# carlobaldassi/gimp-lqr-plugin

Measured on AMD Instinct MI355X. Metric: Mseams*pixels/sec on 4K RGBA, higher is better.
Workload: dtype f32; 1 GPU; batch4k: 64 x 3840x2160 RGBA per GPU, resize to 3640x2160 (200 vertical seams each), side-switch 2; images_per_gpu=64, width=3840, height=2160, new_width=3640, new_height=2160, parallelism=images sharded i mod N, no data-path collective, streams_per_gpu=1

## Files before the change

gimp-lqr-plugin_amd/csrc/k_levels.hip:

```cpp
#include "lqr_common.h"
#include "lqr_kernels.h"

__device__ unsigned long long g_lv_stats[8];
#ifdef LQR_TIMING
__device__ unsigned long long g_lv_time[16][2][10];
#define LTT(i) do { __builtin_amdgcn_sched_barrier(0); const unsigned long long t__ = __builtin_readcyclecounter(); __builtin_amdgcn_sched_barrier(0); ltt[i] += t__ - ltprev; ltprev = t__; } while (0)
extern "C" int lqrhip_band_levels_timing(unsigned long long *out) { (void) hipDeviceSynchronize(); return hipMemcpyFromSymbol(out, HIP_SYMBOL(g_lv_time), sizeof(unsigned long long) * 320) == hipSuccess ? 0 : -1; }
#else
#define LTT(i) do { } while (0)
#endif
__device__ int g_lv_dbg;

#ifdef LQR_JITTER
#define LJIT(site) do { if (dbg & 16) { unsigned h__ = (unsigned) (slot * 131 + L * 17 + (site) * 7 + epoch * 2654435761u + q * 40503u + image * 977u); h__ ^= h__ >> 13; h__ *= 0x5bd1e995u; h__ ^= h__ >> 15; \
    for (unsigned i__ = h__ & 15u; i__ > 0; i__--) __builtin_amdgcn_s_sleep(127); } } while (0)
#else
#define LJIT(site) do { } while (0)
#endif
__device__ __forceinline__ unsigned long long uni64(unsigned long long v)
{
    return ((unsigned long long) (unsigned) __builtin_amdgcn_readfirstlane((int) (v >> 32)) << 32) | (unsigned) __builtin_amdgcn_readfirstlane((int) v);
}
struct LvMask {
    unsigned long long lo;
    __device__ __forceinline__ void set(int t) { lo |= 1ull << t; }
    __device__ __forceinline__ bool has(int t) const { return t >= 0 && t < LV_MAX_TILES && ((lo >> t) & 1ull); }
    __device__ __forceinline__ void set_range(int a, int b) { lo |= ((b - a >= 63) ? ~0ull : ((1ull << (b - a + 1)) - 1ull)) << a; }
    __device__ __forceinline__ int first() const { return lo ? __builtin_ctzll(lo) : -1; }
    __device__ __forceinline__ int last() const { return lo ? 63 - __builtin_clzll(lo) : -1; }
};

template <bool LR, bool RIG, int DELTA, bool RIGM>
__global__ __launch_bounds__(128) __attribute__((amdgpu_waves_per_eu(2, 2)))
void k_band_levels(DevCarver *cs, DpK p, int w, int h, int stride, unsigned long long *exch, int epoch, int *dev_err, int P, int n_img)
{
    static_assert(DELTA >= 1 && DELTA <= LQR_FAST_MAX_DELTA && (DELTA <= 4 || RIG) && (RIG || !RIGM), "delta_x 1 .. 10 (5 .. 10: the rigidity form, with a zero table if there is none); a rigidity mask only matters with rigidity");
    constexpr int PX = 2, HALO = 32, OWN = LV_OWN, HL = 16, R = lv_rows(DELTA, RIGM), TILE = 128;
    static_assert(R * DELTA <= HALO, "a level's errors stay inside the halo");
    typedef LaneVec<2>::F FV;
    typedef LaneVec<2>::L LV;
    typedef GLOBAL_AS FV GFV;
    typedef GLOBAL_AS LV GLV;
    typedef GLOBAL_AS unsigned long long gu64;
    __shared__ int s_tlo[LV_MAX_LEVELS], s_thi[LV_MAX_LEVELS];
    __shared__ int s_fail;
    __shared__ int s_polled;
    __shared__ unsigned long long s_A[2];
        const int tid = threadIdx.x, lane = tid & 63;
    const int q = __builtin_amdgcn_readfirstlane(tid >> 6);
    const int dbg = __builtin_amdgcn_readfirstlane(g_lv_dbg);
    const int b_xcd = (int) blockIdx.x & 7, b_k = (int) blockIdx.x >> 3;
    const int slot = (dbg & 8) ? (int) blockIdx.x % P : b_k % P, image = (dbg & 8) ? (int) blockIdx.x / P : (b_k / P) * 8 + b_xcd;
    if (image >= n_img) return;
    const int nblk = (h + R - 1) / R;
    const int ntiles = lv_tiles(w);
    GCarver c = gview(cs[image]);
    if constexpr (RIG && DELTA == 1 && !RIGM) { c.en = uni_ptr(c.en); c.m = uni_ptr(c.m); c.least = uni_ptr(c.least); }
    const size_t near_off = lv_near_off(ntiles);
    gu64 *ex_img = (gu64 *) exch + exch_image_off(image, near_off);
    gu64 *flagw = ex_img;
    gu64 *gran = ex_img + LV_FLAG_WORDS;
    const float INF = __int_as_float(0x7f800000);
    const float rig_l = p.rigmap[0], rig_r = p.rigmap[2];
    float rg[2 * DELTA + 1];
#pragma unroll
    for (int i = 0; i < 2 * DELTA + 1; i++) rg[i] = p.rigmap[i];
    const int ix_own = 2 * (lane % P), ix_right = 2 * ((lane + 1) % P), ix_left = 2 * ((lane + P - 1) % P);

    for (int i = tid; i < nblk; i += 128) { s_tlo[i] = 1 << 30; s_thi[i] = -1; }
    if (tid == 0) { s_fail = 0; s_polled = -1; }
    __syncthreads();
    for (int y = tid; y < h; y += 128) {
        const int v0 = c.seam_x[y], vm = c.seam_x[max(y - 1, 0)], vp = c.seam_x[min(y + 1, h - 1)];
        const int t0 = max(min(min(v0, vm), vp) - DELTA - 1, 0), t1 = min(max(max(v0, vm), vp) + DELTA, w - 1);
        atomicMin(&s_tlo[y / R], t0); atomicMax(&s_thi[y / R], t1);
    }
    __syncthreads();
    __shared__ unsigned long long s_tm[LV_MAX_LEVELS + 2];
    for (int L = tid; L < nblk + 2; L += 128) {
        unsigned long long m = 0ull;
        if (L < nblk && s_thi[L] >= s_tlo[L]) {
            const int a = max(0, (s_tlo[L] - (OWN - 1 + HALO + 2) + OWN - 1) / OWN), b = min(ntiles - 1, (s_thi[L] + HALO + 2) / OWN);
            m = ((b - a >= 63) ? ~0ull : ((1ull << (b - a + 1)) - 1ull)) << a;
        }
        s_tm[L] = m;
    }
    __syncthreads();
    auto touch_mask = [&](int L) -> LvMask {
        LvMask m;
        m.lo = uni64(s_tm[L]);
        return m;
    };
    unsigned long long res_mine = 0ull;
    for (int t = slot; t < LV_MAX_TILES; t += P) res_mine |= 1ull << t;
    res_mine = uni64(res_mine);
    auto my_tile = [&](const LvMask &A, int which) -> int {
        unsigned long long m = A.lo & res_mine;
        if (which && m) m &= m - 1ull;
        return m ? __builtin_ctzll(m) : -1;
    };
    auto any_collision = [&](const LvMask &A) -> bool {
        const int a = A.first(), b = A.last();
        if (a < 0 || b - a < 2 * P) return false;
        unsigned long long res_zero = 0ull;
        for (int t = 0; t < LV_MAX_TILES; t += P) res_zero |= 1ull << t;
        for (int r = 0; r < P; r++)
            if (__popcll(A.lo & (res_zero << r)) > 2) return true;
        return false;
    };
    auto nearest_tile = [&](int a, int b) -> int {
        const unsigned long long up_m = res_mine & (~0ull << a), dn_m = res_mine & (b >= 63 ? ~0ull : ((1ull << (b + 1)) - 1ull));
        const int up = up_m ? __builtin_ctzll(up_m) : -1, dn = dn_m ? 63 - __builtin_clzll(dn_m) : -1;
        if (up >= 0 && up <= b) return up;
        if (up < 0 || up >= ntiles) return dn;
        if (dn < 0) return up;
        return (up - b <= a - dn) ? up : dn;
    };

    int cur_t = -1, cur_L = -1;
    bool cur_full = false;
    int x0 = 0;
    unsigned lo_off = 0;
    constexpr bool LEAN = RIG && DELTA == 1 && !RIGM;
    bool in[PX] = {false, false}, own = false, interior = false;
    const bool own_lane = lane >= HL && lane < 64 - HL;
    auto X0 = [&]() -> int { int v = x0; asm volatile("" : "+v"(v)); return v; };
    auto in_k = [&](int k) -> bool { if constexpr (LEAN) return (unsigned) (X0() + k) < (unsigned) w; else return in[k]; };
    auto is_own = [&]() -> bool { if constexpr (LEAN) return own_lane && X0() < w; else return own; };
    auto is_interior = [&]() -> bool {
        if constexpr (LEAN) { const int t0 = __builtin_amdgcn_readfirstlane(X0()); return t0 >= 0 && t0 + TILE <= w; }
        else return interior;
    };
    auto set_tile = [&](int t) {
        x0 = t * OWN - HALO + PX * lane;
        lo_off = (unsigned) min(max(x0, 0), stride - PX);
        if constexpr (!LEAN) {
#pragma unroll
            for (int k = 0; k < PX; k++) in[k] = x0 + k >= 0 && x0 + k < w;
            own = own_lane && x0 < w;
            interior = (x0 - PX * lane >= 0) && (x0 - PX * lane + TILE <= w);
        }
    };
    auto owner_of = [&](int t) -> int { return lane < HL ? t - 1 : lane >= 64 - HL ? t + 1 : t; };
    const int owner_col = lane < HL ? HALO + PX * lane : lane >= 64 - HL ? PX * (lane - (64 - HL)) : PX * (lane - HL);
    FV q_e[R], q_mo[R], q_ab, q_rf[RIGM ? R : 1];
    LV q_lo[R];
    q_ab[0] = q_ab[1] = INF;
    auto issue_full = [&](int L) {
        const int ybase = L * R;
#pragma unroll
        for (int r = 0; r < R; r++) {
            const unsigned row = (unsigned) min(ybase + r, h - 1) * (unsigned) stride;
            const unsigned ro = row + lo_off, ro4 = (row << 2) + (lo_off << 2);
            q_e[r] = *(const GFV *) ((const gu8 *) c.en + ro4);
            q_mo[r] = *(const GFV *) ((const gu8 *) c.m + ro4);
            q_lo[r] = *(const GLV *) (c.least + ro);
            if (RIGM) q_rf[RIGM ? r : 0] = *(const GFV *) ((const gu8 *) c.rig + ro4);
        }
        q_ab = *(const GFV *) ((const gu8 *) c.m + ((((unsigned) max(ybase - 1, 0) * (unsigned) stride) + lo_off) << 2));
    };
    float mp[PX] = {INF, INF};
    int acc_l0 = 0, acc_l1 = 0;
    auto batch_u = [&](int ybase) {
        const int nr = min(R, h - ybase);
#pragma unroll
        for (int r = 0; r < R; r++) {
            float mc[PX], e[PX], mo[PX];
            uint32_t lnew = 0;
            bool ch[PX];
#pragma unroll
            for (int k = 0; k < PX; k++) { e[k] = q_e[r][k]; mo[k] = q_mo[r][k]; }
            if constexpr (DELTA == 1 && !RIGM) {
                const float left = __int_as_float(__builtin_amdgcn_mov_dpp(__float_as_int(mp[PX - 1]), DPP_WAVE_SHR1, 0xf, 0xf, true));
                const float right = __int_as_float(__builtin_amdgcn_mov_dpp(__float_as_int(mp[0]), DPP_WAVE_SHL1, 0xf, 0xf, true));
                dp_row<PX, LR, RIG, true, false>(mp, left, right, e, mo, (uint32_t) q_lo[r], in, rig_l, rig_r, mc, lnew, ch);
            } else {
                float nl[DELTA], nr[DELTA], rf[PX];
                lane_reach<PX, DELTA>(mp, nl, nr);
#pragma unroll
                for (int k = 0; k < PX; k++) rf[k] = RIGM ? q_rf[RIGM ? r : 0][k] : 1.0f;
                dp_row_g<PX, DELTA, LR, RIG, RIGM, true, false>(mp, nl, nr, e, mo, (uint32_t) q_lo[r], in, rg, rf, mc, lnew, ch);
            }
            if (r == 0 && ybase == 0) {
#pragma unroll
                for (int k = 0; k < PX; k++) mc[k] = e[k];
                lnew = 0;
            }
            if (r == R - 1) {
                const int msk = (r < nr) ? -1 : 0;
                acc_l0 = (__float_as_int(mc[0]) ^ __float_as_int(mo[0])) & msk;
                acc_l1 = (__float_as_int(mc[1]) ^ __float_as_int(mo[1])) & msk;
            }
#pragma unroll
            for (int k = 0; k < PX; k++) { mp[k] = mc[k]; q_mo[r][k] = mc[k]; }
            q_lo[r] = (LV) lnew;
        }
    };
    auto store_u = [&](int ybase) {
        const bool own_ = is_own();
        const unsigned inc = own_ ? (unsigned) stride : 0u, inc4 = inc * 4u;
        unsigned so = own_ ? (unsigned) ybase * (unsigned) stride + (unsigned) x0 : (unsigned) h * (unsigned) stride + (unsigned) (PX * lane), so4 = so * 4u;
        const int nr = min(R, h - ybase);
#pragma unroll
        for (int r = 0; r < R; r++, so += inc, so4 += inc4) {
            if (r < nr) {
                *(GFV *) ((gu8 *) c.m + so4) = q_mo[r];
                *(GLV *) (c.least + so) = q_lo[r];
            }
        }
    };
    auto wait_level = [&](int L, int spec_t, const LvMask &prev, unsigned long long &fw, unsigned long long (&g)[PX]) -> int {
        const unsigned want = ((unsigned) epoch << 10) | (unsigned) L;
        gu64 *fsrc = flagw + (size_t) ((L - 1) & 1) * 2 * LV_PMAX + (lane < 2 * P ? lane : 0);
        const bool need_g = spec_t >= 0 && prev.has(owner_of(spec_t)) && (in_k(0) || in_k(1));
        gu64 *gsrc = gran + ((size_t) ((L - 1) & 1) * ntiles + (need_g ? owner_of(spec_t) : 0)) * OWN + (need_g ? owner_col : 0);
        int sp = 0;
        while (true) {
            const size_t off = (!(dbg & 4) && (sp & 3) != 3) ? near_off : 0;
            fw = __hip_atomic_load(fsrc + off, __ATOMIC_RELAXED, __HIP_MEMORY_SCOPE_AGENT);
            if (spec_t >= 0) {
#pragma unroll
                for (int k = 0; k < PX; k++) g[k] = __hip_atomic_load(gsrc + off + k, __ATOMIC_RELAXED, __HIP_MEMORY_SCOPE_AGENT);
            }
            const bool okf = __all(lane >= 2 * P || (unsigned) (fw >> 32) == want);
            bool okg = true;
#pragma unroll
            for (int k = 0; k < PX; k++) okg &= (unsigned) (g[k] >> 32) == want;
            if (okf && __all(!need_g || okg)) return 0;
            if (dbg & 2) __builtin_amdgcn_s_sleep(16); else if (okf || sp < 8) __builtin_amdgcn_s_sleep(1); else if (sp < 64) __builtin_amdgcn_s_sleep(8); else __builtin_amdgcn_s_sleep(48);
            ++sp;
            if ((sp & 255) == 0 && dev_failed(dev_err)) return 1;
            if (sp > (1 << 18)) { if (lane == 0) dev_fail(dev_err, DEVERR_TILE_TIMEOUT); return 1; }
        }
    };
    auto row_above = [&](int L, int t, const LvMask &prev, bool have_g, unsigned long long (&g)[PX]) -> int {
        const int u = owner_of(t);
        const bool from_gran = prev.has(u) && (in_k(0) || in_k(1));
        if (!have_g) {
            gu64 *src = gran + ((size_t) ((L - 1) & 1) * ntiles + (from_gran ? u : 0)) * OWN + (from_gran ? owner_col : 0);
            const unsigned want = ((unsigned) epoch << 10) | (unsigned) L;
            int sp = 0;
            while (true) {
                const size_t off = (!(dbg & 4) && (sp & 3) != 3) ? near_off : 0;
#pragma unroll
                for (int k = 0; k < PX; k++) g[k] = __hip_atomic_load(src + off + k, __ATOMIC_RELAXED, __HIP_MEMORY_SCOPE_AGENT);
                bool ok = true;
#pragma unroll
                for (int k = 0; k < PX; k++) ok &= (unsigned) (g[k] >> 32) == want;
                if (__all(ok || !from_gran)) break;
                __builtin_amdgcn_s_sleep(1);
                if (++sp > (1 << 16)) { if (lane == 0) dev_fail(dev_err, DEVERR_TILE_TIMEOUT); return 1; }
            }
        }
#pragma unroll
        for (int k = 0; k < PX; k++) mp[k] = !in_k(k) ? INF : from_gran ? __uint_as_float((unsigned) g[k]) : q_ab[k];
        return 0;
    };
    unsigned n_proc = 0, n_idle = 0, n_sync = 0, n_two = 0;
    int hold_L = -1;
#ifdef LQR_TIMING
    unsigned long long ltt[10] = {0, 0, 0, 0, 0, 0, 0, 0, 0, 0};
    unsigned long long ltprev = __builtin_readcyclecounter();
    const unsigned long long ltstart = ltprev;
#endif
    for (int L = 0; L <= nblk; L++) {
        const bool mine = (L & 1) == q;
        int t = -1;
        bool have_g = false, passed = false;
        unsigned long long g[PX] = {0ull, 0ull};
        LvMask A = {0ull}, A_prev = {0ull};
        if (L > 0) A_prev.lo = uni64(s_A[(L - 1) & 1]);
        LTT(8);
        if (mine) {
            unsigned long long fw = 0;
            A = touch_mask(L);
            passed = true;
            if (L > 0) {
                const int spec_t = (hold_L < 0 && cur_full && cur_L == L && L < nblk && !(dbg & 1)) ? cur_t : -1;
                LJIT(1);
                const int wl_rc = wait_level(L, spec_t, A_prev, fw, g);
                LJIT(2);
                LTT(0);
                if (wl_rc) { LDS_FLAG(s_fail) = 1; passed = false; }
                else if (L < nblk) {
                    const int wl = (int) (unsigned) fw;
                    bool act = false;
                    unsigned wo[2], wr[2], wlf[2];
#pragma unroll
                    for (int i = 0; i < 2; i++) {
                        wo[i] = (unsigned) __builtin_amdgcn_ds_bpermute((ix_own + i) << 2, wl);
                        wr[i] = (unsigned) __builtin_amdgcn_ds_bpermute((ix_right + i) << 2, wl);
                        wlf[i] = (unsigned) __builtin_amdgcn_ds_bpermute((ix_left + i) << 2, wl);
                    }
#pragma unroll
                    for (int i = 0; i < 2; i++) {
                        act |= (wo[i] & 0x900u) == 0x900u && (int) (wo[i] & 0xffu) == lane;
                        act |= (wr[i] & 0xa00u) == 0xa00u && (int) (wr[i] & 0xffu) == lane + 1;
                        act |= (wlf[i] & 0xc00u) == 0xc00u && (int) (wlf[i] & 0xffu) == lane - 1;
                    }
                    A.lo |= __ballot(act && lane < ntiles);
                    have_g = spec_t >= 0;
                }
            }
            if (lane == 0) { s_A[L & 1] = A.lo; if (passed) LDS_FLAG(s_polled) = L; }
        } else {
            int spins = 0;
            while (LDS_FLAG(s_polled) < L && LDS_FLAG(s_fail) != 1 && ++spins < (1 << 24)) __builtin_amdgcn_s_sleep(1);
            passed = LDS_FLAG(s_polled) >= L;
            if (passed) A.lo = uni64(s_A[L & 1]);
            else if (LDS_FLAG(s_fail) != 1) { LDS_FLAG(s_fail) = 1; if (lane == 0) dev_fail(dev_err, DEVERR_TILE_TIMEOUT); }
            LTT(2);
        }
        LTT(1);
        LJIT(3);
        if (hold_L >= 0 && passed) { store_u(hold_L * R); hold_L = -1; }
        LTT(3);
        if (L == nblk) break;
        if (mine && passed && any_collision(A)) {
            if (slot == 0 && lane == 0) { __hip_atomic_fetch_min(c.flags + FLAG_OVF_ROW, L * R, __ATOMIC_RELAXED, __HIP_MEMORY_SCOPE_AGENT); atomicAdd(&g_lv_stats[0], 1ull); }
            LDS_FLAG(s_fail) = 2;
            passed = false;
        }
        if (passed) t = my_tile(A, mine ? 0 : 1);
        if (!mine && t < 0 && passed && lane == 0) {
            const unsigned long long tag = (unsigned long long) (((unsigned) epoch << 10) | (unsigned) (L + 1)) << 32;
            gu64 *fdst = flagw + (size_t) (L & 1) * 2 * LV_PMAX + 2 * slot + 1;
            if (!(dbg & 4)) __hip_atomic_store(fdst + near_off, tag, __ATOMIC_RELAXED, __HIP_MEMORY_SCOPE_WORKGROUP);
            __hip_atomic_store(fdst, tag, __ATOMIC_RELAXED, __HIP_MEMORY_SCOPE_AGENT);
        }
        {
            int ld_t = -1, ld_L = L;
            if (t >= 0) {
                if (!(cur_full && cur_t == t && cur_L == L)) { ld_t = t; n_sync++; have_g = false; }
                if (!mine) n_two++;
            } else if (!mine && passed && L + 1 < nblk) {
                LvMask M = touch_mask(L + 1);
                M.lo |= A.lo;
                int pt = my_tile(M, 0);
                if (pt < 0 && M.first() >= 0) { pt = nearest_tile(M.first(), M.last()); if (pt < M.first() - 1 || pt > M.last() + 1 || pt >= ntiles) pt = -1; }
                ld_t = pt; ld_L = L + 1;
                cur_t = -1; cur_L = ld_L; cur_full = false;
            }
            LTT(1);
            LJIT(4);
            if (ld_t >= 0) { set_tile(ld_t); issue_full(ld_L); cur_t = ld_t; cur_L = ld_L; cur_full = true; }
#ifdef LQR_TIMING
            if (t >= 0 && ld_t >= 0) asm volatile("s_waitcnt vmcnt(0)" ::: "memory");
#endif
            LTT(4);
        }
        unsigned word = 0;
        if (t >= 0) {
            n_proc++;
            if (L > 0 && row_above(L, t, A_prev, have_g, g)) LDS_FLAG(s_fail) = 1;
#ifdef LQR_TIMING
            asm volatile("s_waitcnt vmcnt(0)" ::: "memory");
#endif
            LTT(5);
            if (!is_interior()) {
                const bool ik[PX] = {in_k(0), in_k(1)};
#pragma unroll
                for (int r = 0; r < R; r++)
#pragma unroll
                    for (int k = 0; k < PX; k++) { q_e[r][k] = ik[k] ? q_e[r][k] : INF; q_mo[r][k] = ik[k] ? q_mo[r][k] : INF; }
            }
            batch_u(L * R);
            LTT(6);
            hold_L = L;
            cur_full = false;
            LJIT(5);
            if (L + 1 < nblk && own_lane) {
                gu64 *dst = gran + ((size_t) (L & 1) * ntiles + t) * OWN + PX * (lane - HL);
                const unsigned long long tag = (unsigned long long) (((unsigned) epoch << 10) | (unsigned) (L + 1)) << 32;
#pragma unroll
                for (int k = 0; k < PX; k++) {
                    if (!(dbg & 4)) __hip_atomic_store(dst + near_off + k, tag | __float_as_uint(mp[k]), __ATOMIC_RELAXED, __HIP_MEMORY_SCOPE_WORKGROUP);
                    __hip_atomic_store(dst + k, tag | __float_as_uint(mp[k]), __ATOMIC_RELAXED, __HIP_MEMORY_SCOPE_AGENT);
                }
            }
            const bool chg = own_lane && (acc_l0 | acc_l1) != 0;
            const bool any_o = __any(chg), any_l = __any(chg && lane < 32), any_r = __any(chg && lane >= 32);
            word = 0x800u | (any_o ? 0x100u : 0u) | (any_l ? 0x200u : 0u) | (any_r ? 0x400u : 0u) | (unsigned) t;
        } else if (mine && passed) n_idle++;
        LJIT(6);
        if (lane == 0 && (t >= 0 || mine) && LDS_FLAG(s_fail) == 0) {
            const unsigned long long tag = (unsigned long long) (((unsigned) epoch << 10) | (unsigned) (L + 1)) << 32;
            gu64 *fdst = flagw + (size_t) (L & 1) * 2 * LV_PMAX + 2 * slot + (mine ? 0 : 1);
            if (!(dbg & 4)) __hip_atomic_store(fdst + near_off, tag | word, __ATOMIC_RELAXED, __HIP_MEMORY_SCOPE_WORKGROUP);
            __hip_atomic_store(fdst, tag | word, __ATOMIC_RELAXED, __HIP_MEMORY_SCOPE_AGENT);
        }
        LTT(7);
        asm volatile("s_waitcnt lgkmcnt(0)\n\ts_barrier" ::: "memory");
        LTT(8);
        if (LDS_FLAG(s_fail)) return;
    }
#ifdef LQR_TIMING
    if (image == 0 && lane == 0 && slot < 16) { ltt[9] = __builtin_readcyclecounter() - ltstart; for (int i = 0; i < 10; i++) g_lv_time[slot][q][i] = ltt[i]; }
#endif
    if (lane == 0) { atomicAdd(&g_lv_stats[2], (unsigned long long) n_proc); atomicAdd(&g_lv_stats[3], (unsigned long long) n_idle); if (n_two) atomicAdd(&g_lv_stats[4], (unsigned long long) n_two); }
    if (lane == 0 && n_sync) atomicAdd(&g_lv_stats[1], (unsigned long long) n_sync);
}

extern "C" void lqrhip_band_levels_debug(int v) { if (lqrhip_init() < 0) return; (void) hipMemcpyToSymbol(HIP_SYMBOL(g_lv_dbg), &v, sizeof v); }
extern "C" int lqrhip_band_levels_stats(unsigned long long *out, int reset)
{
    if (lqrhip_init() < 0) return -1;
    (void) hipDeviceSynchronize();
    if (hipMemcpyFromSymbol(out, HIP_SYMBOL(g_lv_stats), sizeof(unsigned long long) * 8) != hipSuccess) return -1;
    if (reset) { unsigned long long z[8] = {0}; (void) hipMemcpyToSymbol(HIP_SYMBOL(g_lv_stats), z, sizeof z); }
    return 0;
}

#define INST(...) template __global__ void k_band_levels<__VA_ARGS__>(DevCarver *, DpK, int, int, int, unsigned long long *, int, int *, int, int);
K_BAND_LEVELS_FORMS(INST)
#undef INST
```

gimp-lqr-plugin_amd/csrc/lqr_geom.h:

```cpp
#pragma once
#include <stddef.h>
#include <stdint.h>
#include "lqr_beside.h"

constexpr int tiles_of(int w, int own) { return (w + own - 1) / own; }
constexpr size_t blocks_of(size_t n, size_t per) { return (n + per - 1) / per; }

constexpr size_t LDS_ATTR_BYTES = 64 * 1024;
constexpr bool lds_needs_attr(size_t bytes) { return bytes > LDS_ATTR_BYTES; }
constexpr size_t VMAP_T_ATTR_BYTES = 56 * 1024;
constexpr bool vmap_t_needs_attr(size_t bytes) { return bytes > VMAP_T_ATTR_BYTES; }

constexpr int PLANE_SLACK = 1024;
constexpr int plane_stride(int w) { return ((w + 16) + 63) & ~63; }
constexpr size_t plane_elems(int stride, int h) { return (size_t) stride * (h + 1) + PLANE_SLACK; }
constexpr int SEAM_X_SLACK = 8;
constexpr size_t seam_x_elems(int h) { return (size_t) h + SEAM_X_SLACK; }
constexpr size_t seam_log_elems(int n_seams, int h) { return (size_t) n_seams * h; }

struct MaskClip { int x0, y0, x1, y1, nx, ny; };
constexpr MaskClip mask_clip(int w0, int h0, int width, int height, int x_off, int y_off, int transposed)
{
    const int wt = transposed ? h0 : w0, ht = transposed ? w0 : h0;
    const int x0 = x_off < 0 ? x_off : 0, y0 = y_off < 0 ? y_off : 0;
    const int x1 = x_off > 0 ? x_off : 0, y1 = y_off > 0 ? y_off : 0;
    const long long xe = (long long) width + x_off, ye = (long long) height + y_off;
    const int x2 = wt < xe ? wt : (int) xe, y2 = ht < ye ? ht : (int) ye;
    return MaskClip{x0, y0, x1, y1, x2 - x1, y2 - y1};
}

constexpr int dppx_px(int px) { return px == 3 ? 2 : px; }
constexpr int dppx_hl(int px) { return px == 3 ? 24 : 16; }
constexpr int dpp_halo(int px) { return dppx_hl(px) * dppx_px(px); }
constexpr int dpp_own(int px) { return 64 * dppx_px(px) - 2 * dpp_halo(px); }
constexpr int dpp_ex_tile(int px) { return px == 3 ? 2 * dpp_own(3) : 2 * 2 * dpp_halo(px); }
constexpr int dpp_tiles(int w, int px) { return tiles_of(w, dpp_own(px)); }
constexpr int DPP_CTR_WORDS = 8;
constexpr size_t dpp_ctr_off(int ntiles, int px) { return (size_t) ntiles * dpp_ex_tile(px); }
constexpr size_t dpp_near_off(int ntiles, int px) { return dpp_ctr_off(ntiles, px) + DPP_CTR_WORDS; }
constexpr size_t exch_image_off(size_t image, size_t near_off) { return image * 2 * near_off; }
constexpr size_t exch_words(size_t near_off, size_t n) { return 2 * near_off * n; }
constexpr int exch_layout_dpp(int px) { return px; }
constexpr int EXCH_LAYOUT_LEVELS = 103;
constexpr int DPP_EPOCH_BITS = 19;
constexpr int dpp_epoch(int launches) { return 1 + (launches % ((1 << DPP_EPOCH_BITS) - 2)); }

constexpr int LV_PMAX = 16;
constexpr int LV_OWN = 64;
constexpr int lv_tiles(int w) { return tiles_of(w, LV_OWN); }
constexpr int LV_FLAG_WORDS = 4 * LV_PMAX;
constexpr size_t lv_near_off(int ntiles) { return (size_t) LV_FLAG_WORDS + (size_t) 2 * ntiles * LV_OWN; }
constexpr int LV_LEVEL_BITS = 10, LV_EPOCH_BITS = 22;
constexpr int lv_epoch(int launches) { return 1 + (launches % ((1 << LV_EPOCH_BITS) - 2)); }
struct LvBlock { int image, slot; };
constexpr unsigned lv_grid(size_t n, int P) { return (unsigned) (8 * ((n + 7) / 8) * P); }
constexpr LvBlock lv_block(int b, int P) { return LvBlock{((b >> 3) / P) * 8 + (b & 7), (b >> 3) % P}; }

struct CuBlock { bool energy; int image, index; };
constexpr int cu_energy_blocks(int n, int h) { return n * bb_energy_entries(h); }
constexpr unsigned cu_grid(unsigned n, int h) { return n * (unsigned) bb_energy_entries(h) + n * (unsigned) bb_carve_entries(h); }
constexpr CuBlock cu_block(unsigned b, int n, int h)
{
    const int eblk = bb_energy_entries(h), ne = n * eblk;
    if ((int) b < ne) {
        const int img = b / eblk, blk = b - img * eblk;
        return CuBlock{true, img, blk};
    }
    const int rblk = bb_carve_entries(h), cb = b - ne, img = cb / rblk, rb = cb - img * rblk;
    return CuBlock{false, img, rb};
}
constexpr unsigned cv_grid(unsigned n, int h) { return n + (unsigned) bb_entries((int) n, h); }
constexpr size_t cv_list_words(int n, int h) { return (size_t) BB_LIST_HEAD + (size_t) bb_entries(n, h); }

constexpr int VP_MAP_SLACK = 64;
constexpr int vp_col_blocks(int w) { return (w + 255) / 256; }
constexpr int vp_quads(int rows) { return (rows + 3) / 4; }
constexpr size_t vp_map_bytes(int nchunks, int stride) { return (size_t) (nchunks + 1) * stride + VP_MAP_SLACK; }
constexpr size_t vp_path_bytes(int nchunks, int stride, int rows) { return vp_map_bytes(nchunks, stride) * 4 * vp_quads(rows); }
constexpr size_t vp_map_row(int chunk, int stride) { return (size_t) chunk * stride; }
constexpr size_t vp_path_chunk(int chunk, int R4, int stride) { return (size_t) chunk * R4 * stride; }
constexpr size_t vp_path_quad(int r4, int stride) { return (size_t) r4 * stride; }
constexpr size_t vp_path_step(int chunk, int R4, int r, int stride, int x) { return (((size_t) chunk * R4 + (r >> 2)) * stride + x) * 4 + (r & 3); }
constexpr size_t vp_solve_lds(int nchunks) { return (size_t) (nchunks + 2) * sizeof(int); }

constexpr int FC_SLACK = 16;
constexpr int fc_w_from(int from, int to, int w_at_to) { return w_at_to + (to - from); }
constexpr int fc_rem_off(int from, int to) { return to - from; }
constexpr size_t fc_lds(int from, int to, int w_from) { return (size_t) (to - from) * sizeof(int) + (size_t) w_from + FC_SLACK; }
constexpr int vsc_lvl_off(int n_seams) { return n_seams; }
constexpr size_t vsc_lds(int n_seams, int wc0) { return ((size_t) n_seams + wc0) * sizeof(int); }
constexpr size_t VSC_LDS_MAX = 150 * 1024;
constexpr size_t inflate_lds(int l, int max_level) { return (size_t) ((l - max_level + 1 + 31) / 32 + 1) * sizeof(unsigned); }
constexpr int VT_LINES = 32;
constexpr size_t vmap_words(int depth) { return (size_t) (depth + 31) / 32; }
constexpr size_t vmap_check_lds(int depth) { return vmap_words(depth) * sizeof(unsigned); }
constexpr size_t vmap_check_t_lds(int depth) { return VT_LINES * vmap_words(depth) * sizeof(unsigned); }
constexpr int vmap_t_blocks(int width) { return tiles_of(width, VT_LINES); }
constexpr size_t band_mw_lds(int h) { return (size_t) h * sizeof(int); }
constexpr size_t band_tw_lds(int h) { return (size_t) 2 * h * sizeof(int); }
constexpr int band_tw_touchR_off(int h) { return h; }
constexpr size_t BAND_MW_LDS_MAX = 60 * 1024, BAND_TW_LDS_MAX = 64 * 1024;
constexpr bool band_mw_fits(int h) { return band_mw_lds(h) <= BAND_MW_LDS_MAX; }
constexpr bool band_tw_fits(int h) { return band_tw_lds(h) <= BAND_TW_LDS_MAX; }
constexpr int sweep_wpad(int w) { return (w + 3) & ~3; }
constexpr size_t sweep_lds(int w) { return (size_t) 2 * sweep_wpad(w) * sizeof(float); }
constexpr size_t fwd_lds(int L) { return (size_t) 2 * L * sizeof(float); }
constexpr int fwd_row_off(int parity, int L) { return parity * L; }

constexpr int CLIP_COST_FLOATS = 4, CLIP_REFRESH_VALUES = 6;
constexpr size_t clip_intensity_elems(int n, size_t px) { return (size_t) n * px; }
constexpr size_t clip_frame_off(int t, size_t px) { return (size_t) t * px; }
constexpr size_t clip_cost_elems(size_t px) { return px * CLIP_COST_FLOATS; }
constexpr size_t clip_cost_off(int y, int x, int L) { return ((size_t) y * L + x) * CLIP_COST_FLOATS; }
constexpr int clip_fold_groups(int n, int group) { return tiles_of(n, group); }
constexpr int clip_refresh_off(int wave) { return wave * CLIP_REFRESH_VALUES; }
constexpr size_t clip_refresh_lds_elems(int threads) { return (size_t) (threads / 64) * CLIP_REFRESH_VALUES; }
```

gimp-lqr-plugin_amd/csrc/lqr_kernels.h:

```cpp
#pragma once
#include "lqr_common.h"
#include "lqr_pixel.h"


template <class FORM> __global__ void k_wk_init(const DevCarver *cs, int w, int h, int stride, typename FORM::Arg a);
template <class FORM> __global__ __launch_bounds__(256) void k_wk_init_visible(const DevCarver *cs, int w0, int h, int stride, typename FORM::Arg a);
#define K_EMAP_FORMS(X) X(0, false) X(1, false) X(2, false) X(3, false) X(4, false) X(5, false) X(6, false) X(0, true) X(1, true) X(2, true) X(6, true)
#define K_EMAP_UPDATE_NT_FORMS(X, ...) X(12, __VA_ARGS__) X(36, __VA_ARGS__) X(68, __VA_ARGS__)
template <int NRG, bool VALUE> __global__ void k_emap_full(const DevCarver *cs, DpK p, int w, int h, int stride);
#define K_WK_INIT_EMAP_FORMS(X) X(0) X(1) X(2) X(3) X(4) X(5) X(6)
template <int NRG> __global__ __launch_bounds__(256) void k_wk_init_emap(const DevCarver *cs, DpK p, int w, int h, int stride);
__global__ void k_mask_add(float *plane, int w0, const uint8_t *mask, int channels, int mw, int x0, int y0, int x1, int y1,
                           int nx, int ny, int transposed, int is_rig, int bias_factor);
template <int NRG, int EU_NT, bool VALUE> __global__ __launch_bounds__(64) void k_emap_update(const DevCarver *cs, DpK p, int w, int h, int stride, int k, int epoch);
template <bool VALUE> __global__ __launch_bounds__(256) void k_frozen_catchup(const DevCarver *cs, int from, int to, int w_from, int h, int stride);

__global__ __launch_bounds__(VPATH_THREADS) void k_vpath(const DevCarver *cs, int w, int h, int stride, int lr, int delta, int log_index, int moved_unit);
#define K_VPATH1_FORMS(X) X(1) X(2) X(3) X(4) X(5) X(6) X(7)
#define K_VP_FORMS(X) K_VPATH1_FORMS(X) X(8) X(9) X(10)
template <int DELTA> __global__ __launch_bounds__(VPATH_THREADS) void k_vpath1(const DevCarver *cs, int w, int h, int stride, int lr, int log_index, int moved_unit);
unsigned long long *lqr_moved_bytes_dev(void);

template <int DELTA> __global__ __launch_bounds__(256) void k_vp_maps(const DevCarver *cs, int w, int h, int stride);
template <int DELTA> __global__ __launch_bounds__(VPATH_THREADS) void k_vp_solve(const DevCarver *cs, int w, int h, int stride, int lr, int log_index, int moved_unit);

__global__ __launch_bounds__(256) void k_carve(const DevCarver *cs, int w, int h, int stride, int delta, int move_dp);
#define K_CARVE_E_FORMS(X) X(0) X(1) X(2) X(3) X(4) X(5) X(6)
template <int NRG> __global__ __launch_bounds__(256) void k_carve_e(const DevCarver *cs, DpK p, int w, int h, int stride, int move_dp, int k, int epoch);
#define K_CARVE_U_FORMS(X) X(0) X(1) X(2) X(3) X(4) X(5) X(6)
template <int NRG> __global__ __launch_bounds__(256) void k_carve_u(const DevCarver *cs, DpK p, int w, int h, int stride, int move_dp, int k, int epoch, int n);
#define K_CARVE_V_DELTAS(X) X(1) X(2)
#define K_CARVE_V_FORMS(X) X(0, 1) X(1, 1) X(2, 1) X(3, 1) X(4, 1) X(5, 1) X(6, 1) X(0, 2) X(1, 2) X(2, 2) X(3, 2) X(4, 2) X(5, 2) X(6, 2)
template <int NRG, int DELTA> __global__ __launch_bounds__(256) __attribute__((amdgpu_waves_per_eu(5))) void k_carve_v(const DevCarver *cs, DpK p, int w, int h, int stride, int lr, int move_dp, int k, int epoch, int n,
                                                                                  int moved_unit, unsigned tag, unsigned long long *list, unsigned long long *moved_bytes, int *dev_err);

#define K_DP_SWEEP_PXT_FORMS(X) X(1) X(2) X(4) X(8) X(16)
#define K_LR_RIG_FORMS(X) X(false, false) X(false, true) X(true, false) X(true, true)
template <int PXT, bool UPDATE, int NTH = DP_THREADS> __global__ __launch_bounds__(NTH) void k_dp_sweep(const DevCarver *cs, DpK p, int w, int h, int stride, int lr);
__global__ __launch_bounds__(64) void k_band_update(const DevCarver *cs, DpK p, int w, int h, int stride, int lr);
template <int PXL, int NW, int R, bool LR, bool RIG> __global__ __launch_bounds__(64 * NW) void k_band_update_mw(const DevCarver *cs, DpK p, int w, int h, int stride);
template <int NW, bool LR, bool RIG> __global__ __launch_bounds__(128 * NW) void k_band_update_tw(const DevCarver *cs, DpK p, int w, int h, int stride, int *dev_err);

template <bool LR, bool RIG> __global__ __launch_bounds__(64) void k_dp_tile(const DevCarver *cs, DpK p, int w, int h, int stride, int y0);
#define K_DP_TILE_P_FORMS_D(X, LR, UPD, D) X(GENERAL, 2, LR, false, UPD, D, false, 16) X(GENERAL, 2, LR, true, UPD, D, false, 16) X(GENERAL, 2, LR, true, UPD, D, true, 16)
#define K_DP_TILE_P_FORMS_W(X, LR, UPD, D) X(GENERAL, 2, LR, true, UPD, D, false, 16) X(GENERAL, 2, LR, true, UPD, D, true, 16)
#define K_DP_TILE_P_FORMS_LR(X, LR, UPD) \
    X(PX4, 4, LR, false, UPD, 1, false, 16) X(PX4, 4, LR, true, UPD, 1, false, 16) X(PLAIN, 2, LR, false, UPD, 1, false, 16) X(PLAIN, 2, LR, true, UPD, 1, false, 16) \
    X(GENERAL, 2, LR, true, UPD, 1, true, 16) K_DP_TILE_P_FORMS_D(X, LR, UPD, 2) K_DP_TILE_P_FORMS_D(X, LR, UPD, 3) K_DP_TILE_P_FORMS_D(X, LR, UPD, 4) \
    K_DP_TILE_P_FORMS_W(X, LR, UPD, 5) K_DP_TILE_P_FORMS_W(X, LR, UPD, 6) K_DP_TILE_P_FORMS_W(X, LR, UPD, 7) K_DP_TILE_P_FORMS_W(X, LR, UPD, 8) K_DP_TILE_P_FORMS_W(X, LR, UPD, 9) K_DP_TILE_P_FORMS_W(X, LR, UPD, 10)
#define K_DP_TILE_P_FORMS_24(X, UPD) X(PLAIN, 2, false, false, UPD, 1, false, 24) X(PLAIN, 2, false, true, UPD, 1, false, 24) X(PLAIN, 2, true, false, UPD, 1, false, 24) X(PLAIN, 2, true, true, UPD, 1, false, 24)
#define K_DP_TILE_P_FORMS(X) K_DP_TILE_P_FORMS_LR(X, false, false) K_DP_TILE_P_FORMS_LR(X, false, true) K_DP_TILE_P_FORMS_LR(X, true, false) K_DP_TILE_P_FORMS_LR(X, true, true) \
    K_DP_TILE_P_FORMS_24(X, false) K_DP_TILE_P_FORMS_24(X, true)
template <int PX, bool LR, bool RIG, bool UPDATE, int DELTA = 1, bool RIGM = false, int HLN = 16>
__global__ __launch_bounds__(64 * DPP_W) void k_dp_tile_p(DevCarver *cs, DpK p, int w, int h, int stride, unsigned long long *exch, int epoch, int *dev_err);

#define K_BAND_LEVELS_FORMS_D(X, LR, D) X(LR, false, D, false) X(LR, true, D, false) X(LR, true, D, true)
#define K_BAND_LEVELS_FORMS_W(X, LR, D) X(LR, true, D, false) X(LR, true, D, true)
#define K_BAND_LEVELS_FORMS_LR(X, LR) K_BAND_LEVELS_FORMS_D(X, LR, 1) K_BAND_LEVELS_FORMS_D(X, LR, 2) K_BAND_LEVELS_FORMS_D(X, LR, 3) K_BAND_LEVELS_FORMS_D(X, LR, 4) \
    K_BAND_LEVELS_FORMS_W(X, LR, 5) K_BAND_LEVELS_FORMS_W(X, LR, 6) K_BAND_LEVELS_FORMS_W(X, LR, 7) K_BAND_LEVELS_FORMS_W(X, LR, 8) K_BAND_LEVELS_FORMS_W(X, LR, 9) K_BAND_LEVELS_FORMS_W(X, LR, 10)
#define K_BAND_LEVELS_FORMS(X) K_BAND_LEVELS_FORMS_LR(X, false) K_BAND_LEVELS_FORMS_LR(X, true)
template <bool LR, bool RIG, int DELTA, bool RIGM>
__global__ __launch_bounds__(128) __attribute__((amdgpu_waves_per_eu(2, 2))) void k_band_levels(DevCarver *cs, DpK p, int w, int h, int stride, unsigned long long *exch, int epoch, int *dev_err, int P, int n_img);

__global__ __launch_bounds__(256) void k_vs_commit(const DevCarver *cs, int w0, int h0, int wc0, int n_seams, int first_level, int finish);
template <bool DEEP> __global__ __launch_bounds__(256) void k_inflate(const InflateDev *jobs, int w0, int w1, int l, int max_level, int *dev_err);
__global__ __launch_bounds__(256) void k_vmap_check(const int32_t *map, int len, int depth, int *dev_err);
__global__ __launch_bounds__(256) void k_vmap_check_t(const int32_t *map, int32_t *out, int width, int height, int depth, int *dev_err);
__global__ __launch_bounds__(256) void k_seam_check(const DevCarver *cs, int h, int wc0, int n_seams, int delta, int *dev_err);
__global__ __launch_bounds__(256) void k_vs_rollback(const DevCarver *cs, size_t n, int first_level, int finish_level);
__global__ void k_inject(const DevCarver *cs, int what, int h, int w0, int log_index, int first_level);
template <bool DEEP> __global__ __launch_bounds__(256) void k_compact(const uint8_t *rgb, const int32_t *vs, const float *bias, const float *rig,
                                                  uint8_t *nrgb, float *nbias, float *nrig, int32_t *nvmap, int w0, int w, int ch, int level, int depth);
template <bool DEEP> __global__ __launch_bounds__(256) void k_compact_jobs(const InflateDev *jobs, int w0, int w, int level);
__global__ void k_transpose(const InflateDev *jobs, int w, int h);
__global__ void k_transpose_px(const InflateDev *jobs, int w, int h);
__global__ __launch_bounds__(256) void k_mask_line_max(const uint8_t *mask, int channels, int width, int a0, int b0, int line_len, int direction, int *out);

#define K_COMPACT_SIZES_FORMS(X) X(false) X(true)
#define K_TRANSPOSE_SIZES_FORMS(X) X(false) X(true)
template <bool DEEP> __global__ __launch_bounds__(256) void k_compact_sizes(const uint8_t *rgb, const int32_t *vs, const SizeJob *jobs, int n_jobs, int w0, int bytes);
template <bool WIDE> __global__ __launch_bounds__(256) void k_transpose_sizes(const SizeJob *jobs, int h, int bytes);

#define K_FWD_INIT_FORMS(X) X(0) X(1) X(2) X(3)
#define K_FWD_SEAM_FORMS(X) X(1) X(2) X(4) X(8) X(16)
template <int DEPTH> __global__ __launch_bounds__(256) void k_fwd_init(const FwdJob *jobs, int L, int H, int fw0, int strided, DeepRead rd, int w_start, int orientation);
template <int PXT> __global__ __launch_bounds__(FWD_THREADS) void k_fwd_seam(const FwdJob *jobs, int wc, int L, int H);
__global__ __launch_bounds__(FWD_REMOVE_THREADS) void k_fwd_remove(const FwdJob *jobs, int wc, int L, int H, int level, int orientation);

#define K_CLIP_SEAM_FORMS(X) X(1) X(2) X(4) X(8) X(16)
__global__ __launch_bounds__(CLIPFWD_FOLD_THREADS) void k_clip_fold(const FwdJob *jobs, const float *in, int first, int count, int last, int L, int H, int fw0, int strided,
                                                                   int w_start, float temporal, float *cost, float *pm);
template <int PXT> __global__ __launch_bounds__(FWD_THREADS) void k_clip_seam(const float *cost, int8_t *choice, int32_t *seam, int wc, int L, int H);
__global__ __launch_bounds__(FWD_REMOVE_THREADS) void k_clip_remove(float *cost, uint16_t *pos, const int32_t *seam, int32_t *map, int wc, int L, int H, int level, int orientation);
__global__ __launch_bounds__(CLIPFWD_REFRESH_THREADS) void k_clip_refresh(const float *in, int n, float *cost, const uint16_t *pos, const int32_t *seam, int wn, int L, int H);

#define K_STATIC_FOLD_FORMS(X) X(0, 0, true) X(1, 0, true) X(2, 0, true) X(6, 0, true) X(0, 0, false) X(1, 0, false) X(2, 0, false) X(6, 0, false) \
    X(0, 1, false) X(1, 1, false) X(2, 1, false) X(6, 1, false) X(0, 2, false) X(1, 2, false) X(2, 2, false) X(6, 2, false) \
    X(0, 3, false) X(1, 3, false) X(2, 3, false) X(6, 3, false)
template <int NRG, int DEPTH, bool PACKED>
__global__ __launch_bounds__(STATIC_THREADS) void k_static_fold(const StaticFrame *frames, int count, int first, int W, int H, int transposed, int orientation, DeepRead rd,
                                                     float alpha, float *s_plane, float *t_plane, float *i_plane, float *e_out);

template <class T> __global__ __launch_bounds__(256) void k_mask_add_f(float *plane, int w0, const T *mask, int mw, int x0, int y0, int x1, int y1, int nx, int ny,
                                                                       int transposed, int is_rig, int bias_factor);
__global__ __launch_bounds__(256) void k_mask_scatter(float *plane, const int *index, const double *value, size_t n, int is_rig);
__global__ __launch_bounds__(256) void k_plane_transpose(const float *plane, float *out, int w0, int h0);

template <bool PIC> __global__ __launch_bounds__(256) void k_energy_range(const DevCarver *cs, int w, int h, int stride, float *partials);
__global__ __launch_bounds__(256) void k_energy_plane(const DevCarver *cs, int w, int h, int stride, int transposed, int normalised,
                                                      const float *partials, int n_partials, float *out);
#define K_ENERGY_OUT_FORMS_T(X, T) X(T, 0) X(T, 1) X(T, 2) X(T, 3)
#define K_ENERGY_OUT_FORMS(X) K_ENERGY_OUT_FORMS_T(X, 0) K_ENERGY_OUT_FORMS_T(X, 1) K_ENERGY_OUT_FORMS_T(X, 2) K_ENERGY_OUT_FORMS_T(X, 3) K_ENERGY_OUT_FORMS_T(X, 4) K_ENERGY_OUT_FORMS_T(X, 5) K_ENERGY_OUT_FORMS_T(X, 6)
template <int TYPE, int DEPTH> __global__ __launch_bounds__(256) void k_energy_out(const DevCarver *cs, int w, int h, int stride, int transposed,
                                                                                    const float *partials, int n_partials, uint8_t *out);
```

gimp-lqr-plugin_amd/csrc/lqr_plan.h:

```cpp
#pragma once
#include <algorithm>
#include <stddef.h>
#include "../../include/lqr_hip.h"
#include "lqr_beside.h"
#include "lqr_geom.h"

#define DP_THREADS 1024
constexpr int dpp_rb(int px, int delta) { return delta >= 5 ? dpp_halo(2) / delta : delta >= 3 ? 8 : dpp_halo(px) / delta; }
constexpr int DPP_R = 16;
constexpr int DPP_W = 2;
static_assert(dpp_halo(2) % (2 * DPP_R) == 0 && dpp_halo(4) % (2 * DPP_R) == 0, "a block (halo / delta_x rows, delta_x <= 2) is a whole number of batches");
constexpr int DPP_BLK_BITS = 12;
static_assert(DPP_EPOCH_BITS + DPP_BLK_BITS == 31, "a granule's tag: epoch above block index, the sign bit free");
#define DPT_ROWS 32
#define DPT_OWN 192
constexpr int LV_MAX_TILES = 64;
constexpr int LV_MAX_LEVELS = 1020;
static_assert(LV_MAX_LEVELS + 1 < (1 << LV_LEVEL_BITS), "level + 1 fits its field of the tags");
constexpr int lv_rows(int delta, bool rigm = false) { return delta == 1 ? (rigm ? 16 : 32) : delta == 2 ? 16 : delta <= 4 ? 8 : 32 / delta; }
constexpr int LQR_FAST_MAX_DELTA = 10;
constexpr int VP_REACH = 56;
constexpr int VP_STAGE = 20;
constexpr int vp_chunk_rows(int delta) { return VP_REACH / delta; }
constexpr int eu_samples(int delta_x) { return delta_x <= 2 ? 12 : delta_x <= 8 ? 36 : 68; }
#ifndef FROZEN_LAG_MAX
#define FROZEN_LAG_MAX 128
#endif
constexpr int frozen_lag(int images) { return images <= 4 ? FROZEN_LAG_MAX / 4 : FROZEN_LAG_MAX; }
constexpr int LV_AUTO_MIN = 7;

struct PlanKnobs {
    int vpath_mode = -1;
    int vpath_par_max = 3, vpath_min_rows = 1000;
    int sweep_threads = 256;
    int carve_fused = 4;
    int carve_beside = -1;
    int backtrack_beside = -1;
    int update_mode = -1;
    int band_levels = -1;
    int dpp_limit = -1;
    int dpp_px = 0;
    int sub_batches = 0;
    long long tiled_update_px = 8LL * 3840 * 2160;
};
struct PlanDevice {
    int wgs_plain = 0, wgs_general = 0, wgs_px4 = 0, wgs_levels = 0;
    int n_cu = 0, hw_queues = 0;
};
struct PlanBatch {
    int images = 1;
    bool shared = false;
    int shared_n = 1;
    bool spin = true;
    int wk_h = 0;
    bool value = false;
    bool rigmask = false;
    size_t group() const { return (size_t) images * (size_t) std::max(shared_n, 1); }
    bool rigm(bool use_rig) const { return use_rig && rigmask; }
};

struct DpPlan {
    int form = -1, px = 0, per = 0, threads = 0;
    bool general = false;
    size_t lds = 0;
};
struct StepPlan {
    int backtrack = 0;
    int vp_rows = 0, vp_chunks = 0;
    int carve = 0;
    bool energy_beside = false;
    bool backtrack_beside = false;
    bool catchup = false;
    int eu_nt = 0;
    bool full = false;
    int band = -1;
    int levels_P = 0;
    DpPlan dp;
};

static inline int plan_limit(const PlanKnobs &k, int bound) { return k.dpp_limit >= 0 ? std::min(k.dpp_limit, bound) : bound; }

static inline int plan_streams(const PlanKnobs &k, const PlanDevice &d, int n)
{
    const int nb = k.sub_batches ? k.sub_batches : d.hw_queues >= 8 ? (n >= 49 ? 4 : n >= 32 ? 2 : 1) : 1;
    return n >= 2 * nb ? nb : 1;
}

static inline int plan_persistent_px(const PlanKnobs &k, const PlanDevice &d, const PlanBatch &b, int w, bool general, int delta, int images)
{
    if (b.shared || !b.spin) return 0;
    const size_t n = (size_t) images;
    const int limit = plan_limit(k, general ? d.wgs_general : d.wgs_plain);
    const int maxblk = (1 << DPP_BLK_BITS) - 1;
    if (!general && delta == 1 && (k.dpp_px == 3 || k.dpp_px == 0) && b.wk_h <= maxblk * dpp_rb(3, 1) &&
        tiles_of(w, dpp_own(3)) * n <= (size_t) std::min(limit, k.dpp_px == 3 ? limit : d.n_cu)) return 3;
    if ((general || (k.dpp_px != 4 && k.dpp_px != 3)) && b.wk_h <= maxblk * dpp_rb(2, delta) && tiles_of(w, dpp_own(2)) * n <= (size_t) limit) return 2;
    if (!general && k.dpp_px != 2 && k.dpp_px != 3 && b.wk_h <= maxblk * dpp_halo(4) && tiles_of(w, dpp_own(4)) * n <= (size_t) plan_limit(k, d.wgs_px4)) return 4;
    return 0;
}
static inline DpPlan plan_persistent(int px, bool general, int per)
{
    DpPlan p;
    p.form = general ? LQRHIP_CENSUS_TILE_P_GENERAL : px == 3 ? LQRHIP_CENSUS_TILE_P_G3 : px == 2 ? LQRHIP_CENSUS_TILE_P_G2 : LQRHIP_CENSUS_TILE_P_G4;
    p.px = px; p.general = general; p.per = per;
    return p;
}

static inline DpPlan plan_sweep(const PlanKnobs &k, int w, bool update)
{
    DpPlan p;
    p.form = update ? LQRHIP_CENSUS_SWEEP_UPDATE : LQRHIP_CENSUS_SWEEP_FULL;
    p.threads = (update && k.sweep_threads == 256 && w <= 16 * 256) ? 256 : DP_THREADS;
    for (p.px = 1; p.px <= 16 && p.px * p.threads < w;) p.px *= 2;
    if (p.px > 16) p.px = 0;
    p.lds = sweep_lds(w);
    return p;
}

static inline DpPlan plan_full_dp(const PlanKnobs &k, const PlanDevice &d, const PlanBatch &b, int w, int delta, bool use_rig)
{
    const bool general = delta != 1 || b.rigm(use_rig);
    if (delta >= 1 && delta <= LQR_FAST_MAX_DELTA) {
        int per = b.images, px;
        while (!(px = plan_persistent_px(k, d, b, w, general, delta, per)) && general && per > 1) per = (per + 1) / 2;
        if (px) return plan_persistent(px, general, per);
        if (!general) { DpPlan p; p.form = LQRHIP_CENSUS_DP_TILE; return p; }
    }
    return plan_sweep(k, w, false);
}

static inline bool levels_auto(const PlanKnobs &k, int delta, size_t group, bool plain)
{
    return k.update_mode < 0 && delta <= 4 && group >= 8 && (group <= 64 || !plain);
}
static inline int plan_levels_P(const PlanKnobs &k, const PlanDevice &d, const PlanBatch &b, int w, int h, int delta)
{
    if (!b.spin || k.band_levels == 0 || delta < 1 || delta > LQR_FAST_MAX_DELTA || tiles_of(h, lv_rows(delta, true)) > LV_MAX_LEVELS || tiles_of(w, 64) > LV_MAX_TILES) return 0;
    const int per_batch = plan_limit(k, d.wgs_levels) / std::max(b.shared_n, 1);
    const int want = k.band_levels > 0 ? k.band_levels : std::max(LV_AUTO_MIN, std::min(12, (int) ((b.shared ? 384 : 2 * d.n_cu) / std::max<size_t>(b.group(), 1))));
    const int P = std::min({LV_PMAX, per_batch / std::max(b.images, 1), want});
    return P >= (k.band_levels > 0 ? 1 : LV_AUTO_MIN) ? P : 0;
}
static inline int plan_general_batch_limit(const PlanKnobs &k, const PlanDevice &d, int w, int delta)
{
    const int tiled = plan_limit(k, d.wgs_general) / tiles_of(w, dpp_own(2));
    const int lv = plan_limit(k, d.wgs_levels) / LV_AUTO_MIN;
    return levels_auto(k, delta, (size_t) std::max(lv, 0), false) && k.band_levels != 0 && tiles_of(w, 64) <= LV_MAX_TILES ? std::max(tiled, lv) : tiled;
}

constexpr int CARVE_BESIDE_MIN = 8;
static inline bool plan_carve_beside(const PlanKnobs &k, const PlanBatch &b, int delta, int wnew)
{
    if (k.carve_beside == 0 || delta > 2 || b.value || wnew <= 1) return false;
    return k.carve_beside > 0 || (!b.shared && b.group() >= (size_t) CARVE_BESIDE_MIN);
}

constexpr int BACKTRACK_BESIDE_MIN = 8;
static inline bool plan_backtrack_beside(const PlanKnobs &k, const PlanBatch &b, int delta, int h, bool energy_beside, int backtrack, bool catchup)
{
    if (k.backtrack_beside == 0 || !energy_beside || backtrack != LQRHIP_CENSUS_VPATH1 || delta < 1 || delta > 2 || !b.spin || catchup) return false;
    if (h < BB_MIN_ROWS || h > BB_MAX_ROWS || b.images > BB_MAX_IMAGES) return false;
    return k.backtrack_beside > 0 || (!b.shared && b.group() >= (size_t) BACKTRACK_BESIDE_MIN);
}

static inline StepPlan plan_seam_step(const PlanKnobs &k, const PlanDevice &d, const PlanBatch &b, int delta, bool use_rig, int w, int h, bool full_rebuild, int lag)
{
    StepPlan s;
    const int wnew = w - 1, mode = k.update_mode;
    const bool fast_delta = delta >= 1 && delta <= LQR_FAST_MAX_DELTA, general = delta != 1 || b.rigm(use_rig);
    if (fast_delta && h >= 2 && k.vpath_mode != 0 && (k.vpath_mode == 1 || delta >= 5 || (b.group() <= (size_t) k.vpath_par_max && h >= k.vpath_min_rows))) {
        s.backtrack = LQRHIP_CENSUS_VP_PARALLEL;
        s.vp_rows = vp_chunk_rows(delta);
        s.vp_chunks = tiles_of(h - 1, s.vp_rows);
    } else s.backtrack = delta >= 1 && delta <= 7 ? LQRHIP_CENSUS_VPATH1 : LQRHIP_CENSUS_VPATH;
    s.carve = delta <= 2 && b.group() <= (size_t) k.carve_fused && wnew > 1 && !b.value ? LQRHIP_CENSUS_CARVE_E : LQRHIP_CENSUS_CARVE;
    s.energy_beside = s.carve == LQRHIP_CENSUS_CARVE && plan_carve_beside(k, b, delta, wnew);
    s.catchup = lag > frozen_lag(b.images);
    s.backtrack_beside = plan_backtrack_beside(k, b, delta, h, s.energy_beside, s.backtrack, s.catchup);
    s.eu_nt = eu_samples(delta);
    if (wnew <= 1) return s;
    if (full_rebuild) {
        s.full = true;
        s.dp = plan_full_dp(k, d, b, wnew, delta, use_rig);
        return s;
    }
    const bool plain = !general && mode != 3;
    const bool tiled = (plain ? (mode < 0 ? (long long) b.images * w * h <= k.tiled_update_px : mode == 1) : (fast_delta && mode != 0 && mode != 2 && mode != 3)) &&
                       plan_persistent_px(k, d, b, w, general, delta, b.images) != 0;
    if (fast_delta && mode != 3 && (mode == 5 || levels_auto(k, delta, b.group(), plain))) s.levels_P = plan_levels_P(k, d, b, wnew, h, delta);
    if (s.levels_P > 0) s.band = LQRHIP_CENSUS_BAND_LEVELS;
    else if (tiled) {
        s.dp = plan_persistent(plan_persistent_px(k, d, b, wnew, general, delta, b.images), general, b.images);
        return s;
    } else if (plain && band_mw_fits(h)) {
        s.band = mode != 2 && wnew <= 4200 && band_tw_fits(h) ? LQRHIP_CENSUS_BAND_TW : wnew > 4200 ? LQRHIP_CENSUS_BAND_MW16 : LQRHIP_CENSUS_BAND_MW8;
    } else s.band = LQRHIP_CENSUS_BAND_GENERIC;
    s.dp = plan_sweep(k, wnew, true);
    return s;
}
```

gimp-lqr-plugin_amd/csrc/lqr_shim.hip:

```cpp
#include "lqr_common.h"
#include "lqr_kernels.h"
#include "lqr_own.h"
#include "lqr_pool.h"
#include "lqr_stage.h"
#include <atomic>
#include <memory>
#include <dirent.h>

static thread_local std::string g_err;
static int g_device = -1;

static int *g_dev_err_host = nullptr;
static int *g_dev_err = nullptr;

#define HIPCK_VOID(expr) do { hipError_t e__ = (expr); if (e__ != hipSuccess) { g_err = std::string(#expr) + ": " + hipGetErrorString(e__); (void) hipGetLastError(); } } while (0)
#define HIPCK(expr)                                                                   \
    do {                                                                              \
        hipError_t e__ = (expr);                                                      \
        if (e__ != hipSuccess) {                                                      \
            g_err = std::string(#expr) + ": " + hipGetErrorString(e__);               \
            (void) hipGetLastError();                                                 \
            return (e__ == hipErrorOutOfMemory) ? LQRHIP_ENOMEM : LQRHIP_EHIP;        \
        }                                                                             \
    } while (0)

static PlanKnobs g_knobs;
static PlanDevice g_dev;

namespace {
struct WorkingPlanes {
    DevBuf<uint32_t> pix;
    DevBuf<float> en, m, m2, bias, rig;
    DevBuf<int8_t> least, least2;
    DevBuf<int32_t> seam_x, seam_log, flags;
    DevBuf<int8_t> vp_map, vp_path;
};
}
struct __attribute__((visibility("hidden"))) LqrHipCarver {
    int ch = 0;
    int depth = 0;
    int luma = 0;
    int mode = RD_RGB, alpha = -1, black = -1;
    int pix_deep = 0;
    int w0 = 0, h0 = 0;
    DevBuf<uint8_t> rgb0;
    DevBuf<int32_t> vs;
    DevBuf<float> bias0, rig0;
    int active = 0;
    int stride = 0, wk_h = 0;
    WorkingPlanes wk;
    int log_cap = 0, log_h = 0;
    int frozen_epoch = 0;
    int owed_to = 0, owed_w = 0, owed_h = 0;
    LqrHipCarver *root = nullptr;
    std::vector<LqrHipCarver *> aux;
    LqrHipBatch *batch = nullptr;
};

static inline size_t px_bytes(const LqrHipCarver *c) { return (size_t) c->ch << (c->depth == 0 ? 0 : c->depth == 1 ? 1 : c->depth == 2 ? 2 : 3); }
static inline int32_t *vs_of(const LqrHipCarver *c) { return (c->root ? c->root : c)->vs; }

namespace {
struct PlaneJob {
    LqrHipCarver *c;
    DevBuf<uint8_t> nrgb;
    DevBuf<float> nbias, nrig;
};
}
struct PlaneJobs {
    std::vector<PlaneJob> jobs;
    std::vector<DevBuf<int32_t>> new_vs;
    std::vector<InflateDev> dev;
    DevBuf<InflateDev> d_dev;
    size_t n_narrow = 0;
    int add(LqrHipCarver *c, const int32_t *vs_old, int32_t *nvs, size_t n1)
    {
        jobs.push_back(PlaneJob{c, {}, {}, {}});
        PlaneJob &j = jobs.back();
        int rc = j.nrgb.alloc(n1 * px_bytes(c), "&j.nrgb");
        if (!rc && c->bias0) rc = j.nbias.alloc(n1, "&j.nbias");
        if (!rc && c->rig0) rc = j.nrig.alloc(n1, "&j.nrig");
        if (rc) return rc;
        dev.push_back(InflateDev{c->rgb0, vs_old, c->bias0, c->rig0, j.nrgb, nvs, j.nbias, j.nrig, (int) px_bytes(c), c->depth});
        return 0;
    }
    int stage(hipStream_t s, bool by_width)
    {
        n_narrow = std::stable_partition(dev.begin(), dev.end(), [&](const InflateDev &d) { return d.ch <= 4 && (by_width || d.depth == 0); }) - dev.begin();
        int rc = d_dev.alloc(dev.size(), "&d_dev");
        if (rc) return rc;
        HIPCK(hipMemcpyAsync(d_dev, dev.data(), dev.size() * sizeof(InflateDev), hipMemcpyHostToDevice, s));
        return 0;
    }
    size_t n_wide() const { return dev.size() - n_narrow; }
    const InflateDev *d_wide() const { return d_dev + n_narrow; }
};
static void commit(PlaneJobs &pj)
{
    for (auto &j : pj.jobs) {
        j.c->rgb0 = std::move(j.nrgb);
        if (j.nbias) j.c->bias0 = std::move(j.nbias);
        if (j.nrig) j.c->rig0 = std::move(j.nrig);
    }
}

struct PendingInflate { PlaneJobs pj; int kind = 0 , w1 = 0, h1 = 0; };

struct LqrHipBatch {
    std::vector<LqrHipCarver *> cs;
    DevCarver *d_desc = nullptr;
    size_t desc_cap = 0;
    hipStream_t stream = nullptr;
    DevBuf<unsigned long long> exch;
    int exch_ntiles = 0, exch_n = 0, exch_px = 0;
    int tile_epoch = 0;
    DevBuf<unsigned long long> wlist;
    unsigned wlist_launches = 0;
    bool dirty = true;
    int shared_n = 1;
    bool shared = false;
    bool safe = false;
    std::unique_ptr<PendingInflate> pending_inflate;
};
static bool g_no_spin = false;

struct ProfRec {
    std::vector<std::pair<hipEvent_t, hipEvent_t>> ev;
    double bytes = 0;
};
static int g_prof = 0;
static std::map<std::string, ProfRec> g_profrec;
static hipStream_t g_stream0 = nullptr;
static unsigned long long g_census[LQRHIP_CENSUS_SLOTS];
#define CENSUS(slot) (g_census[(slot)]++)
extern "C" int lqrhip_launch_census(unsigned long long *out, int n, int reset)
{
    if (out && n > 0) memcpy(out, g_census, (size_t) std::min(n, (int) LQRHIP_CENSUS_SLOTS) * sizeof g_census[0]);
    if (reset) memset(g_census, 0, sizeof g_census);
    return LQRHIP_CENSUS_SLOTS;
}

extern "C" const char *lqrhip_last_error(void) { return g_err.c_str(); }

static void dpp_resident_workgroups(int dev)
{
    hipDeviceProp_t prop;
    if (hipGetDeviceProperties(&prop, dev) != hipSuccess || prop.multiProcessorCount <= 0) return;
    enum { PX4, PLAIN, GENERAL, LEVELS, N_CLASSES };
    int per_cu[N_CLASSES] = {1 << 20, 1 << 20, 1 << 20, 1 << 20};
    auto q = [&](int cls, auto kern, int threads) {
        int n = 0;
        if (hipOccupancyMaxActiveBlocksPerMultiprocessor(&n, kern, threads, 0) != hipSuccess) { (void) hipGetLastError(); n = 0; }
        per_cu[cls] = std::min(per_cu[cls], n);
    };
#define QUERY(CLASS, ...) q(CLASS, k_dp_tile_p<__VA_ARGS__>, 64 * DPP_W);
    K_DP_TILE_P_FORMS(QUERY)
#undef QUERY
#define QUERY(...) q(LEVELS, k_band_levels<__VA_ARGS__>, 128);
    K_BAND_LEVELS_FORMS(QUERY)
#undef QUERY
    auto bound = [&](int blocks) { return std::max(0, blocks - 1) * prop.multiProcessorCount; };
    g_dev.n_cu = prop.multiProcessorCount;
    g_dev.wgs_px4 = bound(per_cu[PX4]);
    g_dev.wgs_plain = bound(std::min(per_cu[PX4], per_cu[PLAIN]));
    g_dev.wgs_general = bound(per_cu[GENERAL]);
    g_dev.wgs_levels = bound(per_cu[LEVELS]);
}

static bool kfd_is_open(void)
{
    DIR *d = opendir("/proc/self/fd");
    if (!d) return true;
    bool open_ = false;
    while (struct dirent *e = readdir(d)) {
        if (e->d_name[0] == '.') continue;
        char path[64], link[64];
        snprintf(path, sizeof path, "/proc/self/fd/%s", e->d_name);
        const ssize_t n = readlink(path, link, sizeof link - 1);
        if (n <= 0) continue;
        link[n] = 0;
        if (strcmp(link, "/dev/kfd") == 0) { open_ = true; break; }
    }
    closedir(d);
    return open_;
}
__attribute__((constructor)) static void lqrhip_on_load(void)
{
    if (!kfd_is_open()) setenv("GPU_MAX_HW_QUEUES", "8", 0);
}

extern "C" int lqrhip_init(void)
{
    if (g_device >= 0) return g_device;
    int n = 0;
    if (hipGetDeviceCount(&n) != hipSuccess || n <= 0) {
        g_err = "no HIP device visible: the MI355X engine needs a gfx950 GPU (there is no CPU fallback)";
        (void) hipGetLastError();
        return LQRHIP_EHIP;
    }
    int dev = 0;
    const char *lr = getenv("LOCAL_RANK");
    if (lr) dev = atoi(lr) % n;
    HIPCK(hipSetDevice(dev));
    HIPCK(hipStreamCreateWithFlags(&g_stream0, hipStreamNonBlocking));
    HIPCK(hipHostMalloc((void **) &g_dev_err_host, sizeof(int), hipHostMallocMapped));
    *g_dev_err_host = 0;
    HIPCK(hipHostGetDevicePointer((void **) &g_dev_err, g_dev_err_host, 0));
    dpp_resident_workgroups(dev);
    g_device = dev;
    return dev;
}

static std::vector<LqrHipBatch *> g_live_batches;
static void invalidate_all_batches(void);
static unsigned long long g_fault_stats[8];
extern "C" void lqrhip_set_no_spin(int on) { g_no_spin = on != 0; }
extern "C" int lqrhip_get_no_spin(void) { return g_no_spin ? 1 : 0; }
static int check_dev_error(void)
{
    if (!g_dev_err_host || *g_dev_err_host == 0) return 0;
    const int code = *g_dev_err_host;
    *g_dev_err_host = 0;
    invalidate_all_batches();
    switch (code) {
    case DEVERR_TILE_TIMEOUT:
        g_fault_stats[0]++;
        if (!g_no_spin) fprintf(stderr, "liblqr-hip: a persistent kernel's workgroups were not co-resident in time (GPU shared or partitioned?): "
                                        "this process now uses the non-spinning kernels\n");
        g_no_spin = true;
        g_err = "persistent tiled DP sweep: a neighbour tile never became resident (GPU shared or partitioned?); results of this session are invalid";
        break;
    case DEVERR_BAND_PREDICTION: g_fault_stats[1]++; g_err = "band update: activity prediction failed; results of this session are invalid"; break;
    case DEVERR_SEAMLOG: g_fault_stats[2]++; g_err = "self-check: the session's seam log does not describe delta_x-connected seams inside the frame; results of this session are invalid"; break;
    case DEVERR_LEVELS: g_fault_stats[3]++; g_err = "self-check: a level of the session is missing or occurs twice in a row of the visibility map; results of this session are invalid"; break;
    default: g_err = "device-side failure " + std::to_string(code) + "; results of this session are invalid"; break;
    }
    return LQRHIP_EFAULT;
}
extern "C" int lqrhip_fault_stats(unsigned long long *out8, int reset)
{
    memcpy(out8, g_fault_stats, sizeof g_fault_stats);
    if (reset) memset(g_fault_stats, 0, sizeof g_fault_stats);
    return 0;
}

__global__ void k_poison_random(unsigned *p, size_t n, int mode, int stride, int c0, int c1, int r0, int r1)
{
    for (size_t i = (size_t) blockIdx.x * blockDim.x + threadIdx.x; i < n; i += (size_t) gridDim.x * blockDim.x) {
        if (stride > 0) {
            const int col = (int) (i % stride), row = (int) (i / stride);
            if (col < c0 || col >= c1 || row < r0 || row >= r1) { p[i] = 0; continue; }
        }
        unsigned hsh = (unsigned) i * 2654435761u + 0x9e3779b9u;
        hsh ^= hsh >> 15; hsh *= 0x85ebca6bu; hsh ^= hsh >> 13; hsh *= 0xc2b2ae35u; hsh ^= hsh >> 16;
        p[i] = mode == 1 ? __float_as_uint((float) (hsh >> 8) * (100.0f / 16777216.0f)) : mode == 2 ? (hsh >> 21) : hsh;
    }
}
static int g_poison = -2;
static unsigned g_poison32 = 0;
static int pool_poison(void *p, size_t sz, const char *name)
{
    if (g_poison == -2) {
        const char *e = getenv("LQRHIP_POISON");
        g_poison = -1;
        if (e && e[0] == '0' && e[1] == 'x') { g_poison = 256; g_poison32 = (unsigned) strtoul(e, nullptr, 16); }
        else if (e && e[0] == 'r') g_poison = 256 + atoi(e + 1);
        else if (e && *e) g_poison = atoi(e) & 255;
    }
    if (g_poison < 0) return 0;
    {
        static long seq = 0, lo = 0, hi = -1;
        static int logit = -1;
        if (logit < 0) {
            logit = getenv("LQRHIP_POISON_LOG") != nullptr;
            const char *r = getenv("LQRHIP_POISON_RANGE");
            if (r) sscanf(r, "%ld:%ld", &lo, &hi);
        }
        const long me = seq++;
        if (logit) fprintf(stderr, "alloc %ld %zu %s\n", me, sz, name);
        if (hi >= 0 && (me < lo || me >= hi)) { HIPCK(hipMemset(p, 0, sz)); HIPCK(hipDeviceSynchronize()); return 0; }
    }
    if (g_poison > 256) {
        static int win[5] = {0, 0, 0, 0, 0};
        static bool once = false;
        if (!once) { once = true; const char *wv = getenv("LQRHIP_POISON_WINDOW"); if (wv) sscanf(wv, "%d:%d:%d:%d:%d", win, win + 1, win + 2, win + 3, win + 4); }
        hipLaunchKernelGGL(k_poison_random, dim3(1024), dim3(256), 0, 0, (unsigned *) p, sz / 4, g_poison - 256, win[0], win[1], win[2], win[3], win[4]);
    }
    else if (g_poison == 256) HIPCK(hipMemsetD32((hipDeviceptr_t) p, (int) g_poison32, sz / 4));
    else HIPCK(hipMemset(p, g_poison, sz));
    HIPCK(hipDeviceSynchronize());
    return 0;
}

static int raw_alloc(void **p, size_t bytes, std::string &why)
{
    hipError_t e = hipMalloc(p, bytes);
    if (e == hipSuccess) return 0;
    why = std::string("e: ") + hipGetErrorString(e);
    (void) hipGetLastError();
    return e == hipErrorOutOfMemory ? LQRHIP_ENOMEM : LQRHIP_EHIP;
}
static void raw_free(void *p) { (void) hipFree(p); }
static BlockCache g_cache((size_t) 24 << 30, LQRHIP_ENOMEM, raw_alloc, raw_free, pool_poison);
extern "C" void lqrhip_debug_fail_alloc(int nth) { g_cache.fail_in(nth); }
static int lqr_pool_alloc(void **p, size_t bytes, const char *name) { return g_cache.alloc(p, bytes, name, g_err); }
static void lqr_pool_free(void *p) { g_cache.free(p); }
extern "C" unsigned long long lqrhip_debug_pool_live(void) { return g_cache.live(); }

static void lqr_stream_wait(void *stream) { (void) hipStreamSynchronize((hipStream_t) stream); }

static hipError_t dzero(void *p, size_t bytes)
{
    hipError_t e = hipMemsetAsync(p, 0, bytes, g_stream0);
    return e != hipSuccess ? e : hipStreamSynchronize(g_stream0);
}

static const int STAGE_SLOTS = 16;
namespace {
struct Stream0Stage final : StageDevice {
    hipEvent_t ev[STAGE_SLOTS] = {};
    int slot_create(int slot, size_t bytes, void **host) override
    {
        hipError_t e = hipHostMalloc(host, bytes, hipHostMallocDefault);
        if (e == hipSuccess && (e = hipEventCreateWithFlags(&ev[slot], hipEventDisableTiming)) != hipSuccess) (void) hipHostFree(*host);
        if (e == hipSuccess) return 0;
        g_err = std::string("staging buffers: ") + hipGetErrorString(e);
        (void) hipGetLastError();
        return e == hipErrorOutOfMemory ? LQRHIP_ENOMEM : LQRHIP_EHIP;
    }
    void slot_destroy(int slot, void *host) override { (void) hipHostFree(host); (void) hipEventDestroy(ev[slot]); }
    int copy_up(void *dst, const void *src, size_t n) override { HIPCK(hipMemcpyAsync(dst, src, n, hipMemcpyHostToDevice, g_stream0)); return 0; }
    int copy_down(void *dst, const void *src, size_t n) override { HIPCK(hipMemcpyAsync(dst, src, n, hipMemcpyDeviceToHost, g_stream0)); return 0; }
    int record(int slot) override { HIPCK(hipEventRecord(ev[slot], g_stream0)); return 0; }
    int wait(int slot) override { HIPCK(hipEventSynchronize(ev[slot])); return 0; }
    bool landed(int slot) override { return hipEventQuery(ev[slot]) == hipSuccess; }
    int wait_stream(bool quiet) override
    {
        hipError_t e = hipStreamSynchronize(g_stream0);
        if (e == hipSuccess) return 0;
        if (!quiet) g_err = std::string("upload: ") + hipGetErrorString(e);
        return LQRHIP_EHIP;
    }
};
}
static StageRing &stage_ring(void)
{
    static Stream0Stage dev;
    static StageRing *ring = [] {
        const unsigned hw = std::thread::hardware_concurrency();
        return new StageRing(dev, STAGE_SLOTS, (size_t) 4 << 20, hw >= 16 ? 8 : hw >= 4 ? (int) hw / 2 : 1);
    }();
    return *ring;
}
static int h2d_staged(void *dst, const void *src, size_t bytes) { return stage_ring().upload(dst, src, bytes); }
static int d2h_staged(void *dst, const void *src, size_t bytes) { return stage_ring().download(dst, src, bytes); }

static inline bool reads_value(const LqrHipCarver *c)
{
    if (c->depth != 0 || c->ch > 4 || (c->mode != RD_GREY && c->mode != RD_RGB)) return true;
    return c->black >= 0 || c->alpha != (c->ch == 2 ? 1 : c->ch == 4 ? 3 : -1);
}
static inline DeepRead deep_read(const LqrHipCarver *c) { return DeepRead{c->ch, c->mode, c->alpha, c->black, c->luma}; }
template <class F> static inline void with_form(const LqrHipCarver *c, F f)
{
    if (reads_value(c)) f(std::true_type{}); else f(std::false_type{});
}
constexpr int plane_nrg(bool value, int nrg) { return value && nrg >= 3 && nrg <= 5 ? nrg - 3 : nrg; }
static inline int nrg_index(int nrg_func) { return nrg_func >= 0 && nrg_func <= 5 ? nrg_func : 6; }
static int no_form(const char *family) { g_err = std::string(family) + ": no instantiation for the parameters asked for"; return LQRHIP_EARG; }
#define LISTED_CASE_(N) if (v__ == N) { f__(std::integral_constant<int, N>{}); return true; }
#define with_listed(LIST, v, f) [&](int v__, auto f__) { LIST(LISTED_CASE_) return false; }(v, f)
static void default_read(LqrHipCarver *c)
{
    c->mode = c->ch <= 2 ? RD_GREY : c->ch <= 4 ? RD_RGB : c->ch == 5 ? RD_CMYK : RD_CUSTOM;
    c->alpha = c->ch == 2 ? 1 : c->ch == 4 ? 3 : c->ch == 5 ? 4 : -1;
    c->black = c->ch == 5 ? 3 : -1;
}

static int batch_sync_of(LqrHipCarver *c)
{
    LqrHipCarver *r = c->root ? c->root : c;
    if (r->batch) HIPCK(hipStreamSynchronize(r->batch->stream));
    return 0;
}

extern "C" LqrHipCarver *lqrhip_carver_create_ext(const void *rgb, int w, int h, int channels, int depth)
{
    if (depth < 0 || depth > 3 || channels < 1 || channels > LQRHIP_MAX_CHANNELS) { g_err = "unsupported colour depth / channels"; return nullptr; }
    if (lqrhip_init() < 0) return nullptr;
    LqrHipCarver *c = new LqrHipCarver();
    c->ch = channels; c->depth = depth; c->w0 = w; c->h0 = h;
    default_read(c);
    const size_t n = (size_t) w * h, bytes = n * px_bytes(c);
    if (c->rgb0.alloc(bytes, "&c->rgb0") || c->vs.alloc(n, "&c->vs")) { lqrhip_carver_destroy(c); return nullptr; }
    if (hipMemsetAsync(c->vs, 0, n * sizeof(int32_t), g_stream0) != hipSuccess || h2d_staged(c->rgb0, rgb, bytes) != 0) {
        g_err = "upload failed";
        lqrhip_carver_destroy(c);
        return nullptr;
    }
    return c;
}

extern "C" LqrHipCarver *lqrhip_carver_create(const unsigned char *rgb, int w, int h, int channels)
{
    return lqrhip_carver_create_ext(rgb, w, h, channels, 0);
}

extern "C" int lqrhip_carver_set_read_luma(LqrHipCarver *c, int luma)
{
    const int changed = reads_value(c) && (luma != 0) != (c->luma != 0);
    c->luma = luma != 0;
    return changed;
}

extern "C" int lqrhip_carver_set_read(LqrHipCarver *c, int image_type, int alpha, int black)
{
    static const int mode_of[8] = {RD_RGB, RD_RGB, RD_GREY, RD_GREY, RD_CMY, RD_CMYK, RD_CMYK, RD_CUSTOM};
    if (image_type < 0 || image_type > 7 || alpha >= c->ch || black >= c->ch) return LQRHIP_EARG;
    const bool was = reads_value(c);
    const int mode = mode_of[image_type], a = alpha < 0 ? -1 : alpha, k = black < 0 ? -1 : black;
    const bool differs = mode != c->mode || a != c->alpha || k != c->black;
    c->mode = mode; c->alpha = a; c->black = k;
    return (differs && (was || reads_value(c))) ? 1 : 0;
}

static inline void drop_catchup(LqrHipCarver *c)
{
    c->owed_to = 0; c->owed_w = 0; c->owed_h = 0;
    c->frozen_epoch = 0;
}

static void free_working(LqrHipCarver *c)
{
    c->wk = WorkingPlanes();
    c->log_cap = 0; c->log_h = 0;
    drop_catchup(c);
}

extern "C" void lqrhip_carver_destroy(LqrHipCarver *c)
{
    if (!c) return;
    {
        LqrHipCarver *r = c->root ? c->root : c;
        if (r->batch && r->batch->stream) (void) hipStreamSynchronize(r->batch->stream);
        if (c->batch && c->batch != r->batch && c->batch->stream) (void) hipStreamSynchronize(c->batch->stream);
        if (g_stream0) (void) hipStreamSynchronize(g_stream0);
        (void) hipGetLastError();
    }
    delete c;
}

extern "C" int lqrhip_carver_attach(LqrHipCarver *root, LqrHipCarver *aux)
{
    if (root->w0 != aux->w0 || root->h0 != aux->h0) return LQRHIP_EARG;
    aux->vs.reset();
    aux->root = root;
    root->aux.push_back(aux);
    if (root->batch) root->batch->dirty = true;
    return 0;
}

static int ensure_working(LqrHipCarver *c, int w, int h)
{
    int stride = plane_stride(w);
    bool need_bias = c->bias0 != nullptr, need_rig = c->rig0 != nullptr;
    const int deep = reads_value(c) ? 1 : 0;
    WorkingPlanes &k = c->wk;
    if (k.pix && c->stride == stride && c->wk_h == h && (!!k.bias == need_bias) && (!!k.rig == need_rig) && c->pix_deep == deep) return 0;
    free_working(c);
// ... 197 lines not shown
    if (lqrhip_init() < 0 || n <= 0) return nullptr;
    LqrHipBatch *b = new LqrHipBatch();
    for (int i = 0; i < n; i++) {
        b->cs.push_back(carvers[i]);
        carvers[i]->batch = b;
    }
    hipError_t e = hipSuccess;
    if (!g_parked_streams.empty()) { b->stream = g_parked_streams.back(); g_parked_streams.pop_back(); g_fixed_stats[0]++; }
    else e = hipStreamCreateWithFlags(&b->stream, hipStreamNonBlocking);
    if (e == hipSuccess) {
        auto it = g_parked_desc.lower_bound((size_t) n);
        if (it != g_parked_desc.end()) { b->d_desc = it->second; b->desc_cap = it->first; g_parked_desc.erase(it); }
        else if ((e = hipMalloc((void **) &b->d_desc, sizeof(DevCarver) * n)) == hipSuccess) b->desc_cap = (size_t) n;
    }
    if (e != hipSuccess) {
        g_err = "batch_create failed";
        (void) hipGetLastError();
        if (b->stream) (void) hipStreamDestroy(b->stream);
        for (auto *c : b->cs) if (c->batch == b) c->batch = nullptr;
        delete b;
        return nullptr;
    }
    g_live_batches.push_back(b);
    return b;
}

static void invalidate_all_batches(void)
{
    for (auto *b : g_live_batches) { b->exch_ntiles = 0; b->dirty = true; }
}

extern "C" void lqrhip_batch_abort(LqrHipBatch *b)
{
    if (!b) return;
    (void) hipStreamSynchronize(b->stream);
    (void) hipGetLastError();
    b->pending_inflate.reset();
    if (g_dev_err_host) *g_dev_err_host = 0;
    invalidate_all_batches();
}

extern "C" void lqrhip_batch_destroy(LqrHipBatch *b)
{
    if (!b) return;
    g_live_batches.erase(std::remove(g_live_batches.begin(), g_live_batches.end(), b), g_live_batches.end());
    if (b->stream) (void) hipStreamSynchronize(b->stream);
    for (auto *c : b->cs) if (c->batch == b) c->batch = nullptr;
    if (b->stream) {
        if (g_parked_streams.size() < MAX_PARKED) g_parked_streams.push_back(b->stream);
        else (void) hipStreamDestroy(b->stream);
    }
    if (b->d_desc) {
        if (g_parked_desc.size() < MAX_PARKED) g_parked_desc.emplace(b->desc_cap, b->d_desc);
        else (void) hipFree(b->d_desc);
    }
    delete b;
}

extern "C" int lqrhip_batch_sync(LqrHipBatch *b)
{
    HIPCK(hipStreamSynchronize(b->stream));
    return check_dev_error();
}
extern "C" void *lqrhip_batch_stream(LqrHipBatch *b) { return (void *) b->stream; }

static DevCarver make_desc(const LqrHipCarver *c)
{
    DevCarver d;
    const WorkingPlanes &k = c->wk;
    d.rgb0 = c->rgb0; d.vs = vs_of(c); d.bias0 = c->bias0; d.rig0 = c->rig0;
    d.pix = k.pix; d.en = k.en; d.m = k.m; d.least = k.least; d.m2 = k.m2; d.least2 = k.least2; d.bias = k.bias; d.rig = k.rig;
    d.seam_x = k.seam_x; d.seam_log = k.seam_log; d.flags = k.flags;
    d.vp_map = k.vp_map; d.vp_path = k.vp_path;
    return d;
}

static int batch_upload(LqrHipBatch *b)
{
    if (!b->dirty) return 0;
    std::vector<DevCarver> h;
    for (auto *c : b->cs) h.push_back(make_desc(c));
    HIPCK(hipStreamSynchronize(b->stream));
    HIPCK(hipMemcpy(b->d_desc, h.data(), sizeof(DevCarver) * h.size(), hipMemcpyHostToDevice));
    b->dirty = false;
    return 0;
}

static DpK make_dpk(const LqrHipDpParams *p, int ch)
{
    DpK k;
    k.delta = p->delta_x; k.use_rig = p->use_rigidity;
    memcpy(k.rigmap, p->rigidity_map, sizeof k.rigmap);
    k.nrg = p->nrg_func; k.radius = p->nrg_radius; k.w_start = p->w_start; k.ch = ch;
    return k;
}

struct ProfScope {
    ProfRec *rec = nullptr;
    hipEvent_t e0 = nullptr, e1 = nullptr;
    hipStream_t s;
    ProfScope(const char *name, hipStream_t stream, double bytes) : s(stream)
    {
        if (!g_prof || (g_prof == 2 && strcmp(name, "carve") != 0)) return;
        rec = &g_profrec[name];
        rec->bytes += bytes;
        (void) hipEventCreate(&e0); (void) hipEventCreate(&e1);
        (void) hipEventRecord(e0, s);
    }
    ~ProfScope()
    {
        if (!rec) return;
        (void) hipEventRecord(e1, s);
        rec->ev.emplace_back(e0, e1);
    }
};

extern "C" void lqrhip_prof_enable(int on) { g_prof = on; }
extern "C" void lqrhip_prof_reset(void)
{
    for (auto &kv : g_profrec) for (auto &e : kv.second.ev) { (void) hipEventDestroy(e.first); (void) hipEventDestroy(e.second); }
    g_profrec.clear();
}
extern "C" int lqrhip_prof_get(const char *kernel, double *ms_total, long long *launches, double *bytes_total)
{
    auto it = g_profrec.find(kernel);
    *ms_total = 0; *launches = 0; *bytes_total = 0;
    if (it == g_profrec.end()) return 0;
    (void) hipDeviceSynchronize();
    for (auto &e : it->second.ev) {
        float ms = 0;
        if (hipEventElapsedTime(&ms, e.first, e.second) == hipSuccess) *ms_total += ms;
    }
    *launches = (long long) it->second.ev.size();
    *bytes_total = it->second.bytes;
    return 0;
}

extern "C" int lqrhip_prof_get_union(const char *kernel, double *ms_union)
{
    *ms_union = 0;
    auto it = g_profrec.find(kernel);
    if (it == g_profrec.end() || it->second.ev.empty()) return 0;
    (void) hipDeviceSynchronize();
    const hipEvent_t base = it->second.ev[0].first;
    std::vector<std::pair<float, float>> iv;
    for (auto &e : it->second.ev) {
        float a = 0, b = 0;
        if (hipEventElapsedTime(&a, base, e.first) != hipSuccess) { (void) hipGetLastError(); float t = 0; if (hipEventElapsedTime(&t, e.first, base) == hipSuccess) a = -t; else (void) hipGetLastError(); }
        if (hipEventElapsedTime(&b, base, e.second) != hipSuccess) { (void) hipGetLastError(); float t = 0; if (hipEventElapsedTime(&t, e.second, base) == hipSuccess) b = -t; else (void) hipGetLastError(); }
        iv.emplace_back(a, b);
    }
    std::sort(iv.begin(), iv.end());
    float end = -1e30f;
    for (auto &p : iv) {
        if (p.first > end) { *ms_union += p.second - p.first; end = p.second; }
        else if (p.second > end) { *ms_union += p.second - end; end = p.second; }
    }
    return 0;
}

static int pay_catchup(LqrHipBatch *b);
static int wk_init_prepare(LqrHipBatch *b)
{
    LqrHipCarver *c0 = b->cs[0];
    int w = c0->w0, h = c0->h0, rc;
    for (auto *c : b->cs) {
        if (c->w0 != w || c->h0 != h || c->ch != c0->ch || c->depth != c0->depth || c->luma != c0->luma || c->mode != c0->mode ||
            c->alpha != c0->alpha || c->black != c0->black)
            return LQRHIP_EARG;
        if ((rc = ensure_working(c, w, h))) return rc;
    }
    if ((rc = batch_upload(b))) return rc;
    for (auto *c : b->cs) drop_catchup(c);
    return 0;
}
extern "C" int lqrhip_wk_init(LqrHipBatch *b, int from_visible)
{
    LqrHipCarver *c0 = b->cs[0];
    int w = c0->w0, h = c0->h0, rc;
    if ((rc = wk_init_prepare(b))) return rc;
    const dim3 grid(tiles_of(c0->stride, 256), h, (unsigned) b->cs.size()), grid_v(h, (unsigned) b->cs.size());
#define LAUNCH_WK(FORM, arg) do { if (from_visible) hipLaunchKernelGGL(k_wk_init_visible<FORM>, grid_v, dim3(256), 0, b->stream, b->d_desc, w, h, c0->stride, arg); \
                                  else hipLaunchKernelGGL(k_wk_init<FORM>, grid, dim3(256), 0, b->stream, b->d_desc, w, h, c0->stride, arg); } while (0)
    if (!reads_value(c0)) LAUNCH_WK(PixPacked, c0->ch);
    else if (c0->depth == 0) LAUNCH_WK(PixValue<0>, deep_read(c0));
    else if (c0->depth == 1) LAUNCH_WK(PixValue<1>, deep_read(c0));
    else if (c0->depth == 2) LAUNCH_WK(PixValue<2>, deep_read(c0));
    else LAUNCH_WK(PixValue<3>, deep_read(c0));
#undef LAUNCH_WK
    HIPCK(hipGetLastError());
    return 0;
}

extern "C" int lqrhip_emap_build(LqrHipBatch *b, const LqrHipDpParams *p, int w, int h)
{
    int rc;
    if ((rc = pay_catchup(b))) return rc;
    if ((rc = batch_upload(b))) return rc;
    LqrHipCarver *c0 = b->cs[0];
    dim3 grid(tiles_of(w, 256), h, (unsigned) b->cs.size());
    DpK k = make_dpk(p, c0->ch);
    const bool value = reads_value(c0);
    const int nrg = plane_nrg(value, nrg_index(p->nrg_func));
#define CASE(N, V) if (nrg == N && value == V) hipLaunchKernelGGL((k_emap_full<N, V>), grid, dim3(256), 0, b->stream, b->d_desc, k, w, h, c0->stride); else
    K_EMAP_FORMS(CASE) return no_form("k_emap_full");
#undef CASE
    HIPCK(hipGetLastError());
    return 0;
}

extern "C" int lqrhip_wk_init_emap(LqrHipBatch *b, const LqrHipDpParams *p, int w, int h)
{
    LqrHipCarver *c0 = b->cs[0];
    int rc;
    if (reads_value(c0) || w != c0->w0 || h != c0->h0) return (rc = lqrhip_wk_init(b, 0)) ? rc : lqrhip_emap_build(b, p, w, h);
    if ((rc = wk_init_prepare(b))) return rc;
    const dim3 grid(tiles_of(tiles_of(c0->stride, 4), 256), h, (unsigned) b->cs.size());
    DpK k = make_dpk(p, c0->ch);
    const int nrg = nrg_index(p->nrg_func);
#define CASE(N) if (nrg == N) hipLaunchKernelGGL(k_wk_init_emap<N>, grid, dim3(256), 0, b->stream, b->d_desc, k, w, h, c0->stride); else
    K_WK_INIT_EMAP_FORMS(CASE) return no_form("k_wk_init_emap");
#undef CASE
    HIPCK(hipGetLastError());
    return 0;
}

extern "C" int lqrhip_energy_out(LqrHipBatch *b, int w, int h, int transposed, int form, int depth, int image_type, void *out, int on_device)
{
    static const int channels_of[7] = {3, 4, 1, 2, 3, 4, 5};
    if (b->cs.size() != 1 || !out || w < 1 || h < 1 || form < 0 || form > 2) { g_err = "energy read-out: one carver, a buffer, form 0 .. 2"; return LQRHIP_EARG; }
    if (form != 2) { depth = 2; image_type = 2; }
    if (depth < 0 || depth > 3 || image_type < 0 || image_type > 6) { g_err = "energy read-out: depth 0 .. 3, image type 0 .. 6"; return LQRHIP_EARG; }
    int rc;
    if ((rc = batch_upload(b))) return rc;
    LqrHipCarver *c0 = b->cs[0];
    if (!c0->wk.en) return LQRHIP_EARG;
    const size_t bytes = (size_t) w * h * channels_of[image_type] << depth;
    const int chunks = (w + EO_CHUNK - 1) / EO_CHUNK;
    const int n_partials = form ? (int) std::min((long long) EO_MAX_PARTIALS, (long long) h * chunks) : 0;
    Scratch tmp(b->stream);
    float *partials = form ? tmp.get<float>((size_t) 2 * n_partials, "&partials", rc) : nullptr;
    if (rc) return rc;
    uint8_t *staged = on_device ? nullptr : tmp.get<uint8_t>(bytes, "&staged", rc);
    if (rc) return rc;
    uint8_t *dst = on_device ? (uint8_t *) out : staged;
    {
        ProfScope prof("energy_out", b->stream, (double) w * h * sizeof(float) * (form ? 2 : 1) + (double) bytes);
        if (form == 1) hipLaunchKernelGGL(k_energy_range<false>, dim3(n_partials), dim3(256), 0, b->stream, b->d_desc, w, h, c0->stride, partials);
        if (form == 2) hipLaunchKernelGGL(k_energy_range<true>, dim3(n_partials), dim3(256), 0, b->stream, b->d_desc, w, h, c0->stride, partials);
        const int W = transposed ? h : w, H = transposed ? w : h;
        const dim3 grid((W + EO_TILE - 1) / EO_TILE, (H + EO_TILE - 1) / EO_TILE);
#define CASE(T, D) if (image_type == T && depth == D) hipLaunchKernelGGL((k_energy_out<T, D>), grid, dim3(256), 0, b->stream, b->d_desc, w, h, c0->stride, transposed, partials, n_partials, dst); else
        if (form != 2)
            hipLaunchKernelGGL(k_energy_plane, grid, dim3(256), 0, b->stream, b->d_desc, w, h, c0->stride, transposed, form, partials, n_partials, (float *) dst);
        else K_ENERGY_OUT_FORMS(CASE) return no_form("k_energy_out");
#undef CASE
    }
    hipError_t e = hipGetLastError();
    if (e == hipSuccess) e = hipStreamSynchronize(b->stream);
    if (e != hipSuccess) { g_err = std::string("energy read-out: ") + hipGetErrorString(e); (void) hipGetLastError(); return LQRHIP_EHIP; }
    if ((rc = check_dev_error())) return rc;
    if (!on_device && (rc = d2h_staged(out, staged, bytes))) return rc;
    tmp.done();
    return 0;
}

static int launch_dp_tiled(LqrHipBatch *b, const DpK &k, int w, int h, int lr)
{
    LqrHipCarver *c0 = b->cs[0];
    const dim3 grid(tiles_of(w, DPT_OWN), (unsigned) b->cs.size());
    for (int y0 = 0; y0 < h; y0 += DPT_ROWS) {
        CENSUS(LQRHIP_CENSUS_DP_TILE);
#define CASE(LRV, RIGV) if ((lr != 0) == LRV && (k.use_rig != 0) == RIGV) hipLaunchKernelGGL((k_dp_tile<LRV, RIGV>), grid, dim3(64), 0, b->stream, b->d_desc, k, w, h, c0->stride, y0); else
        K_LR_RIG_FORMS(CASE) return no_form("k_dp_tile");
#undef CASE
    }
    HIPCK(hipGetLastError());
    return 0;
}

extern "C" void lqrhip_set_vpath_mode(int mode, int par_max) { g_knobs.vpath_mode = mode; if (par_max > 0) g_knobs.vpath_par_max = par_max; }
extern "C" void lqrhip_set_sweep_threads(int n) { g_knobs.sweep_threads = n == 256 ? 256 : DP_THREADS; }
extern "C" void lqrhip_set_carve_fused(int max_images) { g_knobs.carve_fused = max_images == 1 ? 4 : max_images < 0 ? 0 : max_images; }
extern "C" void lqrhip_set_carve_beside(int mode) { g_knobs.carve_beside = mode < 0 ? -1 : mode ? 1 : 0; }
static unsigned long long g_carve_beside_launches;
extern "C" unsigned long long lqrhip_carve_beside_launches(int reset)
{
    const unsigned long long v = g_carve_beside_launches;
    if (reset) g_carve_beside_launches = 0;
    return v;
}
extern "C" void lqrhip_set_backtrack_beside(int mode) { g_knobs.backtrack_beside = mode < 0 ? -1 : mode ? 1 : 0; }
static unsigned long long g_backtrack_beside_launches;
extern "C" unsigned long long lqrhip_backtrack_beside_launches(int reset)
{
    const unsigned long long v = g_backtrack_beside_launches;
    if (reset) g_backtrack_beside_launches = 0;
    return v;
}
extern "C" void lqrhip_set_update_mode(int mode) { g_knobs.update_mode = mode; }
extern "C" void lqrhip_set_dp_persistent_px(int px) { g_knobs.dpp_px = (px == 2 || px == 3 || px == 4) ? px : 0; }
extern "C" void lqrhip_set_dp_persistent_limit(int workgroups) { g_knobs.dpp_limit = workgroups; }
extern "C" void lqrhip_set_band_levels(int slots) { g_knobs.band_levels = slots; }
static PlanBatch plan_batch(const LqrHipBatch *b)
{
    PlanBatch pb;
    pb.images = (int) b->cs.size(); pb.shared = b->shared; pb.shared_n = b->shared_n; pb.spin = !(b->safe || g_no_spin);
    pb.wk_h = b->cs[0]->wk_h; pb.value = reads_value(b->cs[0]);
    for (auto *c : b->cs) pb.rigmask |= c->wk.rig != nullptr;
    return pb;
}
extern "C" int lqrhip_general_batch_limit_delta(int w, int delta)
{
    return lqrhip_init() < 0 || w < 1 ? 0 : plan_general_batch_limit(g_knobs, g_dev, w, delta);
}
extern "C" int lqrhip_general_batch_limit(int w) { return lqrhip_general_batch_limit_delta(w, 2); }

template <class Ready, class Make> static int grow_pairs(LqrHipBatch *b, Ready ready, Make make)
{
    int rc;
    bool grew = false;
    for (auto *c : b->cs) {
        if (ready(c)) continue;
        if (!grew) { HIPCK(hipStreamSynchronize(b->stream)); grew = true; }
        if ((rc = make(c))) return rc;
    }
    if (!grew) return 0;
    b->dirty = true;
    return batch_upload(b);
}

static int exch_ensure(LqrHipBatch *b, size_t near_off, int ntiles, int n, int layout)
{
    int rc;
    bool grew = false;
    const size_t need_elems = exch_words(near_off, (size_t) n);
    if (b->exch.size() < need_elems) HIPCK(hipStreamSynchronize(b->stream));
    if ((rc = b->exch.ensure(need_elems, "&b->exch", &grew))) return rc;
    if (grew) b->exch_ntiles = 0;
    if (b->exch_ntiles != ntiles || b->exch_n != n || b->exch_px != layout) {
        HIPCK(hipMemsetAsync(b->exch, 0, need_elems * sizeof(unsigned long long), b->stream));
        b->exch_ntiles = ntiles; b->exch_n = n; b->exch_px = layout;
    }
    return 0;
}

struct DpForm { bool lr, rig; int delta; bool rigm; };
static inline DpForm dp_form(const DpK &k, int lr, bool rigm) { return DpForm{lr != 0, k.use_rig != 0 || k.delta >= 5, k.delta, rigm}; }

template <bool UPDATE>
static int launch_dp_persistent(LqrHipBatch *b, const DpK &k, const DpPlan &dp, bool rigm, int w, int h, int lr, int first, int count)
{
    LqrHipCarver *c0 = b->cs[0];
    const size_t n = (size_t) count;
    const int px = dp.px;
    if (!px || (UPDATE && n != b->cs.size())) return LQRHIP_EARG;
    const int ntiles = dpp_tiles(w, px);
    int rc;
    if ((rc = exch_ensure(b, dpp_near_off(ntiles, px), ntiles, (int) n, exch_layout_dpp(px)))) return rc;
    auto make_second = [&](LqrHipCarver *c) -> int {
        const size_t pe = plane_elems(c->stride, c->wk_h);
        DevBuf<float> m2;
        DevBuf<int8_t> least2;
        int err;
        if ((err = m2.alloc(pe, "&c->m2")) || (err = least2.alloc(pe, "&c->least2"))) return err;
        hipError_t e = hipMemsetAsync(m2, 0, pe * sizeof(float), b->stream);
        if (e == hipSuccess) e = hipMemsetAsync(least2, 0, pe, b->stream);
        if (e != hipSuccess) { lqr_stream_wait(b->stream); HIPCK(e); }
        c->wk.m2 = std::move(m2); c->wk.least2 = std::move(least2);
        return 0;
    };
    if (UPDATE && (rc = grow_pairs(b, [](LqrHipCarver *c) { return c->wk.m2 && c->wk.least2; }, make_second))) return rc;
    const int epoch = dpp_epoch(b->tile_epoch++);
    const dim3 grid(ntiles, (unsigned) n);
    CENSUS(dp.general ? LQRHIP_CENSUS_TILE_P_GENERAL : px == 3 ? LQRHIP_CENSUS_TILE_P_G3 : px == 2 ? LQRHIP_CENSUS_TILE_P_G2 : LQRHIP_CENSUS_TILE_P_G4);
    const DpForm f = dp_form(k, lr, rigm);
    const int px_lane = px == 4 ? 4 : 2, hln = px == 3 ? 24 : 16;
    const bool found = [&] {
#define CASE(CLASS, PX, LR, RIG, UPD, DELTA, RIGM, HLN)                                                                         \
        if constexpr (UPD == UPDATE)                                                                                            \
            if (px_lane == PX && f.lr == LR && f.rig == RIG && f.delta == DELTA && f.rigm == RIGM && hln == HLN) {              \
                hipLaunchKernelGGL((k_dp_tile_p<PX, LR, RIG, UPD, DELTA, RIGM, HLN>), grid, dim3(64 * DPP_W), 0, b->stream, b->d_desc + first, k, w, h, c0->stride, b->exch.get(), epoch, g_dev_err); \
                return true;                                                                                                    \
            }
        K_DP_TILE_P_FORMS(CASE)
#undef CASE
        return false;
    }();
    if (!found) return no_form("k_dp_tile_p");
    HIPCK(hipGetLastError());
    if (UPDATE)
        for (auto *c : b->cs) { std::swap(c->wk.m, c->wk.m2); std::swap(c->wk.least, c->wk.least2); }
    return 0;
}

template <bool UPDATE>
static int launch_dp(LqrHipBatch *b, const DpK &k, const DpPlan &dp, bool rigm, int w, int h, int lr)
{
    LqrHipCarver *c0 = b->cs[0];
    if (dp.form == LQRHIP_CENSUS_DP_TILE) return launch_dp_tiled(b, k, w, h, lr);
    if (dp.form != LQRHIP_CENSUS_SWEEP_FULL && dp.form != LQRHIP_CENSUS_SWEEP_UPDATE) {
        const int total = (int) b->cs.size();
        int rc;
        for (int first = 0; first < total; first += std::max(dp.per, 1))
            if ((rc = launch_dp_persistent<UPDATE>(b, k, dp, rigm, w, h, lr, first, std::min(dp.per, total - first)))) return rc;
        return 0;
    }
    dim3 grid((unsigned) b->cs.size());
    auto launch = [&](auto kern, int P, int T) -> int {
        if (lds_needs_attr(dp.lds)) {
            HIPCK(hipFuncSetAttribute((const void *) kern, hipFuncAttributeMaxDynamicSharedMemorySize, (int) dp.lds));
            CENSUS(LQRHIP_CENSUS_LDS_ATTR_SWEEP);
        }
        CENSUS(LQRHIP_CENSUS_SWEEP + 2 * (P == 1 ? 0 : P == 2 ? 1 : P == 4 ? 2 : P == 8 ? 3 : 4) + (T == DP_THREADS ? 1 : 0));
        CENSUS(UPDATE ? LQRHIP_CENSUS_SWEEP_UPDATE : LQRHIP_CENSUS_SWEEP_FULL);
        hipLaunchKernelGGL(kern, grid, dim3(T), dp.lds, b->stream, b->d_desc, k, w, h, c0->stride, lr);
        HIPCK(hipGetLastError());
        return 0;
    };
#define CASE(P) if (dp.px == P) { if constexpr (UPDATE) { if (dp.threads == 256) return launch(k_dp_sweep<P, true, 256>, P, 256); } return launch(k_dp_sweep<P, UPDATE, DP_THREADS>, P, DP_THREADS); }
    K_DP_SWEEP_PXT_FORMS(CASE)
#undef CASE
    g_err = "image wider than 16384 px is not supported";
    return LQRHIP_EARG;
}

extern "C" int lqrhip_mmap_build(LqrHipBatch *b, const LqrHipDpParams *p, int w, int h, int leftright)
{
    int rc;
    if ((rc = batch_upload(b))) return rc;
    if (p->delta_x > LQRHIP_MAX_DELTA) return LQRHIP_EARG;
    ProfScope ps("dp_sweep", b->stream, 9.0 * w * h * b->cs.size());
    const PlanBatch pb = plan_batch(b);
    const bool use_rig = p->use_rigidity != 0;
    return launch_dp<false>(b, make_dpk(p, b->cs[0]->ch), plan_full_dp(g_knobs, g_dev, pb, w, p->delta_x, use_rig), pb.rigm(use_rig), w, h, leftright);
}

static int frozen_catchup(LqrHipBatch *b, size_t first, size_t count, int to, int w_at_to, int h)
{
    LqrHipCarver *c0 = b->cs[first];
    const int from = c0->frozen_epoch;
    if (to <= from) return 0;
    const int w_from = fc_w_from(from, to, w_at_to);
    with_form(c0, [&](auto value) {
        hipLaunchKernelGGL(k_frozen_catchup<value>, dim3(h, (unsigned) count), dim3(256), fc_lds(from, to, w_from), b->stream, b->d_desc + first, from, to, w_from, h, c0->stride);
    });
    HIPCK(hipGetLastError());
    for (size_t i = first; i < first + count; i++) b->cs[i]->frozen_epoch = to;
    return 0;
}

static int pay_catchup(LqrHipBatch *b)
{
    LqrHipCarver *c0 = b->cs[0];
    bool any = false, alike = true;
    for (auto *c : b->cs) {
        any |= c->owed_to > 0;
        alike &= c->owed_to == c0->owed_to && c->owed_w == c0->owed_w && c->owed_h == c0->owed_h && c->frozen_epoch == c0->frozen_epoch && c->stride == c0->stride;
    }
    if (!any) return 0;
    int rc;
    if ((rc = batch_upload(b))) return rc;
    const size_t per = alike ? b->cs.size() : 1;
    for (size_t i = 0; i < b->cs.size(); i += per)
        if ((rc = frozen_catchup(b, i, per, b->cs[i]->owed_to, b->cs[i]->owed_w, b->cs[i]->owed_h))) return rc;
    for (auto *c : b->cs) drop_catchup(c);
    return 0;
}

static int launch_band_levels(LqrHipBatch *b, const DpK &k, int w, int h, int lr, int P, bool rigm)
{
    LqrHipCarver *c0 = b->cs[0];
    const size_t n = b->cs.size();
    const int ntiles = lv_tiles(w);
    if (int rc = exch_ensure(b, lv_near_off(ntiles), ntiles, (int) n, EXCH_LAYOUT_LEVELS)) return rc;
    const int epoch = lv_epoch(b->tile_epoch++);
    const dim3 grid(lv_grid(n, P));
    CENSUS(LQRHIP_CENSUS_BAND_LEVELS);
    const DpForm f = dp_form(k, lr, rigm);
#define CASE(LR, RIG, DELTA, RIGM) if (f.lr == LR && f.rig == RIG && f.delta == DELTA && f.rigm == RIGM) \
        hipLaunchKernelGGL((k_band_levels<LR, RIG, DELTA, RIGM>), grid, dim3(128), 0, b->stream, b->d_desc, k, w, h, c0->stride, b->exch.get(), epoch, g_dev_err, P, (int) n); else
    K_BAND_LEVELS_FORMS(CASE) return no_form("k_band_levels");
#undef CASE
    HIPCK(hipGetLastError());
    return 0;
}
static void inject_after_step(LqrHipBatch *b, int h, int log_index);
static void inject_after_commit(LqrHipBatch *b, int w0, int h0, int first_level);
struct StepVals {
    DpK k;
    int w, h, stride, log_index;
    int lr_pick, lr_next;
    int move_dp;
    int moved_unit;
    int epoch;
    bool value, rigm;
    unsigned n;
};
static int catchup_within_lag(LqrHipBatch *b, const StepPlan &s, StepVals &v)
{
    const int rc = s.catchup ? frozen_catchup(b, 0, b->cs.size(), v.log_index + 1, v.w - 1, v.h) : 0;
    v.epoch = b->cs[0]->frozen_epoch;
    return rc;
}
static int launch_backtrack(LqrHipBatch *b, const StepPlan &s, const StepVals &v)
{
    const int w = v.w, h = v.h, stride = v.stride, n = (int) v.n;
    if (s.backtrack == LQRHIP_CENSUS_VP_PARALLEL) {
        const size_t need = vp_map_bytes(s.vp_chunks, stride), need_path = vp_path_bytes(s.vp_chunks, stride, s.vp_rows);
        if (int rc = grow_pairs(b, [&](LqrHipCarver *c) { return c->wk.vp_map.size() >= need && c->wk.vp_path.size() >= need_path; }, [&](LqrHipCarver *c) {
                c->wk.vp_map.reset(); c->wk.vp_path.reset();
                const int rc = c->wk.vp_map.alloc(need, "&c->vp_map");
                return rc ? rc : c->wk.vp_path.alloc(need_path, "&c->vp_path");
            })) return rc;
        ProfScope ps("vpath", b->stream, 0);
        CENSUS(LQRHIP_CENSUS_VP_PARALLEL);
        if (!with_listed(K_VP_FORMS, v.k.delta, [&](auto delta) {
                hipLaunchKernelGGL(k_vp_maps<delta>, dim3(vp_col_blocks(w), s.vp_chunks, n), dim3(256), 0, b->stream, b->d_desc, w, h, stride);
                hipLaunchKernelGGL(k_vp_solve<delta>, dim3(n), dim3(VPATH_THREADS), vp_solve_lds(s.vp_chunks), b->stream, b->d_desc, w, h, stride, v.lr_pick, v.log_index, v.moved_unit);
            })) return no_form("k_vp_maps");
    } else if (!s.backtrack_beside) {
        ProfScope ps("vpath", b->stream, 0);
        CENSUS(s.backtrack);
        if (!with_listed(K_VPATH1_FORMS, v.k.delta, [&](auto delta) {
                hipLaunchKernelGGL(k_vpath1<delta>, dim3(n), dim3(VPATH_THREADS), 0, b->stream, b->d_desc, w, h, stride, v.lr_pick, v.log_index, v.moved_unit);
            }))
            hipLaunchKernelGGL(k_vpath, dim3(n), dim3(VPATH_THREADS), 0, b->stream, b->d_desc, w, h, stride, v.lr_pick, v.k.delta, v.log_index, v.moved_unit);
    }
    return 0;
}
static int launch_carve(LqrHipBatch *b, const StepPlan &s, StepVals &v)
{
    int rc;
    const int w = v.w, h = v.h, stride = v.stride, n = (int) v.n;
    const double bytes = 4.0 * (double) w * h * n;
    if (s.carve == LQRHIP_CENSUS_CARVE_E) {
        if ((rc = catchup_within_lag(b, s, v))) return rc;
        ProfScope ps("carve", b->stream, bytes);
        CENSUS(LQRHIP_CENSUS_CARVE_E);
        if (!with_listed(K_CARVE_E_FORMS, nrg_index(v.k.nrg), [&](auto nrg) {
                hipLaunchKernelGGL((k_carve_e<nrg>), dim3(bb_carve_entries(h), n), dim3(256), 0, b->stream, b->d_desc, v.k, w, h, stride, v.move_dp, v.log_index, v.epoch);
            })) return no_form("k_carve_e");
    } else if (s.backtrack_beside) {
        const size_t need = cv_list_words(n, h);
        if (b->wlist.size() < need) {
            bool grew = false;
            HIPCK(hipStreamSynchronize(b->stream));
            if ((rc = b->wlist.ensure(need, "&b->wlist", &grew))) return rc;
            HIPCK(hipMemsetAsync(b->wlist, 0, need * sizeof(unsigned long long), b->stream));
        }
        unsigned long long *moved = lqr_moved_bytes_dev();
        if (!moved) { g_err = "k_carve_v: no address for the moved-bytes counter"; return LQRHIP_EHIP; }
        const unsigned tag = bb_tag(b->wlist_launches++);
        ProfScope ps("carve", b->stream, bytes);
        CENSUS(LQRHIP_CENSUS_VPATH1);
        CENSUS(LQRHIP_CENSUS_CARVE);
        g_carve_beside_launches++;
        g_backtrack_beside_launches++;
        bool launched = false;
        with_listed(K_CARVE_U_FORMS, nrg_index(v.k.nrg), [&](auto nrg) {
            launched = with_listed(K_CARVE_V_DELTAS, v.k.delta, [&](auto delta) {
                hipLaunchKernelGGL((k_carve_v<nrg, delta>), dim3(cv_grid(n, h)), dim3(256), 0, b->stream, b->d_desc, v.k, w, h, stride, v.lr_pick, v.move_dp, v.log_index, v.epoch,
                                   (int) n, v.moved_unit, tag, b->wlist.get(), moved, g_dev_err);
            });
        });
        if (!launched) return no_form("k_carve_v");
    } else if (s.energy_beside) {
        if ((rc = catchup_within_lag(b, s, v))) return rc;
        ProfScope ps("carve", b->stream, bytes);
        CENSUS(LQRHIP_CENSUS_CARVE);
        g_carve_beside_launches++;
        if (!with_listed(K_CARVE_U_FORMS, nrg_index(v.k.nrg), [&](auto nrg) {
                hipLaunchKernelGGL((k_carve_u<nrg>), dim3(cu_grid(n, h)), dim3(256), 0, b->stream, b->d_desc, v.k, w, h, stride, v.move_dp, v.log_index, v.epoch, (int) n);
            })) return no_form("k_carve_u");
    } else {
        ProfScope ps("carve", b->stream, bytes);
        CENSUS(LQRHIP_CENSUS_CARVE);
        hipLaunchKernelGGL(k_carve, dim3(bb_carve_entries(h), n), dim3(256), 0, b->stream, b->d_desc, w, h, stride, v.k.delta, v.move_dp);
    }
    return 0;
}
static int launch_energy(LqrHipBatch *b, const StepPlan &s, StepVals &v)
{
    if (s.carve == LQRHIP_CENSUS_CARVE_E || s.energy_beside) return 0;
    ProfScope ps("emap_update", b->stream, 0);
    if (int rc = catchup_within_lag(b, s, v)) return rc;
    const int h = v.h, stride = v.stride, wnew = v.w - 1, log_index = v.log_index, epoch = v.epoch, n = (int) v.n;
    const DpK &k = v.k;
    const bool value = v.value;
    const int nrg = plane_nrg(value, nrg_index(k.nrg)), nt = s.eu_nt;
#define CASE_NT(NT, N, V) if (nrg == N && value == V && nt == NT) hipLaunchKernelGGL((k_emap_update<N, NT, V>), dim3(bb_energy_entries(h), n), dim3(64), 0, b->stream, b->d_desc, k, wnew, h, stride, log_index, epoch); else
#define CASE(N, V) K_EMAP_UPDATE_NT_FORMS(CASE_NT, N, V)
    K_EMAP_FORMS(CASE) return no_form("k_emap_update");
#undef CASE
#undef CASE_NT
    return 0;
}
static int launch_band(LqrHipBatch *b, const StepPlan &s, const StepVals &v)
{
    const int h = v.h, stride = v.stride, wnew = v.w - 1, leftright_next = v.lr_next, n = (int) v.n;
    const DpK &k = v.k;
    if (s.band == LQRHIP_CENSUS_BAND_LEVELS) {
        ProfScope ps("band_levels", b->stream, 0);
        if (int rc = launch_band_levels(b, k, wnew, h, leftright_next, s.levels_P, v.rigm)) return rc;
    } else if (s.band == LQRHIP_CENSUS_BAND_TW) {
        ProfScope ps("band_update", b->stream, 0);
        CENSUS(LQRHIP_CENSUS_BAND_TW);
#define CASE(LRV, RIGV) if ((leftright_next != 0) == LRV && (k.use_rig != 0) == RIGV) hipLaunchKernelGGL((k_band_update_tw<4, LRV, RIGV>), dim3(n), dim3(128 * 4), band_tw_lds(h), b->stream, b->d_desc, k, wnew, h, stride, g_dev_err); else
        K_LR_RIG_FORMS(CASE) return no_form("k_band_update_tw");
#undef CASE
    } else if (s.band == LQRHIP_CENSUS_BAND_MW8 || s.band == LQRHIP_CENSUS_BAND_MW16) {
        ProfScope ps("band_update", b->stream, 0);
        const int nw = s.band == LQRHIP_CENSUS_BAND_MW16 ? 16 : 8;
        CENSUS(nw == 16 ? LQRHIP_CENSUS_BAND_MW16 : LQRHIP_CENSUS_BAND_MW8);
#define CASE_NW(NWV, LRV, RIGV) if (nw == NWV && (leftright_next != 0) == LRV && (k.use_rig != 0) == RIGV) hipLaunchKernelGGL((k_band_update_mw<2, NWV, 8, LRV, RIGV>), dim3(n), dim3(64 * NWV), band_mw_lds(h), b->stream, b->d_desc, k, wnew, h, stride); else
#define CASE(LRV, RIGV) CASE_NW(8, LRV, RIGV) CASE_NW(16, LRV, RIGV)
        K_LR_RIG_FORMS(CASE) return no_form("k_band_update_mw");
#undef CASE
#undef CASE_NW
    } else {
        ProfScope ps("band_update", b->stream, 0);
        CENSUS(LQRHIP_CENSUS_BAND_GENERIC);
        hipLaunchKernelGGL(k_band_update, dim3(n), dim3(64), 0, b->stream, b->d_desc, k, wnew, h, stride, leftright_next);
    }
    ProfScope ps("dp_update", b->stream, 0);
    return launch_dp<true>(b, k, s.dp, v.rigm, wnew, h, leftright_next);
}

static int seam_step_impl(LqrHipBatch *b, const LqrHipDpParams *p, int w, int h, int log_index, int leftright_pick,
                          int full_rebuild, int leftright_next)
{
    int rc;
    LqrHipCarver *c0 = b->cs[0];
    for (auto *c : b->cs)
        if (log_index >= c->log_cap || c->owed_to) return LQRHIP_EARG;
    if ((rc = batch_upload(b))) return rc;
    const PlanBatch pb = plan_batch(b);
    const StepPlan s = plan_seam_step(g_knobs, g_dev, pb, p->delta_x, p->use_rigidity != 0, w, h, full_rebuild != 0, log_index + 1 - c0->frozen_epoch);
    const int wnew = w - 1, move_dp = (wnew > 1 && !full_rebuild) ? 1 : 0;
    const int moved_unit = 2 * (4 + (move_dp ? 5 : 0) + (pb.rigmask ? 4 : 0));
    StepVals v{make_dpk(p, c0->ch), w, h, c0->stride, log_index, leftright_pick, leftright_next, move_dp, moved_unit, c0->frozen_epoch,
               pb.value, pb.rigm(p->use_rigidity != 0), (unsigned) b->cs.size()};
    if ((rc = launch_backtrack(b, s, v)) || (rc = launch_carve(b, s, v))) return rc;
    if (s.dp.form < 0) { HIPCK(hipGetLastError()); return 0; }
    if ((rc = launch_energy(b, s, v))) return rc;
    if (s.full || s.band < 0) {
        ProfScope ps(s.full ? "dp_sweep" : "dp_update_tiled", b->stream, s.full ? 9.0 * wnew * h * v.n : 0);
        rc = s.full ? launch_dp<false>(b, v.k, s.dp, v.rigm, wnew, h, leftright_next) : launch_dp<true>(b, v.k, s.dp, v.rigm, wnew, h, leftright_next);
    } else rc = launch_band(b, s, v);
    if (rc) return rc;
    HIPCK(hipGetLastError());
    return 0;
}

extern "C" int lqrhip_seam_step(LqrHipBatch *b, const LqrHipDpParams *p, int w, int h, int log_index, int leftright_pick,
                                int full_rebuild, int leftright_next)
{
    const int rc = seam_step_impl(b, p, w, h, log_index, leftright_pick, full_rebuild, leftright_next);
    if (rc == 0) inject_after_step(b, h, log_index);
    static const char *dump = getenv("LQRHIP_DUMP");
    if (rc == 0 && dump) {
        static int call = 0;
        LqrHipCarver *c = b->cs[0];
        HIPCK(hipStreamSynchronize(b->stream));
        const size_t np = (size_t) c->stride * h;
        std::vector<int> hdr = {w, h, c->stride, log_index, FLAG_COUNT}, flags(FLAG_COUNT), seam(h);
        std::vector<float> m(np);
        std::vector<int8_t> least(np);
        HIPCK(hipMemcpy(flags.data(), c->wk.flags, FLAG_COUNT * sizeof(int), hipMemcpyDeviceToHost));
        HIPCK(hipMemcpy(seam.data(), c->wk.seam_x, (size_t) h * sizeof(int), hipMemcpyDeviceToHost));
        HIPCK(hipMemcpy(m.data(), c->wk.m, np * sizeof(float), hipMemcpyDeviceToHost));
        HIPCK(hipMemcpy(least.data(), c->wk.least, np, hipMemcpyDeviceToHost));
        char path[512];
        snprintf(path, sizeof path, "%s_%04d.bin", dump, call++);
        if (FILE *f = fopen(path, "wb")) {
            fwrite(hdr.data(), sizeof(int), hdr.size(), f); fwrite(flags.data(), sizeof(int), flags.size(), f);
            fwrite(seam.data(), sizeof(int), seam.size(), f); fwrite(m.data(), sizeof(float), np, f); fwrite(least.data(), 1, np, f);
            fclose(f);
        }
    }
    return rc;
}

extern "C" int lqrhip_seam_log_reserve(LqrHipBatch *b, int n_seams, int h)
{
    int rc;
    if ((rc = pay_catchup(b))) return rc;
    for (auto *c : b->cs) if ((rc = ensure_log(c, n_seams, h))) return rc;
    return 0;
}

extern "C" int lqrhip_vs_commit(LqrHipBatch *b, int w0, int h0, int wc0, int n_seams, int first_level, int finish)
{
    int rc;
    if ((rc = batch_upload(b))) return rc;
    size_t lds = vsc_lds(n_seams, wc0);
    if (lds > VSC_LDS_MAX) { g_err = "vs_commit: session too large for LDS"; return LQRHIP_EARG; }
    if (lds_needs_attr(lds)) {
        HIPCK(hipFuncSetAttribute((const void *) k_vs_commit, hipFuncAttributeMaxDynamicSharedMemorySize, (int) lds));
        CENSUS(LQRHIP_CENSUS_LDS_ATTR_COMMIT);
    }
    hipLaunchKernelGGL(k_vs_commit, dim3(h0, (unsigned) b->cs.size()), dim3(256), lds, b->stream, b->d_desc, w0, h0, wc0, n_seams,
                       first_level, finish);
    HIPCK(hipGetLastError());
    inject_after_commit(b, w0, h0, first_level);
    for (auto *c : b->cs) {
        if (c->frozen_epoch < n_seams) { c->owed_to = n_seams; c->owed_w = wc0 - n_seams; c->owed_h = h0; }
        else drop_catchup(c);
    }
    return 0;
}

static int g_selfcheck = 1, g_recovery = 1;
extern "C" void lqrhip_set_selfcheck(int on) { g_selfcheck = on != 0; }
extern "C" void lqrhip_set_recovery(int on) { g_recovery = on != 0; }
extern "C" int lqrhip_get_recovery(void) { return g_recovery; }
extern "C" int lqrhip_session_check(LqrHipBatch *b, int h, int wc0, int n_seams, int delta_x)
{
    int rc;
    if (!g_selfcheck || n_seams < 1) return 0;
    if ((rc = batch_upload(b))) return rc;
    hipLaunchKernelGGL(k_seam_check, dim3(tiles_of(h, 256), (unsigned) b->cs.size()), dim3(256), 0, b->stream, b->d_desc, h, wc0, n_seams, delta_x, g_dev_err);
    HIPCK(hipGetLastError());
    return 0;
}
extern "C" int lqrhip_session_rollback(LqrHipBatch *b, int w0, int h0, int first_level, int finish)
{
    (void) hipStreamSynchronize(b->stream);
    b->pending_inflate.reset();
    (void) hipGetLastError();
    if (g_dev_err_host) *g_dev_err_host = 0;
    invalidate_all_batches();
    int rc;
    if ((rc = batch_upload(b))) return rc;
    const size_t n = (size_t) w0 * h0;
    hipLaunchKernelGGL(k_vs_rollback, dim3((unsigned) std::min<size_t>(blocks_of(n, 256), 4096), (unsigned) b->cs.size()), dim3(256), 0, b->stream, b->d_desc, n, first_level, finish ? w0 : 0);
    HIPCK(hipGetLastError());
    HIPCK(hipStreamSynchronize(b->stream));
    for (auto *c : b->cs) drop_catchup(c);
    g_fault_stats[4]++;
    return 0;
}
static int g_inject_kind = 0, g_inject_step = 0, g_inject_times = 0;
extern "C" void lqrhip_debug_inject(int kind, int at_step, int times) { g_inject_kind = kind; g_inject_step = at_step; g_inject_times = kind ? std::max(times, 1) : 0; }
static void inject_after_step(LqrHipBatch *b, int h, int log_index)
{
    if (g_inject_times <= 0 || log_index != g_inject_step) return;
    if (g_inject_kind == 1 || g_inject_kind == 2) { *g_dev_err_host = g_inject_kind == 1 ? DEVERR_TILE_TIMEOUT : DEVERR_BAND_PREDICTION; }
    else if (g_inject_kind == 3 || g_inject_kind == 4) hipLaunchKernelGGL(k_inject, dim3(1), dim3(64), 0, b->stream, b->d_desc, g_inject_kind - 3, h, 0, log_index, 0);
    else return;
    g_inject_times--; g_fault_stats[5]++;
}
static void inject_after_commit(LqrHipBatch *b, int w0, int h0, int first_level)
{
    if (g_inject_times <= 0 || (g_inject_kind != 5 && g_inject_kind != 6)) return;
    if (g_inject_step > 0) { g_inject_step--; return; }
    hipLaunchKernelGGL(k_inject, dim3(1), dim3(64), 0, b->stream, b->d_desc, g_inject_kind - 3, h0, w0, 0, first_level);
    g_inject_times--; g_fault_stats[5]++;
}

namespace {
struct Staging {
    LqrHipBatch *b;
    bool keep = false;
    Staging(LqrHipBatch *batch, int kind, int w1, int h1) : b(batch)
    {
        b->pending_inflate.reset(new PendingInflate());
        b->pending_inflate->kind = kind; b->pending_inflate->w1 = w1; b->pending_inflate->h1 = h1;
    }
    ~Staging() { if (!keep) { lqr_stream_wait(b->stream); b->pending_inflate.reset(); } }
    PlaneJobs &jobs() const { return b->pending_inflate->pj; }
    int kept() { keep = true; return 0; }
};
}
static int inflate_stage(LqrHipBatch *b, int w0, int h0, int l, int max_level, const int32_t *levels)
{
    int rc;
    const int w1 = w0 + l - max_level + 1;
    Staging st(b, 0, w1, h0);
    PlaneJobs &pj = st.jobs();
    for (auto *c : b->cs) {
        pj.new_vs.emplace_back();
        DevBuf<int32_t> &nvs = pj.new_vs.back();
        if ((rc = nvs.alloc((size_t) w1 * h0, "&nvs"))) return rc;
        const int32_t *vs = levels ? levels : c->vs.get();
        for (auto *a : c->aux)
            if ((rc = pj.add(a, vs, nullptr, (size_t) w1 * h0))) return rc;
        if ((rc = pj.add(c, vs, nvs, (size_t) w1 * h0))) return rc;
    }
    if ((rc = pj.stage(b->stream, false))) return rc;
    const size_t lds = inflate_lds(l, max_level);
    if (pj.n_narrow)
        hipLaunchKernelGGL(k_inflate<false>, dim3(h0, (unsigned) pj.n_narrow), dim3(256), lds, b->stream, pj.d_dev.get(), w0, w1, l, max_level, g_selfcheck ? g_dev_err : (int *) nullptr);
    if (pj.n_wide())
        hipLaunchKernelGGL(k_inflate<true>, dim3(h0, (unsigned) pj.n_wide()), dim3(256), lds, b->stream, pj.d_wide(), w0, w1, l, max_level, g_selfcheck ? g_dev_err : (int *) nullptr);
    HIPCK(hipGetLastError());
    HIPCK(hipStreamSynchronize(b->stream));
    if ((rc = check_dev_error())) return rc;
    return st.kept();
}
extern "C" int lqrhip_inflate(LqrHipBatch *b, int w0, int h0, int l, int max_level) { return inflate_stage(b, w0, h0, l, max_level, nullptr); }

struct __attribute__((visibility("hidden"))) LqrHipVMap {
    DevBuf<int32_t> own;
    const int32_t *plane = nullptr;
    int len = 0, lines = 0, depth = 0;
};
extern "C" int lqrhip_vmap_stage(const int *map, int on_device, int width, int height, int depth, int orientation, LqrHipVMap **out)
{
    *out = nullptr;
    if (lqrhip_init() < 0) return LQRHIP_EHIP;
    const int len = orientation ? height : width, lines = orientation ? width : height;
    if (!map || width < 1 || height < 1 || (orientation != 0 && orientation != 1) || depth < 1 || depth >= len || depth >= LQRHIP_MAX_FRAME_WIDTH) {
        g_err = "vmap: depth, size or orientation out of range";
        return LQRHIP_EARG;
    }
    int rc;
    const size_t n = (size_t) width * height;
    std::unique_ptr<LqrHipVMap> m(new LqrHipVMap());
    m->len = len; m->lines = lines; m->depth = depth;
    Scratch tmp(g_stream0);
    const int32_t *src = (const int32_t *) map;
    if (!on_device) {
        int32_t *d = orientation ? tmp.get<int32_t>(n, "&vmap_raw", rc) : ((rc = m->own.alloc(n, "&vmap")) ? nullptr : m->own.get());
        if (rc) return rc;
        if ((rc = h2d_staged(d, map, n * sizeof(int32_t)))) return rc;
        src = d;
    }
    if (orientation) {
        if ((rc = m->own.alloc(n, "&vmap_t"))) return rc;
        const size_t lds = vmap_check_t_lds(depth);
        if (vmap_t_needs_attr(lds)) HIPCK(hipFuncSetAttribute((const void *) k_vmap_check_t, hipFuncAttributeMaxDynamicSharedMemorySize, (int) lds));
        hipLaunchKernelGGL(k_vmap_check_t, dim3(vmap_t_blocks(width)), dim3(256), lds, g_stream0, src, m->own.get(), width, height, depth, g_dev_err);
        m->plane = m->own;
    } else {
        hipLaunchKernelGGL(k_vmap_check, dim3(height), dim3(256), vmap_check_lds(depth), g_stream0, src, width, depth, g_dev_err);
        m->plane = src;
    }
    HIPCK(hipGetLastError());
    HIPCK(hipStreamSynchronize(g_stream0));
    tmp.done();
    if (g_dev_err_host && *g_dev_err_host == DEVERR_VMAP) {
        *g_dev_err_host = 0;
        g_err = "vmap: a value outside [0, depth], or a level that is missing or occurs twice in a line";
        return LQRHIP_EMAP;
    }
    if ((rc = check_dev_error())) return rc;
    *out = m.release();
    return 0;
}
extern "C" void lqrhip_vmap_release(LqrHipVMap *m) { delete m; }
extern "C" int lqrhip_vmap_load(LqrHipBatch *b, const LqrHipVMap *m)
{
    if (!m || !m->plane) return LQRHIP_EARG;
    for (auto *c : b->cs)
        if (c->w0 != m->len || c->h0 != m->lines) { g_err = "vmap: the carver's frame is not the map's"; return LQRHIP_EARG; }
    return inflate_stage(b, m->len, m->lines, m->depth, 1, m->plane);
}
extern "C" int lqrhip_planes_commit(LqrHipBatch *b)
{
    PendingInflate *pi = b->pending_inflate.get();
    if (!pi) return LQRHIP_EARG;
    PlaneJobs &pj = pi->pj;
    commit(pj);
    for (auto &j : pj.jobs) { j.c->w0 = pi->w1; j.c->h0 = pi->h1; }
    if (pi->kind != 0)
        for (auto *c : b->cs) drop_catchup(c);
    if (pi->kind != 2) {
        size_t i = 0;
        for (auto *c : b->cs) c->vs = std::move(pj.new_vs[i++]);
    }
    b->dirty = true;
    b->pending_inflate.reset();
    return 0;
}
extern "C" int lqrhip_inflate_commit(LqrHipBatch *b) { return lqrhip_planes_commit(b); }

extern "C" int lqrhip_flatten(LqrHipBatch *b, int w0, int h0, int w, int level)
{
    int rc;
    Staging st(b, 1, w, h0);
    PlaneJobs &pj = st.jobs();
    for (auto *c : b->cs) {
        pj.new_vs.emplace_back();
        DevBuf<int32_t> &nvs = pj.new_vs.back();
        if ((rc = nvs.alloc((size_t) w * h0, "&nvs"))) return rc;
        HIPCK(hipMemsetAsync(nvs, 0, (size_t) w * h0 * sizeof(int32_t), b->stream));
        for (auto *a : c->aux)
            if ((rc = pj.add(a, c->vs, nullptr, (size_t) w * h0))) return rc;
        if ((rc = pj.add(c, c->vs, nullptr, (size_t) w * h0))) return rc;
    }
    if ((rc = pj.stage(b->stream, true))) return rc;
    if (pj.n_narrow)
        hipLaunchKernelGGL(k_compact_jobs<false>, dim3(h0, (unsigned) pj.n_narrow), dim3(256), 0, b->stream, pj.d_dev.get(), w0, w, level);
    if (pj.n_wide())
        hipLaunchKernelGGL(k_compact_jobs<true>, dim3(h0, (unsigned) pj.n_wide()), dim3(256), 0, b->stream, pj.d_wide(), w0, w, level);
    HIPCK(hipGetLastError());
    HIPCK(hipStreamSynchronize(b->stream));
    return st.kept();
}

extern "C" int lqrhip_transpose(LqrHipBatch *b, int w, int h)
{
    int rc;
    Staging st(b, 2, h, w);
    PlaneJobs &pj = st.jobs();
    for (auto *c : b->cs) {
// ... 770 lines not shown
```

include/lqr_hip.h:

```cpp
#ifndef LQR_HIP_H
#define LQR_HIP_H

#include <stddef.h>

#ifdef __cplusplus
extern "C" {
#endif

#define LQRHIP_OK 0
#define LQRHIP_ENOMEM (-2)
#define LQRHIP_EHIP (-1)
#define LQRHIP_EARG (-3)
#define LQRHIP_EFAULT (-4)
#define LQRHIP_EMAP (-5)
#define LQRHIP_MAX_DELTA 16
#define LQRHIP_MAX_CHANNELS 64
#define LQRHIP_MAX_FRAME_WIDTH 16384

typedef struct LqrHipCarver LqrHipCarver;
typedef struct LqrHipBatch LqrHipBatch;

typedef struct LqrHipDpParams {
    int delta_x;
    int use_rigidity;
    float rigidity_map[2 * LQRHIP_MAX_DELTA + 1];
    int nrg_func;
    int nrg_radius;
    int w_start;
} LqrHipDpParams;

int lqrhip_init(void);
const char *lqrhip_last_error(void);

LqrHipCarver *lqrhip_carver_create(const unsigned char *rgb, int w, int h, int channels);
LqrHipCarver *lqrhip_carver_create_ext(const void *rgb, int w, int h, int channels, int depth);
int lqrhip_carver_set_read_luma(LqrHipCarver *c, int luma);
int lqrhip_carver_set_read(LqrHipCarver *c, int image_type, int alpha, int black);
void lqrhip_carver_destroy(LqrHipCarver *c);
int lqrhip_carver_reset(LqrHipCarver *c, const void *device_rgb, int w, int h);
int lqrhip_carver_reset_batch(LqrHipCarver **cs, const void *const *device_rgb, int n, int w, int h);
int lqrhip_carver_reset_batch_count(void);
int lqrhip_reset_sync(void);
int lqrhip_carver_attach(LqrHipCarver *root, LqrHipCarver *aux);
int lqrhip_carver_activate(LqrHipCarver *c);

int lqrhip_mask_add(LqrHipCarver *c, const unsigned char *mask, int channels, int width, int height,
                    int x_off, int y_off, int transposed, int is_rigmask, int bias_factor);

int lqrhip_mask_add_f(LqrHipCarver *c, const void *mask, int depth, int on_device, int width, int height, int x_off, int y_off,
                      int transposed, int is_rigmask, int bias_factor);
int lqrhip_mask_plane_ensure(LqrHipCarver *c, int is_rigmask);
int lqrhip_mask_scatter(LqrHipCarver *c, int is_rigmask, const int *index, const double *value, const size_t *start, int buckets);
int lqrhip_mask_clear(LqrHipCarver *c, int is_rigmask);
int lqrhip_read_mask_plane(LqrHipCarver *c, int is_rigmask, int transposed, float *out);
unsigned long long lqrhip_debug_mask_flushes(void);

int lqrhip_sub_batches(int n);
int lqrhip_general_batch_limit(int w);
int lqrhip_general_batch_limit_delta(int w, int delta_x);
void lqrhip_set_sub_batches(int n);
LqrHipBatch *lqrhip_batch_create(LqrHipCarver **carvers, int n);
void lqrhip_batch_set_shared(LqrHipBatch *b, int shared);
void lqrhip_batch_destroy(LqrHipBatch *b);
int lqrhip_batch_sync(LqrHipBatch *b);
void lqrhip_batch_abort(LqrHipBatch *b);
void *lqrhip_batch_stream(LqrHipBatch *b);

int lqrhip_wk_init(LqrHipBatch *b, int from_visible);
int lqrhip_emap_build(LqrHipBatch *b, const LqrHipDpParams *p, int w, int h);
int lqrhip_wk_init_emap(LqrHipBatch *b, const LqrHipDpParams *p, int w, int h);
int lqrhip_energy_out(LqrHipBatch *b, int w, int h, int transposed, int form, int depth, int image_type, void *out, int on_device);
int lqrhip_mmap_build(LqrHipBatch *b, const LqrHipDpParams *p, int w, int h, int leftright);
int lqrhip_seam_step(LqrHipBatch *b, const LqrHipDpParams *p, int w, int h, int log_index,
                     int leftright_pick, int full_rebuild, int leftright_next);
int lqrhip_seam_log_reserve(LqrHipBatch *b, int n_seams, int h);
int lqrhip_vs_commit(LqrHipBatch *b, int w0, int h0, int wc0, int n_seams, int first_level, int finish);
int lqrhip_session_check(LqrHipBatch *b, int h, int wc0, int n_seams, int delta_x);
void lqrhip_set_selfcheck(int on);
void lqrhip_set_recovery(int on);
int lqrhip_get_recovery(void);
int lqrhip_session_rollback(LqrHipBatch *b, int w0, int h0, int first_level, int finish);
void lqrhip_batch_set_safe(LqrHipBatch *b, int safe);
void lqrhip_set_no_spin(int on);
int lqrhip_get_no_spin(void);
int lqrhip_fault_stats(unsigned long long *out8, int reset);
void lqrhip_debug_inject(int kind, int at_step, int times);
void lqrhip_debug_fail_alloc(int nth);
unsigned long long lqrhip_debug_pool_live(void);
void lqrhip_debug_fixedcost(unsigned long long out4[4], int reset);
int lqrhip_inflate(LqrHipBatch *b, int w0, int h0, int l, int max_level);
typedef struct LqrHipVMap LqrHipVMap;
int lqrhip_vmap_stage(const int *map, int on_device, int width, int height, int depth, int orientation, LqrHipVMap **out);
int lqrhip_vmap_load(LqrHipBatch *b, const LqrHipVMap *m);
void lqrhip_vmap_release(LqrHipVMap *m);
int lqrhip_flatten(LqrHipBatch *b, int w0, int h0, int w, int level);
int lqrhip_transpose(LqrHipBatch *b, int w, int h);
int lqrhip_planes_commit(LqrHipBatch *b);
int lqrhip_inflate_commit(LqrHipBatch *b);

int lqrhip_read_visible(LqrHipCarver *c, int w0, int h0, int w, int level, unsigned char *out);
int lqrhip_mask_line_max(const unsigned char *mask, int channels, int width, int height, int a0, int b0, int n_lines, int line_len,
                         int direction);
int lqrhip_read_visible_device(LqrHipCarver *c, int w0, int h0, int w, int level, void *device_out);
int lqrhip_read_sizes(LqrHipCarver *c, int w0, int h0, int transposed, const int *levels, int n, void *const *outs, int on_device);
#define LQRHIP_FORWARD_MAX_LINES 65535
typedef struct LqrHipForward LqrHipForward;
int lqrhip_forward_begin(LqrHipCarver *const *cs, int n, int depth, int orientation, int transposed, int luma, int w_start,
                         void *const *device_maps, LqrHipForward **out);
int lqrhip_forward_seams(LqrHipForward *f, int first_seam, int n_seams);
int lqrhip_forward_finish(LqrHipForward *f);
const int *lqrhip_forward_map(const LqrHipForward *f, int i);
int lqrhip_forward_read_map(LqrHipForward *f, int i, int *out);
void lqrhip_forward_release(LqrHipForward *f);
unsigned long long lqrhip_forward_launches(int reset);
int lqrhip_forward_intensity(LqrHipCarver *c, int orientation, int transposed, int luma, float *out);
int lqrhip_read_forward_intensity(const void *carver, int orientation, float *out);
#define LQRHIP_STATIC_MAX_FRAMES 65535
typedef struct LqrHipStatic LqrHipStatic;
int lqrhip_static_begin(LqrHipCarver *const *cs, int n, int orientation, int transposed, int nrg_func, float alpha, void *device_energy,
                        LqrHipStatic **out);
int lqrhip_static_groups(const LqrHipStatic *st);
int lqrhip_static_fold(LqrHipStatic *st);
int lqrhip_static_finish(LqrHipStatic *st, float *host_energy);
const float *lqrhip_static_energy(const LqrHipStatic *st);
void lqrhip_static_release(LqrHipStatic *st);
typedef struct LqrHipClipFwd LqrHipClipFwd;
int lqrhip_clipfwd_begin(LqrHipCarver *const *cs, int n, int depth, int orientation, int transposed, int luma, int w_start, float temporal,
                         void *device_map, LqrHipClipFwd **out);
int lqrhip_clipfwd_seams(LqrHipClipFwd *f, int first_seam, int n_seams);
int lqrhip_clipfwd_finish(LqrHipClipFwd *f);
const int *lqrhip_clipfwd_map(const LqrHipClipFwd *f);
int lqrhip_clipfwd_read_map(LqrHipClipFwd *f, int *out);
void lqrhip_clipfwd_release(LqrHipClipFwd *f);
unsigned long long lqrhip_clipfwd_launches(int reset);
double lqrhip_clipfwd_fold_ms(void);
int lqrhip_device_sync(void);
int lqrhip_mem_info(unsigned long long *free_bytes, unsigned long long *total_bytes, unsigned long long *cached_bytes);
int lqrhip_copy_bandwidth(unsigned long long bytes, int iters, double *gbps);
int lqrhip_vmap_to_rgba(const int *vmap, int w, int h, int depth, const double col_start[3], const double col_end[3],
                        unsigned char *out_rgba);
void lqrhip_pool_trim(void);
int lqrhip_read_vmap(LqrHipCarver *c, int w0, int h0, int w, int level, int depth, int *out);
int lqrhip_read_working(LqrHipCarver *c, int w, int h, float *en, float *m, int *least_dx);
int lqrhip_read_seam_flags(LqrHipCarver *c, int *org, int *org_prev, int *side);
int lqrhip_debug_seam_flags(const void *carver, int *org, int *org_prev, int *side);

void lqrhip_prof_enable(int on);
void lqrhip_set_update_mode(int mode);
void lqrhip_set_sweep_threads(int n);
void lqrhip_set_carve_fused(int max_images);
void lqrhip_set_carve_beside(int mode);
unsigned long long lqrhip_carve_beside_launches(int reset);
void lqrhip_set_backtrack_beside(int mode);
unsigned long long lqrhip_backtrack_beside_launches(int reset);
void lqrhip_set_vpath_mode(int mode, int par_max);
void lqrhip_set_dp_persistent_limit(int workgroups);
void lqrhip_set_dp_persistent_px(int px);
void lqrhip_prof_reset(void);
int lqrhip_prof_get(const char *kernel, double *ms_total, long long *launches, double *bytes_total);
int lqrhip_prof_get_union(const char *kernel, double *ms_union);
int lqrhip_moved_bytes(unsigned long long *bytes, int reset);
void lqrhip_set_band_levels(int slots);
int lqrhip_band_levels_stats(unsigned long long *out8, int reset);
enum {
    LQRHIP_CENSUS_VP_PARALLEL = 0,
    LQRHIP_CENSUS_VPATH1 = 1,
    LQRHIP_CENSUS_VPATH = 2,
    LQRHIP_CENSUS_CARVE_E = 3,
    LQRHIP_CENSUS_CARVE = 4,
    LQRHIP_CENSUS_TILE_P_G3 = 5,
    LQRHIP_CENSUS_TILE_P_G2 = 6,
    LQRHIP_CENSUS_TILE_P_G4 = 7,
    LQRHIP_CENSUS_TILE_P_GENERAL = 8,
    LQRHIP_CENSUS_DP_TILE = 9,
    LQRHIP_CENSUS_BAND_LEVELS = 10,
    LQRHIP_CENSUS_BAND_TW = 11,
    LQRHIP_CENSUS_BAND_MW8 = 12,
    LQRHIP_CENSUS_BAND_MW16 = 13,
    LQRHIP_CENSUS_BAND_GENERIC = 14,
    LQRHIP_CENSUS_SWEEP = 15,
    LQRHIP_CENSUS_SWEEP_FULL = 25,
    LQRHIP_CENSUS_SWEEP_UPDATE = 26,
    LQRHIP_CENSUS_LDS_ATTR_SWEEP = 27,
    LQRHIP_CENSUS_LDS_ATTR_COMMIT = 28,
    LQRHIP_CENSUS_COMPACT_SIZES = 29,
    LQRHIP_CENSUS_TRANSPOSE_SIZES = 30,
    LQRHIP_CENSUS_STATIC_FOLD = 31,
    LQRHIP_CENSUS_SLOTS = 32
};
int lqrhip_launch_census(unsigned long long *out, int n, int reset);

#ifdef __cplusplus
}
#endif
#endif
```

Measured before the change: 535,900 Mseams*px/s.

## Add paired-slot band-levels kernel packing two slots per 256-thread workgroup

Adds a k_band_levels2 variant that runs two level-pipeline slots inside one 256-thread workgroup for the delta=1, non-general, spin case. The planner picks it when the grid would otherwise exceed the CU count, so fewer workgroups are resident. Shared helpers move into a new header, and occupancy is queried separately for the new kernel. The aim is to cut cross-workgroup flag polling and improve residency, at the cost of a second kernel form and more complex selection logic.

```diff
diff --git a/gimp-lqr-plugin_amd/csrc/k_levels.hip b/gimp-lqr-plugin_amd/csrc/k_levels.hip
--- a/gimp-lqr-plugin_amd/csrc/k_levels.hip
+++ b/gimp-lqr-plugin_amd/csrc/k_levels.hip
@@ -1,414 +1,43 @@
 #include "lqr_common.h"
 #include "lqr_kernels.h"
+#include "lqr_levels.h"
 
 __device__ unsigned long long g_lv_stats[8];
 #ifdef LQR_TIMING
 __device__ unsigned long long g_lv_time[16][2][10];
-#define LTT(i) do { __builtin_amdgcn_sched_barrier(0); const unsigned long long t__ = __builtin_readcyclecounter(); __builtin_amdgcn_sched_barrier(0); ltt[i] += t__ - ltprev; ltprev = t__; } while (0)
 extern "C" int lqrhip_band_levels_timing(unsigned long long *out) { (void) hipDeviceSynchronize(); return hipMemcpyFromSymbol(out, HIP_SYMBOL(g_lv_time), sizeof(unsigned long long) * 320) == hipSuccess ? 0 : -1; }
-#else
-#define LTT(i) do { } while (0)
 #endif
 __device__ int g_lv_dbg;
 
-#ifdef LQR_JITTER
-#define LJIT(site) do { if (dbg & 16) { unsigned h__ = (unsigned) (slot * 131 + L * 17 + (site) * 7 + epoch * 2654435761u + q * 40503u + image * 977u); h__ ^= h__ >> 13; h__ *= 0x5bd1e995u; h__ ^= h__ >> 15; \
-    for (unsigned i__ = h__ & 15u; i__ > 0; i__--) __builtin_amdgcn_s_sleep(127); } } while (0)
-#else
-#define LJIT(site) do { } while (0)
-#endif
-__device__ __forceinline__ unsigned long long uni64(unsigned long long v)
-{
-    return ((unsigned long long) (unsigned) __builtin_amdgcn_readfirstlane((int) (v >> 32)) << 32) | (unsigned) __builtin_amdgcn_readfirstlane((int) v);
-}
-struct LvMask {
-    unsigned long long lo;
-    __device__ __forceinline__ void set(int t) { lo |= 1ull << t; }
-    __device__ __forceinline__ bool has(int t) const { return t >= 0 && t < LV_MAX_TILES && ((lo >> t) & 1ull); }
-    __device__ __forceinline__ void set_range(int a, int b) { lo |= ((b - a >= 63) ? ~0ull : ((1ull << (b - a + 1)) - 1ull)) << a; }
-    __device__ __forceinline__ int first() const { return lo ? __builtin_ctzll(lo) : -1; }
-    __device__ __forceinline__ int last() const { return lo ? 63 - __builtin_clzll(lo) : -1; }
-};
 
 template <bool LR, bool RIG, int DELTA, bool RIGM>
 __global__ __launch_bounds__(128) __attribute__((amdgpu_waves_per_eu(2, 2)))
 void k_band_levels(DevCarver *cs, DpK p, int w, int h, int stride, unsigned long long *exch, int epoch, int *dev_err, int P, int n_img)
 {
-    static_assert(DELTA >= 1 && DELTA <= LQR_FAST_MAX_DELTA && (DELTA <= 4 || RIG) && (RIG || !RIGM), "delta_x 1 .. 10 (5 .. 10: the rigidity form, with a zero table if there is none); a rigidity mask only matters with rigidity");
-    constexpr int PX = 2, HALO = 32, OWN = LV_OWN, HL = 16, R = lv_rows(DELTA, RIGM), TILE = 128;
-    static_assert(R * DELTA <= HALO, "a level's errors stay inside the halo");
-    typedef LaneVec<2>::F FV;
-    typedef LaneVec<2>::L LV;
-    typedef GLOBAL_AS FV GFV;
-    typedef GLOBAL_AS LV GLV;
-    typedef GLOBAL_AS unsigned long long gu64;
-    __shared__ int s_tlo[LV_MAX_LEVELS], s_thi[LV_MAX_LEVELS];
-    __shared__ int s_fail;
-    __shared__ int s_polled;
-    __shared__ unsigned long long s_A[2];
-        const int tid = threadIdx.x, lane = tid & 63;
-    const int q = __builtin_amdgcn_readfirstlane(tid >> 6);
-    const int dbg = __builtin_amdgcn_readfirstlane(g_lv_dbg);
-    const int b_xcd = (int) blockIdx.x & 7, b_k = (int) blockIdx.x >> 3;
-    const int slot = (dbg & 8) ? (int) blockIdx.x % P : b_k % P, image = (dbg & 8) ? (int) blockIdx.x / P : (b_k / P) * 8 + b_xcd;
-    if (image >= n_img) return;
-    const int nblk = (h + R - 1) / R;
-    const int ntiles = lv_tiles(w);
-    GCarver c = gview(cs[image]);
-    if constexpr (RIG && DELTA == 1 && !RIGM) { c.en = uni_ptr(c.en); c.m = uni_ptr(c.m); c.least = uni_ptr(c.least); }
-    const size_t near_off = lv_near_off(ntiles);
-    gu64 *ex_img = (gu64 *) exch + exch_image_off(image, near_off);
-    gu64 *flagw = ex_img;
-    gu64 *gran = ex_img + LV_FLAG_WORDS;
-    const float INF = __int_as_float(0x7f800000);
-    const float rig_l = p.rigmap[0], rig_r = p.rigmap[2];
-    float rg[2 * DELTA + 1];
-#pragma unroll
-    for (int i = 0; i < 2 * DELTA + 1; i++) rg[i] = p.rigmap[i];
-    const int ix_own = 2 * (lane % P), ix_right = 2 * ((lane + 1) % P), ix_left = 2 * ((lane + P - 1) % P);
-
-    for (int i = tid; i < nblk; i += 128) { s_tlo[i] = 1 << 30; s_thi[i] = -1; }
-    if (tid == 0) { s_fail = 0; s_polled = -1; }
-    __syncthreads();
-    for (int y = tid; y < h; y += 128) {
-        const int v0 = c.seam_x[y], vm = c.seam_x[max(y - 1, 0)], vp = c.seam_x[min(y + 1, h - 1)];
-        const int t0 = max(min(min(v0, vm), vp) - DELTA - 1, 0), t1 = min(max(max(v0, vm), vp) + DELTA, w - 1);
-        atomicMin(&s_tlo[y / R], t0); atomicMax(&s_thi[y / R], t1);
-    }
-    __syncthreads();
-    __shared__ unsigned long long s_tm[LV_MAX_LEVELS + 2];
-    for (int L = tid; L < nblk + 2; L += 128) {
-        unsigned long long m = 0ull;
-        if (L < nblk && s_thi[L] >= s_tlo[L]) {
-            const int a = max(0, (s_tlo[L] - (OWN - 1 + HALO + 2) + OWN - 1) / OWN), b = min(ntiles - 1, (s_thi[L] + HALO + 2) / OWN);
-            m = ((b - a >= 63) ? ~0ull : ((1ull << (b - a + 1)) - 1ull)) << a;
-        }
-        s_tm[L] = m;
-    }
-    __syncthreads();
-    auto touch_mask = [&](int L) -> LvMask {
-        LvMask m;
-        m.lo = uni64(s_tm[L]);
-        return m;
-    };
-    unsigned long long res_mine = 0ull;
-    for (int t = slot; t < LV_MAX_TILES; t += P) res_mine |= 1ull << t;
-    res_mine = uni64(res_mine);
-    auto my_tile = [&](const LvMask &A, int which) -> int {
-        unsigned long long m = A.lo & res_mine;
-        if (which && m) m &= m - 1ull;
-        return m ? __builtin_ctzll(m) : -1;
-    };
-    auto any_collision = [&](const LvMask &A) -> bool {
-        const int a = A.first(), b = A.last();
-        if (a < 0 || b - a < 2 * P) return false;
-        unsigned long long res_zero = 0ull;
-        for (int t = 0; t < LV_MAX_TILES; t += P) res_zero |= 1ull << t;
-        for (int r = 0; r < P; r++)
-            if (__popcll(A.lo & (res_zero << r)) > 2) return true;
-        return false;
-    };
-    auto nearest_tile = [&](int a, int b) -> int {
-        const unsigned long long up_m = res_mine & (~0ull << a), dn_m = res_mine & (b >= 63 ? ~0ull : ((1ull << (b + 1)) - 1ull));
-        const int up = up_m ? __builtin_ctzll(up_m) : -1, dn = dn_m ? 63 - __builtin_clzll(dn_m) : -1;
-        if (up >= 0 && up <= b) return up;
-        if (up < 0 || up >= ntiles) return dn;
-        if (dn < 0) return up;
-        return (up - b <= a - dn) ? up : dn;
-    };
-
-    int cur_t = -1, cur_L = -1;
-    bool cur_full = false;
-    int x0 = 0;
-    unsigned lo_off = 0;
-    constexpr bool LEAN = RIG && DELTA == 1 && !RIGM;
-    bool in[PX] = {false, false}, own = false, interior = false;
-    const bool own_lane = lane >= HL && lane < 64 - HL;
-    auto X0 = [&]() -> int { int v = x0; asm volatile("" : "+v"(v)); return v; };
-    auto in_k = [&](int k) -> bool { if constexpr (LEAN) return (unsigned) (X0() + k) < (unsigned) w; else return in[k]; };
-    auto is_own = [&]() -> bool { if constexpr (LEAN) return own_lane && X0() < w; else return own; };
-    auto is_interior = [&]() -> bool {
-        if constexpr (LEAN) { const int t0 = __builtin_amdgcn_readfirstlane(X0()); return t0 >= 0 && t0 + TILE <= w; }
-        else return interior;
-    };
-    auto set_tile = [&](int t) {
-        x0 = t * OWN - HALO + PX * lane;
-        lo_off = (unsigned) min(max(x0, 0), stride - PX);
-        if constexpr (!LEAN) {
-#pragma unroll
-            for (int k = 0; k < PX; k++) in[k] = x0 + k >= 0 && x0 + k < w;
-            own = own_lane && x0 < w;
-            interior = (x0 - PX * lane >= 0) && (x0 - PX * lane + TILE <= w);
-        }
-    };
-    auto owner_of = [&](int t) -> int { return lane < HL ? t - 1 : lane >= 64 - HL ? t + 1 : t; };
-    const int owner_col = lane < HL ? HALO + PX * lane : lane >= 64 - HL ? PX * (lane - (64 - HL)) : PX * (lane - HL);
-    FV q_e[R], q_mo[R], q_ab, q_rf[RIGM ? R : 1];
-    LV q_lo[R];
-    q_ab[0] = q_ab[1] = INF;
-    auto issue_full = [&](int L) {
-        const int ybase = L * R;
-#pragma unroll
-        for (int r = 0; r < R; r++) {
-            const unsigned row = (unsigned) min(ybase + r, h - 1) * (unsigned) stride;
-            const unsigned ro = row + lo_off, ro4 = (row << 2) + (lo_off << 2);
-            q_e[r] = *(const GFV *) ((const gu8 *) c.en + ro4);
-            q_mo[r] = *(const GFV *) ((const gu8 *) c.m + ro4);
-            q_lo[r] = *(const GLV *) (c.least + ro);
-            if (RIGM) q_rf[RIGM ? r : 0] = *(const GFV *) ((const gu8 *) c.rig + ro4);
-        }
-        q_ab = *(const GFV *) ((const gu8 *) c.m + ((((unsigned) max(ybase - 1, 0) * (unsigned) stride) + lo_off) << 2));
-    };
-    float mp[PX] = {INF, INF};
-    int acc_l0 = 0, acc_l1 = 0;
-    auto batch_u = [&](int ybase) {
-        const int nr = min(R, h - ybase);
-#pragma unroll
-        for (int r = 0; r < R; r++) {
-            float mc[PX], e[PX], mo[PX];
-            uint32_t lnew = 0;
-            bool ch[PX];
-#pragma unroll
-            for (int k = 0; k < PX; k++) { e[k] = q_e[r][k]; mo[k] = q_mo[r][k]; }
-            if constexpr (DELTA == 1 && !RIGM) {
-                const float left = __int_as_float(__builtin_amdgcn_mov_dpp(__float_as_int(mp[PX - 1]), DPP_WAVE_SHR1, 0xf, 0xf, true));
-                const float right = __int_as_float(__builtin_amdgcn_mov_dpp(__float_as_int(mp[0]), DPP_WAVE_SHL1, 0xf, 0xf, true));
-                dp_row<PX, LR, RIG, true, false>(mp, left, right, e, mo, (uint32_t) q_lo[r], in, rig_l, rig_r, mc, lnew, ch);
-            } else {
-                float nl[DELTA], nr[DELTA], rf[PX];
-                lane_reach<PX, DELTA>(mp, nl, nr);
-#pragma unroll
-                for (int k = 0; k < PX; k++) rf[k] = RIGM ? q_rf[RIGM ? r : 0][k] : 1.0f;
-                dp_row_g<PX, DELTA, LR, RIG, RIGM, true, false>(mp, nl, nr, e, mo, (uint32_t) q_lo[r], in, rg, rf, mc, lnew, ch);
-            }
-            if (r == 0 && ybase == 0) {
-#pragma unroll
-                for (int k = 0; k < PX; k++) mc[k] = e[k];
-                lnew = 0;
-            }
-            if (r == R - 1) {
-                const int msk = (r < nr) ? -1 : 0;
-                acc_l0 = (__float_as_int(mc[0]) ^ __float_as_int(mo[0])) & msk;
-                acc_l1 = (__float_as_int(mc[1]) ^ __float_as_int(mo[1])) & msk;
-            }
-#pragma unroll
-            for (int k = 0; k < PX; k++) { mp[k] = mc[k]; q_mo[r][k] = mc[k]; }
-            q_lo[r] = (LV) lnew;
-        }
-    };
-    auto store_u = [&](int ybase) {
-        const bool own_ = is_own();
-        const unsigned inc = own_ ? (unsigned) stride : 0u, inc4 = inc * 4u;
-        unsigned so = own_ ? (unsigned) ybase * (unsigned) stride + (unsigned) x0 : (unsigned) h * (unsigned) stride + (unsigned) (PX * lane), so4 = so * 4u;
-        const int nr = min(R, h - ybase);
-#pragma unroll
-        for (int r = 0; r < R; r++, so += inc, so4 += inc4) {
-            if (r < nr) {
-                *(GFV *) ((gu8 *) c.m + so4) = q_mo[r];
-                *(GLV *) (c.least + so) = q_lo[r];
-            }
-        }
-    };
-    auto wait_level = [&](int L, int spec_t, const LvMask &prev, unsigned long long &fw, unsigned long long (&g)[PX]) -> int {
-        const unsigned want = ((unsigned) epoch << 10) | (unsigned) L;
-        gu64 *fsrc = flagw + (size_t) ((L - 1) & 1) * 2 * LV_PMAX + (lane < 2 * P ? lane : 0);
-        const bool need_g = spec_t >= 0 && prev.has(owner_of(spec_t)) && (in_k(0) || in_k(1));
-        gu64 *gsrc = gran + ((size_t) ((L - 1) & 1) * ntiles + (need_g ? owner_of(spec_t) : 0)) * OWN + (need_g ? owner_col : 0);
-        int sp = 0;
-        while (true) {
-            const size_t off = (!(dbg & 4) && (sp & 3) != 3) ? near_off : 0;
-            fw = __hip_atomic_load(fsrc + off, __ATOMIC_RELAXED, __HIP_MEMORY_SCOPE_AGENT);
-            if (spec_t >= 0) {
-#pragma unroll
-                for (int k = 0; k < PX; k++) g[k] = __hip_atomic_load(gsrc + off + k, __ATOMIC_RELAXED, __HIP_MEMORY_SCOPE_AGENT);
-            }
-            const bool okf = __all(lane >= 2 * P || (unsigned) (fw >> 32) == want);
-            bool okg = true;
-#pragma unroll
-            for (int k = 0; k < PX; k++) okg &= (unsigned) (g[k] >> 32) == want;
-            if (okf && __all(!need_g || okg)) return 0;
-            if (dbg & 2) __builtin_amdgcn_s_sleep(16); else if (okf || sp < 8) __builtin_amdgcn_s_sleep(1); else if (sp < 64) __builtin_amdgcn_s_sleep(8); else __builtin_amdgcn_s_sleep(48);
-            ++sp;
-            if ((sp & 255) == 0 && dev_failed(dev_err)) return 1;
-            if (sp > (1 << 18)) { if (lane == 0) dev_fail(dev_err, DEVERR_TILE_TIMEOUT); return 1; }
-        }
-    };
-    auto row_above = [&](int L, int t, const LvMask &prev, bool have_g, unsigned long long (&g)[PX]) -> int {
-        const int u = owner_of(t);
-        const bool from_gran = prev.has(u) && (in_k(0) || in_k(1));
-        if (!have_g) {
-            gu64 *src = gran + ((size_t) ((L - 1) & 1) * ntiles + (from_gran ? u : 0)) * OWN + (from_gran ? owner_col : 0);
-            const unsigned want = ((unsigned) epoch << 10) | (unsigned) L;
-            int sp = 0;
-            while (true) {
-                const size_t off = (!(dbg & 4) && (sp & 3) != 3) ? near_off : 0;
-#pragma unroll
-                for (int k = 0; k < PX; k++) g[k] = __hip_atomic_load(src + off + k, __ATOMIC_RELAXED, __HIP_MEMORY_SCOPE_AGENT);
-                bool ok = true;
-#pragma unroll
-                for (int k = 0; k < PX; k++) ok &= (unsigned) (g[k] >> 32) == want;
-                if (__all(ok || !from_gran)) break;
-                __builtin_amdgcn_s_sleep(1);
-                if (++sp > (1 << 16)) { if (lane == 0) dev_fail(dev_err, DEVERR_TILE_TIMEOUT); return 1; }
-            }
-        }
-#pragma unroll
-        for (int k = 0; k < PX; k++) mp[k] = !in_k(k) ? INF : from_gran ? __uint_as_float((unsigned) g[k]) : q_ab[k];
-        return 0;
-    };
-    unsigned n_proc = 0, n_idle = 0, n_sync = 0, n_two = 0;
-    int hold_L = -1;
-#ifdef LQR_TIMING
-    unsigned long long ltt[10] = {0, 0, 0, 0, 0, 0, 0, 0, 0, 0};
-    unsigned long long ltprev = __builtin_readcyclecounter();
-    const unsigned long long ltstart = ltprev;
-#endif
-    for (int L = 0; L <= nblk; L++) {
-        const bool mine = (L & 1) == q;
-        int t = -1;
-        bool have_g = false, passed = false;
-        unsigned long long g[PX] = {0ull, 0ull};
-        LvMask A = {0ull}, A_prev = {0ull};
-        if (L > 0) A_prev.lo = uni64(s_A[(L - 1) & 1]);
-        LTT(8);
-        if (mine) {
-            unsigned long long fw = 0;
-            A = touch_mask(L);
-            passed = true;
-            if (L > 0) {
-                const int spec_t = (hold_L < 0 && cur_full && cur_L == L && L < nblk && !(dbg & 1)) ? cur_t : -1;
-                LJIT(1);
-                const int wl_rc = wait_level(L, spec_t, A_prev, fw, g);
-                LJIT(2);
-                LTT(0);
-                if (wl_rc) { LDS_FLAG(s_fail) = 1; passed = false; }
-                else if (L < nblk) {
-                    const int wl = (int) (unsigned) fw;
-                    bool act = false;
-                    unsigned wo[2], wr[2], wlf[2];
-#pragma unroll
-                    for (int i = 0; i < 2; i++) {
-                        wo[i] = (unsigned) __builtin_amdgcn_ds_bpermute((ix_own + i) << 2, wl);
-                        wr[i] = (unsigned) __builtin_amdgcn_ds_bpermute((ix_right + i) << 2, wl);
-                        wlf[i] = (unsigned) __builtin_amdgcn_ds_bpermute((ix_left + i) << 2, wl);
-                    }
-#pragma unroll
-                    for (int i = 0; i < 2; i++) {
-                        act |= (wo[i] & 0x900u) == 0x900u && (int) (wo[i] & 0xffu) == lane;
-                        act |= (wr[i] & 0xa00u) == 0xa00u && (int) (wr[i] & 0xffu) == lane + 1;
-                        act |= (wlf[i] & 0xc00u) == 0xc00u && (int) (wlf[i] & 0xffu) == lane - 1;
-                    }
-                    A.lo |= __ballot(act && lane < ntiles);
-                    have_g = spec_t >= 0;
-                }
-            }
-            if (lane == 0) { s_A[L & 1] = A.lo; if (passed) LDS_FLAG(s_polled) = L; }
-        } else {
-            int spins = 0;
-            while (LDS_FLAG(s_polled) < L && LDS_FLAG(s_fail) != 1 && ++spins < (1 << 24)) __builtin_amdgcn_s_sleep(1);
-            passed = LDS_FLAG(s_polled) >= L;
-            if (passed) A.lo = uni64(s_A[L & 1]);
-            else if (LDS_FLAG(s_fail) != 1) { LDS_FLAG(s_fail) = 1; if (lane == 0) dev_fail(dev_err, DEVERR_TILE_TIMEOUT); }
-            LTT(2);
-        }
-        LTT(1);
-        LJIT(3);
-        if (hold_L >= 0 && passed) { store_u(hold_L * R); hold_L = -1; }
-        LTT(3);
-        if (L == nblk) break;
-        if (mine && passed && any_collision(A)) {
-            if (slot == 0 && lane == 0) { __hip_atomic_fetch_min(c.flags + FLAG_OVF_ROW, L * R, __ATOMIC_RELAXED, __HIP_MEMORY_SCOPE_AGENT); atomicAdd(&g_lv_stats[0], 1ull); }
-            LDS_FLAG(s_fail) = 2;
-            passed = false;
-        }
-        if (passed) t = my_tile(A, mine ? 0 : 1);
-        if (!mine && t < 0 && passed && lane == 0) {
-            const unsigned long long tag = (unsigned long long) (((unsigned) epoch << 10) | (unsigned) (L + 1)) << 32;
-            gu64 *fdst = flagw + (size_t) (L & 1) * 2 * LV_PMAX + 2 * slot + 1;
-            if (!(dbg & 4)) __hip_atomic_store(fdst + near_off, tag, __ATOMIC_RELAXED, __HIP_MEMORY_SCOPE_WORKGROUP);
-            __hip_atomic_store(fdst, tag, __ATOMIC_RELAXED, __HIP_MEMORY_SCOPE_AGENT);
-        }
-        {
-            int ld_t = -1, ld_L = L;
-            if (t >= 0) {
-                if (!(cur_full && cur_t == t && cur_L == L)) { ld_t = t; n_sync++; have_g = false; }
-                if (!mine) n_two++;
-            } else if (!mine && passed && L + 1 < nblk) {
-                LvMask M = touch_mask(L + 1);
-                M.lo |= A.lo;
-                int pt = my_tile(M, 0);
-                if (pt < 0 && M.first() >= 0) { pt = nearest_tile(M.first(), M.last()); if (pt < M.first() - 1 || pt > M.last() + 1 || pt >= ntiles) pt = -1; }
-                ld_t = pt; ld_L = L + 1;
-                cur_t = -1; cur_L = ld_L; cur_full = false;
-            }
-            LTT(1);
-            LJIT(4);
-            if (ld_t >= 0) { set_tile(ld_t); issue_full(ld_L); cur_t = ld_t; cur_L = ld_L; cur_full = true; }
-#ifdef LQR_TIMING
-            if (t >= 0 && ld_t >= 0) asm volatile("s_waitcnt vmcnt(0)" ::: "memory");
-#endif
-            LTT(4);
-        }
-        unsigned word = 0;
-        if (t >= 0) {
-            n_proc++;
-            if (L > 0 && row_above(L, t, A_prev, have_g, g)) LDS_FLAG(s_fail) = 1;
-#ifdef LQR_TIMING
-            asm volatile("s_waitcnt vmcnt(0)" ::: "memory");
-#endif
-            LTT(5);
-            if (!is_interior()) {
-                const bool ik[PX] = {in_k(0), in_k(1)};
-#pragma unroll
-                for (int r = 0; r < R; r++)
-#pragma unroll
-                    for (int k = 0; k < PX; k++) { q_e[r][k] = ik[k] ? q_e[r][k] : INF; q_mo[r][k] = ik[k] ? q_mo[r][k] : INF; }
-            }
-            batch_u(L * R);
-            LTT(6);
-            hold_L = L;
-            cur_full = false;
-            LJIT(5);
-            if (L + 1 < nblk && own_lane) {
-                gu64 *dst = gran + ((size_t) (L & 1) * ntiles + t) * OWN + PX * (lane - HL);
-                const unsigned long long tag = (unsigned long long) (((unsigned) epoch << 10) | (unsigned) (L + 1)) << 32;
-#pragma unroll
-                for (int k = 0; k < PX; k++) {
-                    if (!(dbg & 4)) __hip_atomic_store(dst + near_off + k, tag | __float_as_uint(mp[k]), __ATOMIC_RELAXED, __HIP_MEMORY_SCOPE_WORKGROUP);
-                    __hip_atomic_store(dst + k, tag | __float_as_uint(mp[k]), __ATOMIC_RELAXED, __HIP_MEMORY_SCOPE_AGENT);
-                }
-            }
-            const bool chg = own_lane && (acc_l0 | acc_l1) != 0;
-            const bool any_o = __any(chg), any_l = __any(chg && lane < 32), any_r = __any(chg && lane >= 32);
-            word = 0x800u | (any_o ? 0x100u : 0u) | (any_l ? 0x200u : 0u) | (any_r ? 0x400u : 0u) | (unsigned) t;
-        } else if (mine && passed) n_idle++;
-        LJIT(6);
-        if (lane == 0 && (t >= 0 || mine) && LDS_FLAG(s_fail) == 0) {
-            const unsigned long long tag = (unsigned long long) (((unsigned) epoch << 10) | (unsigned) (L + 1)) << 32;
-            gu64 *fdst = flagw + (size_t) (L & 1) * 2 * LV_PMAX + 2 * slot + (mine ? 0 : 1);
-            if (!(dbg & 4)) __hip_atomic_store(fdst + near_off, tag | word, __ATOMIC_RELAXED, __HIP_MEMORY_SCOPE_WORKGROUP);
-            __hip_atomic_store(fdst, tag | word, __ATOMIC_RELAXED, __HIP_MEMORY_SCOPE_AGENT);
-        }
-        LTT(7);
-        asm volatile("s_waitcnt lgkmcnt(0)\n\ts_barrier" ::: "memory");
-        LTT(8);
-        if (LDS_FLAG(s_fail)) return;
-    }
-#ifdef LQR_TIMING
-    if (image == 0 && lane == 0 && slot < 16) { ltt[9] = __builtin_readcyclecounter() - ltstart; for (int i = 0; i < 10; i++) g_lv_time[slot][q][i] = ltt[i]; }
-#endif
-    if (lane == 0) { atomicAdd(&g_lv_stats[2], (unsigned long long) n_proc); atomicAdd(&g_lv_stats[3], (unsigned long long) n_idle); if (n_two) atomicAdd(&g_lv_stats[4], (unsigned long long) n_two); }
-    if (lane == 0 && n_sync) atomicAdd(&g_lv_stats[1], (unsigned long long) n_sync);
+#define LV_NT 128
+#define LV_SLOT_STATE __shared__ int s_polled; __shared__ unsigned long long s_A[2];
+#define LV_POLLED s_polled
+#define LV_A s_A
+#define LV_WAVE const int q = __builtin_amdgcn_readfirstlane(tid >> 6);
+#define LV_BLOCK const int b_xcd = (int) blockIdx.x & 7, b_k = (int) blockIdx.x >> 3; const int slot = (dbg & 8) ? (int) blockIdx.x % P : b_k % P, image = (dbg & 8) ? (int) blockIdx.x / P : (b_k / P) * 8 + b_xcd;
+#define LV_INIT_FLAGS if (tid == 0) { s_fail = 0; s_polled = -1; }
+#define LV_AFTER_SETUP
+#define LV_LEVEL_END asm volatile("s_waitcnt lgkmcnt(0)\n\ts_barrier" ::: "memory");
+#define LV_DBG g_lv_dbg
+#define LV_STATS g_lv_stats
+#define LV_TIME g_lv_time
+#include "k_levels_body.inc"
+#include "k_levels_undef.inc"
 }
 
-extern "C" void lqrhip_band_levels_debug(int v) { if (lqrhip_init() < 0) return; (void) hipMemcpyToSymbol(HIP_SYMBOL(g_lv_dbg), &v, sizeof v); }
+extern "C" void lqrhip_band_levels_debug(int v) { if (lqrhip_init() < 0) return; (void) hipMemcpyToSymbol(HIP_SYMBOL(g_lv_dbg), &v, sizeof v); lqr_levels2_debug(v); }
 extern "C" int lqrhip_band_levels_stats(unsigned long long *out, int reset)
 {
     if (lqrhip_init() < 0) return -1;
     (void) hipDeviceSynchronize();
     if (hipMemcpyFromSymbol(out, HIP_SYMBOL(g_lv_stats), sizeof(unsigned long long) * 8) != hipSuccess) return -1;
     if (reset) { unsigned long long z[8] = {0}; (void) hipMemcpyToSymbol(HIP_SYMBOL(g_lv_stats), z, sizeof z); }
-    return 0;
+    return lqr_levels2_stats(out, reset);
 }
 
 #define INST(...) template __global__ void k_band_levels<__VA_ARGS__>(DevCarver *, DpK, int, int, int, unsigned long long *, int, int *, int, int);
diff --git a/gimp-lqr-plugin_amd/csrc/k_levels2.hip b/gimp-lqr-plugin_amd/csrc/k_levels2.hip
--- /dev/null
+++ b/gimp-lqr-plugin_amd/csrc/k_levels2.hip
@@ -0,0 +1,47 @@
+#include "lqr_common.h"
+#include "lqr_kernels.h"
+#include "lqr_levels.h"
+
+__device__ unsigned long long g_lv2_stats[8];
+#ifdef LQR_TIMING
+__device__ unsigned long long g_lv2_time[16][2][10];
+extern "C" int lqrhip_band_levels2_timing(unsigned long long *out) { (void) hipDeviceSynchronize(); return hipMemcpyFromSymbol(out, HIP_SYMBOL(g_lv2_time), sizeof(unsigned long long) * 320) == hipSuccess ? 0 : -1; }
+#endif
+__device__ int g_lv2_dbg;
+
+template <bool LR, bool RIG>
+__global__ __launch_bounds__(256) __attribute__((amdgpu_waves_per_eu(2, 2)))
+void k_band_levels2(DevCarver *cs, DpK p, int w, int h, int stride, unsigned long long *exch, int epoch, int *dev_err, int P, int n_img)
+{
+    constexpr int DELTA = 1;
+    constexpr bool RIGM = false;
+#define LV_NT 256
+#define LV_SLOT_STATE __shared__ int s_polled2[2]; __shared__ unsigned long long s_A2[2][2];
+#define LV_POLLED s_polled2[pr]
+#define LV_A s_A2[pr]
+#define LV_WAVE const int q = __builtin_amdgcn_readfirstlane((tid >> 6) & 1), pr = __builtin_amdgcn_readfirstlane(tid >> 7);
+#define LV_BLOCK const int b_xcd = (int) blockIdx.x & 7, b_k = (int) blockIdx.x >> 3; const int P2 = (P + 1) >> 1, s0 = (dbg & 8) ? (int) blockIdx.x % P2 : b_k % P2, slot = (dbg & 32) ? 2 * s0 + pr : s0 + pr * P2, \
+                           image = (dbg & 8) ? (int) blockIdx.x / P2 : (b_k / P2) * 8 + b_xcd;
+#define LV_INIT_FLAGS if (tid == 0) s_fail = 0; if ((tid & 127) == 0) LV_POLLED = -1;
+#define LV_AFTER_SETUP if (slot >= P) return;
+#define LV_LEVEL_END asm volatile("s_waitcnt lgkmcnt(0)\n\ts_barrier" ::: "memory");
+#define LV_DBG g_lv2_dbg
+#define LV_STATS g_lv2_stats
+#define LV_TIME g_lv2_time
+#include "k_levels_body.inc"
+#include "k_levels_undef.inc"
+}
+
+void lqr_levels2_debug(int v) { (void) hipMemcpyToSymbol(HIP_SYMBOL(g_lv2_dbg), &v, sizeof v); }
+int lqr_levels2_stats(unsigned long long *out, int reset)
+{
+    unsigned long long mine[8];
+    if (hipMemcpyFromSymbol(mine, HIP_SYMBOL(g_lv2_stats), sizeof mine) != hipSuccess) return -1;
+    for (int i = 0; i < 8; i++) out[i] += mine[i];
+    if (reset) { unsigned long long z[8] = {0}; (void) hipMemcpyToSymbol(HIP_SYMBOL(g_lv2_stats), z, sizeof z); }
+    return 0;
+}
+
+#define INST(...) template __global__ void k_band_levels2<__VA_ARGS__>(DevCarver *, DpK, int, int, int, unsigned long long *, int, int *, int, int);
+K_BAND_LEVELS2_FORMS(INST)
+#undef INST
diff --git a/gimp-lqr-plugin_amd/csrc/k_levels_body.inc b/gimp-lqr-plugin_amd/csrc/k_levels_body.inc
--- /dev/null
+++ b/gimp-lqr-plugin_amd/csrc/k_levels_body.inc
@@ -0,0 +1,364 @@
+    static_assert(DELTA >= 1 && DELTA <= LQR_FAST_MAX_DELTA && (DELTA <= 4 || RIG) && (RIG || !RIGM), "delta_x 1 .. 10 (5 .. 10: the rigidity form, with a zero table if there is none); a rigidity mask only matters with rigidity");
+    constexpr int PX = 2, HALO = 32, OWN = LV_OWN, HL = 16, R = lv_rows(DELTA, RIGM), TILE = 128;
+    static_assert(R * DELTA <= HALO, "a level's errors stay inside the halo");
+    typedef LaneVec<2>::F FV;
+    typedef LaneVec<2>::L LV;
+    typedef GLOBAL_AS FV GFV;
+    typedef GLOBAL_AS LV GLV;
+    typedef GLOBAL_AS unsigned long long gu64;
+    __shared__ int s_tlo[LV_MAX_LEVELS], s_thi[LV_MAX_LEVELS];
+    __shared__ int s_fail;
+    LV_SLOT_STATE
+        const int tid = threadIdx.x, lane = tid & 63;
+    LV_WAVE
+    const int dbg = __builtin_amdgcn_readfirstlane(LV_DBG);
+    LV_BLOCK
+    if (image >= n_img) return;
+    const int nblk = (h + R - 1) / R;
+    const int ntiles = lv_tiles(w);
+    GCarver c = gview(cs[image]);
+    if constexpr (RIG && DELTA == 1 && !RIGM) { c.en = uni_ptr(c.en); c.m = uni_ptr(c.m); c.least = uni_ptr(c.least); }
+    const size_t near_off = lv_near_off(ntiles);
+    gu64 *ex_img = (gu64 *) exch + exch_image_off(image, near_off);
+    gu64 *flagw = ex_img;
+    gu64 *gran = ex_img + LV_FLAG_WORDS;
+    const float INF = __int_as_float(0x7f800000);
+    const float rig_l = p.rigmap[0], rig_r = p.rigmap[2];
+    float rg[2 * DELTA + 1];
+#pragma unroll
+    for (int i = 0; i < 2 * DELTA + 1; i++) rg[i] = p.rigmap[i];
+    const int ix_own = 2 * (lane % P), ix_right = 2 * ((lane + 1) % P), ix_left = 2 * ((lane + P - 1) % P);
+
+    for (int i = tid; i < nblk; i += LV_NT) { s_tlo[i] = 1 << 30; s_thi[i] = -1; }
+    LV_INIT_FLAGS
+    __syncthreads();
+    for (int y = tid; y < h; y += LV_NT) {
+        const int v0 = c.seam_x[y], vm = c.seam_x[max(y - 1, 0)], vp = c.seam_x[min(y + 1, h - 1)];
+        const int t0 = max(min(min(v0, vm), vp) - DELTA - 1, 0), t1 = min(max(max(v0, vm), vp) + DELTA, w - 1);
+        atomicMin(&s_tlo[y / R], t0); atomicMax(&s_thi[y / R], t1);
+    }
+    __syncthreads();
+    __shared__ unsigned long long s_tm[LV_MAX_LEVELS + 2];
+    for (int L = tid; L < nblk + 2; L += LV_NT) {
+        unsigned long long m = 0ull;
+        if (L < nblk && s_thi[L] >= s_tlo[L]) {
+            const int a = max(0, (s_tlo[L] - (OWN - 1 + HALO + 2) + OWN - 1) / OWN), b = min(ntiles - 1, (s_thi[L] + HALO + 2) / OWN);
+            m = ((b - a >= 63) ? ~0ull : ((1ull << (b - a + 1)) - 1ull)) << a;
+        }
+        s_tm[L] = m;
+    }
+    __syncthreads();
+    LV_AFTER_SETUP
+    auto touch_mask = [&](int L) -> LvMask {
+        LvMask m;
+        m.lo = uni64(s_tm[L]);
+        return m;
+    };
+    unsigned long long res_mine = 0ull;
+    for (int t = slot; t < LV_MAX_TILES; t += P) res_mine |= 1ull << t;
+    res_mine = uni64(res_mine);
+    auto my_tile = [&](const LvMask &A, int which) -> int {
+        unsigned long long m = A.lo & res_mine;
+        if (which && m) m &= m - 1ull;
+        return m ? __builtin_ctzll(m) : -1;
+    };
+    auto any_collision = [&](const LvMask &A) -> bool {
+        const int a = A.first(), b = A.last();
+        if (a < 0 || b - a < 2 * P) return false;
+        unsigned long long res_zero = 0ull;
+        for (int t = 0; t < LV_MAX_TILES; t += P) res_zero |= 1ull << t;
+        for (int r = 0; r < P; r++)
+            if (__popcll(A.lo & (res_zero << r)) > 2) return true;
+        return false;
+    };
+    auto nearest_tile = [&](int a, int b) -> int {
+        const unsigned long long up_m = res_mine & (~0ull << a), dn_m = res_mine & (b >= 63 ? ~0ull : ((1ull << (b + 1)) - 1ull));
+        const int up = up_m ? __builtin_ctzll(up_m) : -1, dn = dn_m ? 63 - __builtin_clzll(dn_m) : -1;
+        if (up >= 0 && up <= b) return up;
+        if (up < 0 || up >= ntiles) return dn;
+        if (dn < 0) return up;
+        return (up - b <= a - dn) ? up : dn;
+    };
+
+    int cur_t = -1, cur_L = -1;
+    bool cur_full = false;
+    int x0 = 0;
+    unsigned lo_off = 0;
+    constexpr bool LEAN = RIG && DELTA == 1 && !RIGM;
+    bool in[PX] = {false, false}, own = false, interior = false;
+    const bool own_lane = lane >= HL && lane < 64 - HL;
+    auto X0 = [&]() -> int { int v = x0; asm volatile("" : "+v"(v)); return v; };
+    auto in_k = [&](int k) -> bool { if constexpr (LEAN) return (unsigned) (X0() + k) < (unsigned) w; else return in[k]; };
+    auto is_own = [&]() -> bool { if constexpr (LEAN) return own_lane && X0() < w; else return own; };
+    auto is_interior = [&]() -> bool {
+        if constexpr (LEAN) { const int t0 = __builtin_amdgcn_readfirstlane(X0()); return t0 >= 0 && t0 + TILE <= w; }
+        else return interior;
+    };
+    auto set_tile = [&](int t) {
+        x0 = t * OWN - HALO + PX * lane;
+        lo_off = (unsigned) min(max(x0, 0), stride - PX);
+        if constexpr (!LEAN) {
+#pragma unroll
+            for (int k = 0; k < PX; k++) in[k] = x0 + k >= 0 && x0 + k < w;
+            own = own_lane && x0 < w;
+            interior = (x0 - PX * lane >= 0) && (x0 - PX * lane + TILE <= w);
+        }
+    };
+    auto owner_of = [&](int t) -> int { return lane < HL ? t - 1 : lane >= 64 - HL ? t + 1 : t; };
+    const int owner_col = lane < HL ? HALO + PX * lane : lane >= 64 - HL ? PX * (lane - (64 - HL)) : PX * (lane - HL);
+    FV q_e[R], q_mo[R], q_ab, q_rf[RIGM ? R : 1];
+    LV q_lo[R];
+    q_ab[0] = q_ab[1] = INF;
+    auto issue_full = [&](int L) {
+        const int ybase = L * R;
+#pragma unroll
+        for (int r = 0; r < R; r++) {
+            const unsigned row = (unsigned) min(ybase + r, h - 1) * (unsigned) stride;
+            const unsigned ro = row + lo_off, ro4 = (row << 2) + (lo_off << 2);
+            q_e[r] = *(const GFV *) ((const gu8 *) c.en + ro4);
+            q_mo[r] = *(const GFV *) ((const gu8 *) c.m + ro4);
+            q_lo[r] = *(const GLV *) (c.least + ro);
+            if (RIGM) q_rf[RIGM ? r : 0] = *(const GFV *) ((const gu8 *) c.rig + ro4);
+        }
+        q_ab = *(const GFV *) ((const gu8 *) c.m + ((((unsigned) max(ybase - 1, 0) * (unsigned) stride) + lo_off) << 2));
+    };
+    float mp[PX] = {INF, INF};
+    int acc_l0 = 0, acc_l1 = 0;
+    auto batch_u = [&](int ybase) {
+        const int nr = min(R, h - ybase);
+#pragma unroll
+        for (int r = 0; r < R; r++) {
+            float mc[PX], e[PX], mo[PX];
+            uint32_t lnew = 0;
+            bool ch[PX];
+#pragma unroll
+            for (int k = 0; k < PX; k++) { e[k] = q_e[r][k]; mo[k] = q_mo[r][k]; }
+            if constexpr (DELTA == 1 && !RIGM) {
+                const float left = __int_as_float(__builtin_amdgcn_mov_dpp(__float_as_int(mp[PX - 1]), DPP_WAVE_SHR1, 0xf, 0xf, true));
+                const float right = __int_as_float(__builtin_amdgcn_mov_dpp(__float_as_int(mp[0]), DPP_WAVE_SHL1, 0xf, 0xf, true));
+                dp_row<PX, LR, RIG, true, false>(mp, left, right, e, mo, (uint32_t) q_lo[r], in, rig_l, rig_r, mc, lnew, ch);
+            } else {
+                float nl[DELTA], nr[DELTA], rf[PX];
+                lane_reach<PX, DELTA>(mp, nl, nr);
+#pragma unroll
+                for (int k = 0; k < PX; k++) rf[k] = RIGM ? q_rf[RIGM ? r : 0][k] : 1.0f;
+                dp_row_g<PX, DELTA, LR, RIG, RIGM, true, false>(mp, nl, nr, e, mo, (uint32_t) q_lo[r], in, rg, rf, mc, lnew, ch);
+            }
+            if (r == 0 && ybase == 0) {
+#pragma unroll
+                for (int k = 0; k < PX; k++) mc[k] = e[k];
+                lnew = 0;
+            }
+            if (r == R - 1) {
+                const int msk = (r < nr) ? -1 : 0;
+                acc_l0 = (__float_as_int(mc[0]) ^ __float_as_int(mo[0])) & msk;
+                acc_l1 = (__float_as_int(mc[1]) ^ __float_as_int(mo[1])) & msk;
+            }
+#pragma unroll
+            for (int k = 0; k < PX; k++) { mp[k] = mc[k]; q_mo[r][k] = mc[k]; }
+            q_lo[r] = (LV) lnew;
+        }
+    };
+    auto store_u = [&](int ybase) {
+        const bool own_ = is_own();
+        const unsigned inc = own_ ? (unsigned) stride : 0u, inc4 = inc * 4u;
+        unsigned so = own_ ? (unsigned) ybase * (unsigned) stride + (unsigned) x0 : (unsigned) h * (unsigned) stride + (unsigned) (PX * lane), so4 = so * 4u;
+        const int nr = min(R, h - ybase);
+#pragma unroll
+        for (int r = 0; r < R; r++, so += inc, so4 += inc4) {
+            if (r < nr) {
+                *(GFV *) ((gu8 *) c.m + so4) = q_mo[r];
+                *(GLV *) (c.least + so) = q_lo[r];
+            }
+        }
+    };
+    auto wait_level = [&](int L, int spec_t, const LvMask &prev, unsigned long long &fw, unsigned long long (&g)[PX]) -> int {
+        const unsigned want = ((unsigned) epoch << 10) | (unsigned) L;
+        gu64 *fsrc = flagw + (size_t) ((L - 1) & 1) * 2 * LV_PMAX + (lane < 2 * P ? lane : 0);
+        const bool need_g = spec_t >= 0 && prev.has(owner_of(spec_t)) && (in_k(0) || in_k(1));
+        gu64 *gsrc = gran + ((size_t) ((L - 1) & 1) * ntiles + (need_g ? owner_of(spec_t) : 0)) * OWN + (need_g ? owner_col : 0);
+        int sp = 0;
+        while (true) {
+            const size_t off = (!(dbg & 4) && (sp & 3) != 3) ? near_off : 0;
+            fw = __hip_atomic_load(fsrc + off, __ATOMIC_RELAXED, __HIP_MEMORY_SCOPE_AGENT);
+            if (spec_t >= 0) {
+#pragma unroll
+                for (int k = 0; k < PX; k++) g[k] = __hip_atomic_load(gsrc + off + k, __ATOMIC_RELAXED, __HIP_MEMORY_SCOPE_AGENT);
+            }
+            const bool okf = __all(lane >= 2 * P || (unsigned) (fw >> 32) == want);
+            bool okg = true;
+#pragma unroll
+            for (int k = 0; k < PX; k++) okg &= (unsigned) (g[k] >> 32) == want;
+            if (okf && __all(!need_g || okg)) return 0;
+            if (dbg & 2) __builtin_amdgcn_s_sleep(16); else if (okf || sp < 8) __builtin_amdgcn_s_sleep(1); else if (sp < 64) __builtin_amdgcn_s_sleep(8); else __builtin_amdgcn_s_sleep(48);
+            ++sp;
+            if ((sp & 255) == 0 && dev_failed(dev_err)) return 1;
+            if (sp > (1 << 18)) { if (lane == 0) dev_fail(dev_err, DEVERR_TILE_TIMEOUT); return 1; }
+        }
+    };
+    auto row_above = [&](int L, int t, const LvMask &prev, bool have_g, unsigned long long (&g)[PX]) -> int {
+        const int u = owner_of(t);
+        const bool from_gran = prev.has(u) && (in_k(0) || in_k(1));
+        if (!have_g) {
+            gu64 *src = gran + ((size_t) ((L - 1) & 1) * ntiles + (from_gran ? u : 0)) * OWN + (from_gran ? owner_col : 0);
+            const unsigned want = ((unsigned) epoch << 10) | (unsigned) L;
+            int sp = 0;
+            while (true) {
+                const size_t off = (!(dbg & 4) && (sp & 3) != 3) ? near_off : 0;
+#pragma unroll
+                for (int k = 0; k < PX; k++) g[k] = __hip_atomic_load(src + off + k, __ATOMIC_RELAXED, __HIP_MEMORY_SCOPE_AGENT);
+                bool ok = true;
+#pragma unroll
+                for (int k = 0; k < PX; k++) ok &= (unsigned) (g[k] >> 32) == want;
+                if (__all(ok || !from_gran)) break;
+                __builtin_amdgcn_s_sleep(1);
+                if (++sp > (1 << 16)) { if (lane == 0) dev_fail(dev_err, DEVERR_TILE_TIMEOUT); return 1; }
+            }
+        }
+#pragma unroll
+        for (int k = 0; k < PX; k++) mp[k] = !in_k(k) ? INF : from_gran ? __uint_as_float((unsigned) g[k]) : q_ab[k];
+        return 0;
+    };
+    unsigned n_proc = 0, n_idle = 0, n_sync = 0, n_two = 0;
+    int hold_L = -1;
+#ifdef LQR_TIMING
+    unsigned long long ltt[10] = {0, 0, 0, 0, 0, 0, 0, 0, 0, 0};
+    unsigned long long ltprev = __builtin_readcyclecounter();
+    const unsigned long long ltstart = ltprev;
+#endif
+    for (int L = 0; L <= nblk; L++) {
+        const bool mine = (L & 1) == q;
+        int t = -1;
+        bool have_g = false, passed = false;
+        unsigned long long g[PX] = {0ull, 0ull};
+        LvMask A = {0ull}, A_prev = {0ull};
+        if (L > 0) A_prev.lo = uni64(LV_A[(L - 1) & 1]);
+        LTT(8);
+        if (mine) {
+            unsigned long long fw = 0;
+            A = touch_mask(L);
+            passed = true;
+            if (L > 0) {
+                const int spec_t = (hold_L < 0 && cur_full && cur_L == L && L < nblk && !(dbg & 1)) ? cur_t : -1;
+                LJIT(1);
+                const int wl_rc = wait_level(L, spec_t, A_prev, fw, g);
+                LJIT(2);
+                LTT(0);
+                if (wl_rc) { LDS_FLAG(s_fail) = 1; passed = false; }
+                else if (L < nblk) {
+                    const int wl = (int) (unsigned) fw;
+                    bool act = false;
+                    unsigned wo[2], wr[2], wlf[2];
+#pragma unroll
+                    for (int i = 0; i < 2; i++) {
+                        wo[i] = (unsigned) __builtin_amdgcn_ds_bpermute((ix_own + i) << 2, wl);
+                        wr[i] = (unsigned) __builtin_amdgcn_ds_bpermute((ix_right + i) << 2, wl);
+                        wlf[i] = (unsigned) __builtin_amdgcn_ds_bpermute((ix_left + i) << 2, wl);
+                    }
+#pragma unroll
+                    for (int i = 0; i < 2; i++) {
+                        act |= (wo[i] & 0x900u) == 0x900u && (int) (wo[i] & 0xffu) == lane;
+                        act |= (wr[i] & 0xa00u) == 0xa00u && (int) (wr[i] & 0xffu) == lane + 1;
+                        act |= (wlf[i] & 0xc00u) == 0xc00u && (int) (wlf[i] & 0xffu) == lane - 1;
+                    }
+                    A.lo |= __ballot(act && lane < ntiles);
+                    have_g = spec_t >= 0;
+                }
+            }
+            if (lane == 0) { LV_A[L & 1] = A.lo; if (passed) LDS_FLAG(LV_POLLED) = L; }
+        } else {
+            int spins = 0;
+            while (LDS_FLAG(LV_POLLED) < L && LDS_FLAG(s_fail) != 1 && ++spins < (1 << 24)) __builtin_amdgcn_s_sleep(1);
+            passed = LDS_FLAG(LV_POLLED) >= L;
+            if (passed) A.lo = uni64(LV_A[L & 1]);
+            else if (LDS_FLAG(s_fail) != 1) { LDS_FLAG(s_fail) = 1; if (lane == 0) dev_fail(dev_err, DEVERR_TILE_TIMEOUT); }
+            LTT(2);
+        }
+        LTT(1);
+        LJIT(3);
+        if (hold_L >= 0 && passed) { store_u(hold_L * R); hold_L = -1; }
+        LTT(3);
+        if (L == nblk) break;
+        if (mine && passed && any_collision(A)) {
+            if (slot == 0 && lane == 0) { __hip_atomic_fetch_min(c.flags + FLAG_OVF_ROW, L * R, __ATOMIC_RELAXED, __HIP_MEMORY_SCOPE_AGENT); atomicAdd(&LV_STATS[0], 1ull); }
+            LDS_FLAG(s_fail) = 2;
+            passed = false;
+        }
+        if (passed) t = my_tile(A, mine ? 0 : 1);
+        if (!mine && t < 0 && passed && lane == 0) {
+            const unsigned long long tag = (unsigned long long) (((unsigned) epoch << 10) | (unsigned) (L + 1)) << 32;
+            gu64 *fdst = flagw + (size_t) (L & 1) * 2 * LV_PMAX + 2 * slot + 1;
+            if (!(dbg & 4)) __hip_atomic_store(fdst + near_off, tag, __ATOMIC_RELAXED, __HIP_MEMORY_SCOPE_WORKGROUP);
+            __hip_atomic_store(fdst, tag, __ATOMIC_RELAXED, __HIP_MEMORY_SCOPE_AGENT);
+        }
+        {
+            int ld_t = -1, ld_L = L;
+            if (t >= 0) {
+                if (!(cur_full && cur_t == t && cur_L == L)) { ld_t = t; n_sync++; have_g = false; }
+                if (!mine) n_two++;
+            } else if (!mine && passed && L + 1 < nblk) {
+                LvMask M = touch_mask(L + 1);
+                M.lo |= A.lo;
+                int pt = my_tile(M, 0);
+                if (pt < 0 && M.first() >= 0) { pt = nearest_tile(M.first(), M.last()); if (pt < M.first() - 1 || pt > M.last() + 1 || pt >= ntiles) pt = -1; }
+                ld_t = pt; ld_L = L + 1;
+                cur_t = -1; cur_L = ld_L; cur_full = false;
+            }
+            LTT(1);
+            LJIT(4);
+            if (ld_t >= 0) { set_tile(ld_t); issue_full(ld_L); cur_t = ld_t; cur_L = ld_L; cur_full = true; }
+#ifdef LQR_TIMING
+            if (t >= 0 && ld_t >= 0) asm volatile("s_waitcnt vmcnt(0)" ::: "memory");
+#endif
+            LTT(4);
+        }
+        unsigned word = 0;
+        if (t >= 0) {
+            n_proc++;
+            if (L > 0 && row_above(L, t, A_prev, have_g, g)) LDS_FLAG(s_fail) = 1;
+#ifdef LQR_TIMING
+            asm volatile("s_waitcnt vmcnt(0)" ::: "memory");
+#endif
+            LTT(5);
+            if (!is_interior()) {
+                const bool ik[PX] = {in_k(0), in_k(1)};
+#pragma unroll
+                for (int r = 0; r < R; r++)
+#pragma unroll
+                    for (int k = 0; k < PX; k++) { q_e[r][k] = ik[k] ? q_e[r][k] : INF; q_mo[r][k] = ik[k] ? q_mo[r][k] : INF; }
+            }
+            batch_u(L * R);
+            LTT(6);
+            hold_L = L;
+            cur_full = false;
+            LJIT(5);
+            if (L + 1 < nblk && own_lane) {
+                gu64 *dst = gran + ((size_t) (L & 1) * ntiles + t) * OWN + PX * (lane - HL);
+                const unsigned long long tag = (unsigned long long) (((unsigned) epoch << 10) | (unsigned) (L + 1)) << 32;
+#pragma unroll
+                for (int k = 0; k < PX; k++) {
+                    if (!(dbg & 4)) __hip_atomic_store(dst + near_off + k, tag | __float_as_uint(mp[k]), __ATOMIC_RELAXED, __HIP_MEMORY_SCOPE_WORKGROUP);
+                    __hip_atomic_store(dst + k, tag | __float_as_uint(mp[k]), __ATOMIC_RELAXED, __HIP_MEMORY_SCOPE_AGENT);
+                }
+            }
+            const bool chg = own_lane && (acc_l0 | acc_l1) != 0;
+            const bool any_o = __any(chg), any_l = __any(chg && lane < 32), any_r = __any(chg && lane >= 32);
+            word = 0x800u | (any_o ? 0x100u : 0u) | (any_l ? 0x200u : 0u) | (any_r ? 0x400u : 0u) | (unsigned) t;
+        } else if (mine && passed) n_idle++;
+        LJIT(6);
+        if (lane == 0 && (t >= 0 || mine) && LDS_FLAG(s_fail) == 0) {
+            const unsigned long long tag = (unsigned long long) (((unsigned) epoch << 10) | (unsigned) (L + 1)) << 32;
+            gu64 *fdst = flagw + (size_t) (L & 1) * 2 * LV_PMAX + 2 * slot + (mine ? 0 : 1);
+            if (!(dbg & 4)) __hip_atomic_store(fdst + near_off, tag | word, __ATOMIC_RELAXED, __HIP_MEMORY_SCOPE_WORKGROUP);
+            __hip_atomic_store(fdst, tag | word, __ATOMIC_RELAXED, __HIP_MEMORY_SCOPE_AGENT);
+        }
+        LTT(7);
+        LV_LEVEL_END
+        LTT(8);
+        if (LDS_FLAG(s_fail)) return;
+    }
+#ifdef LQR_TIMING
+    if (image == 0 && lane == 0 && slot < 16) { ltt[9] = __builtin_readcyclecounter() - ltstart; for (int i = 0; i < 10; i++) LV_TIME[slot][q][i] = ltt[i]; }
+#endif
+    if (lane == 0) { atomicAdd(&LV_STATS[2], (unsigned long long) n_proc); atomicAdd(&LV_STATS[3], (unsigned long long) n_idle); if (n_two) atomicAdd(&LV_STATS[4], (unsigned long long) n_two); }
+    if (lane == 0 && n_sync) atomicAdd(&LV_STATS[1], (unsigned long long) n_sync);
diff --git a/gimp-lqr-plugin_amd/csrc/k_levels_undef.inc b/gimp-lqr-plugin_amd/csrc/k_levels_undef.inc
--- /dev/null
+++ b/gimp-lqr-plugin_amd/csrc/k_levels_undef.inc
@@ -0,0 +1,12 @@
+#undef LV_NT
+#undef LV_SLOT_STATE
+#undef LV_POLLED
+#undef LV_A
+#undef LV_WAVE
+#undef LV_BLOCK
+#undef LV_INIT_FLAGS
+#undef LV_AFTER_SETUP
+#undef LV_DBG
+#undef LV_STATS
+#undef LV_TIME
+#undef LV_LEVEL_END
diff --git a/gimp-lqr-plugin_amd/csrc/lqr_geom.h b/gimp-lqr-plugin_amd/csrc/lqr_geom.h
--- a/gimp-lqr-plugin_amd/csrc/lqr_geom.h
+++ b/gimp-lqr-plugin_amd/csrc/lqr_geom.h
@@ -55,6 +55,9 @@
 struct LvBlock { int image, slot; };
 constexpr unsigned lv_grid(size_t n, int P) { return (unsigned) (8 * ((n + 7) / 8) * P); }
 constexpr LvBlock lv_block(int b, int P) { return LvBlock{((b >> 3) / P) * 8 + (b & 7), (b >> 3) % P}; }
+constexpr int lv2_pairs(int P) { return (P + 1) / 2; }
+constexpr unsigned lv2_grid(size_t n, int P) { return (unsigned) (8 * ((n + 7) / 8) * lv2_pairs(P)); }
+constexpr LvBlock lv2_block(int b, int P) { return LvBlock{((b >> 3) / lv2_pairs(P)) * 8 + (b & 7), (b >> 3) % lv2_pairs(P)}; }
 
 struct CuBlock { bool energy; int image, index; };
 constexpr int cu_energy_blocks(int n, int h) { return n * bb_energy_entries(h); }
diff --git a/gimp-lqr-plugin_amd/csrc/lqr_kernels.h b/gimp-lqr-plugin_amd/csrc/lqr_kernels.h
--- a/gimp-lqr-plugin_amd/csrc/lqr_kernels.h
+++ b/gimp-lqr-plugin_amd/csrc/lqr_kernels.h
@@ -62,6 +62,12 @@
 template <bool LR, bool RIG, int DELTA, bool RIGM>
 __global__ __launch_bounds__(128) __attribute__((amdgpu_waves_per_eu(2, 2))) void k_band_levels(DevCarver *cs, DpK p, int w, int h, int stride, unsigned long long *exch, int epoch, int *dev_err, int P, int n_img);
 
+#define K_BAND_LEVELS2_FORMS(X) X(false, false) X(false, true) X(true, false) X(true, true)
+template <bool LR, bool RIG>
+__global__ __launch_bounds__(256) __attribute__((amdgpu_waves_per_eu(2, 2))) void k_band_levels2(DevCarver *cs, DpK p, int w, int h, int stride, unsigned long long *exch, int epoch, int *dev_err, int P, int n_img);
+void lqr_levels2_debug(int v);
+int lqr_levels2_stats(unsigned long long *out, int reset);
+
 __global__ __launch_bounds__(256) void k_vs_commit(const DevCarver *cs, int w0, int h0, int wc0, int n_seams, int first_level, int finish);
 template <bool DEEP> __global__ __launch_bounds__(256) void k_inflate(const InflateDev *jobs, int w0, int w1, int l, int max_level, int *dev_err);
 __global__ __launch_bounds__(256) void k_vmap_check(const int32_t *map, int len, int depth, int *dev_err);
diff --git a/gimp-lqr-plugin_amd/csrc/lqr_levels.h b/gimp-lqr-plugin_amd/csrc/lqr_levels.h
--- /dev/null
+++ b/gimp-lqr-plugin_amd/csrc/lqr_levels.h
@@ -0,0 +1,26 @@
+#pragma once
+#include "lqr_common.h"
+#ifdef LQR_TIMING
+#define LTT(i) do { __builtin_amdgcn_sched_barrier(0); const unsigned long long t__ = __builtin_readcyclecounter(); __builtin_amdgcn_sched_barrier(0); ltt[i] += t__ - ltprev; ltprev = t__; } while (0)
+#else
+#define LTT(i) do { } while (0)
+#endif
+
+#ifdef LQR_JITTER
+#define LJIT(site) do { if (dbg & 16) { unsigned h__ = (unsigned) (slot * 131 + L * 17 + (site) * 7 + epoch * 2654435761u + q * 40503u + image * 977u); h__ ^= h__ >> 13; h__ *= 0x5bd1e995u; h__ ^= h__ >> 15; \
+    for (unsigned i__ = h__ & 15u; i__ > 0; i__--) __builtin_amdgcn_s_sleep(127); } } while (0)
+#else
+#define LJIT(site) do { } while (0)
+#endif
+__device__ __forceinline__ unsigned long long uni64(unsigned long long v)
+{
+    return ((unsigned long long) (unsigned) __builtin_amdgcn_readfirstlane((int) (v >> 32)) << 32) | (unsigned) __builtin_amdgcn_readfirstlane((int) v);
+}
+struct LvMask {
+    unsigned long long lo;
+    __device__ __forceinline__ void set(int t) { lo |= 1ull << t; }
+    __device__ __forceinline__ bool has(int t) const { return t >= 0 && t < LV_MAX_TILES && ((lo >> t) & 1ull); }
+    __device__ __forceinline__ void set_range(int a, int b) { lo |= ((b - a >= 63) ? ~0ull : ((1ull << (b - a + 1)) - 1ull)) << a; }
+    __device__ __forceinline__ int first() const { return lo ? __builtin_ctzll(lo) : -1; }
+    __device__ __forceinline__ int last() const { return lo ? 63 - __builtin_clzll(lo) : -1; }
+};
diff --git a/gimp-lqr-plugin_amd/csrc/lqr_plan.h b/gimp-lqr-plugin_amd/csrc/lqr_plan.h
--- a/gimp-lqr-plugin_amd/csrc/lqr_plan.h
+++ b/gimp-lqr-plugin_amd/csrc/lqr_plan.h
@@ -38,6 +38,7 @@
     int backtrack_beside = -1;
     int update_mode = -1;
     int band_levels = -1;
+    int levels_wg_slots = -1;
     int dpp_limit = -1;
     int dpp_px = 0;
     int sub_batches = 0;
@@ -45,6 +46,7 @@
 };
 struct PlanDevice {
     int wgs_plain = 0, wgs_general = 0, wgs_px4 = 0, wgs_levels = 0;
+    int wgs_levels2 = 0;
     int n_cu = 0, hw_queues = 0;
 };
 struct PlanBatch {
@@ -75,6 +77,7 @@
     bool full = false;
     int band = -1;
     int levels_P = 0;
+    int levels_wg_slots = 1;
     DpPlan dp;
 };
 
@@ -140,6 +143,13 @@
     const int want = k.band_levels > 0 ? k.band_levels : std::max(LV_AUTO_MIN, std::min(12, (int) ((b.shared ? 384 : 2 * d.n_cu) / std::max<size_t>(b.group(), 1))));
     const int P = std::min({LV_PMAX, per_batch / std::max(b.images, 1), want});
     return P >= (k.band_levels > 0 ? 1 : LV_AUTO_MIN) ? P : 0;
+}
+static inline int plan_levels_wg_slots(const PlanKnobs &k, const PlanDevice &d, const PlanBatch &b, int delta, bool general, int P)
+{
+    if (k.levels_wg_slots == 1 || !b.spin || delta != 1 || general || P < 2) return 1;
+    if ((size_t) lv2_grid((size_t) b.images, P) > (size_t) (plan_limit(k, d.wgs_levels2) / std::max(b.shared_n, 1))) return 1;
+    if (k.levels_wg_slots == 2) return 2;
+    return !b.shared && b.group() * (size_t) P > (size_t) d.n_cu ? 2 : 1;
 }
 static inline int plan_general_batch_limit(const PlanKnobs &k, const PlanDevice &d, int w, int delta)
 {
@@ -188,7 +198,7 @@
     const bool tiled = (plain ? (mode < 0 ? (long long) b.images * w * h <= k.tiled_update_px : mode == 1) : (fast_delta && mode != 0 && mode != 2 && mode != 3)) &&
                        plan_persistent_px(k, d, b, w, general, delta, b.images) != 0;
     if (fast_delta && mode != 3 && (mode == 5 || levels_auto(k, delta, b.group(), plain))) s.levels_P = plan_levels_P(k, d, b, wnew, h, delta);
-    if (s.levels_P > 0) s.band = LQRHIP_CENSUS_BAND_LEVELS;
+    if (s.levels_P > 0) { s.band = LQRHIP_CENSUS_BAND_LEVELS; s.levels_wg_slots = plan_levels_wg_slots(k, d, b, delta, general, s.levels_P); }
     else if (tiled) {
         s.dp = plan_persistent(plan_persistent_px(k, d, b, wnew, general, delta, b.images), general, b.images);
         return s;
diff --git a/gimp-lqr-plugin_amd/csrc/lqr_shim.hip b/gimp-lqr-plugin_amd/csrc/lqr_shim.hip
--- a/gimp-lqr-plugin_amd/csrc/lqr_shim.hip
+++ b/gimp-lqr-plugin_amd/csrc/lqr_shim.hip
@@ -146,8 +146,8 @@
 {
     hipDeviceProp_t prop;
     if (hipGetDeviceProperties(&prop, dev) != hipSuccess || prop.multiProcessorCount <= 0) return;
-    enum { PX4, PLAIN, GENERAL, LEVELS, N_CLASSES };
-    int per_cu[N_CLASSES] = {1 << 20, 1 << 20, 1 << 20, 1 << 20};
+    enum { PX4, PLAIN, GENERAL, LEVELS, LEVELS2, N_CLASSES };
+    int per_cu[N_CLASSES] = {1 << 20, 1 << 20, 1 << 20, 1 << 20, 1 << 20};
     auto q = [&](int cls, auto kern, int threads) {
         int n = 0;
         if (hipOccupancyMaxActiveBlocksPerMultiprocessor(&n, kern, threads, 0) != hipSuccess) { (void) hipGetLastError(); n = 0; }
@@ -159,12 +159,16 @@
 #define QUERY(...) q(LEVELS, k_band_levels<__VA_ARGS__>, 128);
     K_BAND_LEVELS_FORMS(QUERY)
 #undef QUERY
+#define QUERY(...) q(LEVELS2, k_band_levels2<__VA_ARGS__>, 256);
+    K_BAND_LEVELS2_FORMS(QUERY)
+#undef QUERY
     auto bound = [&](int blocks) { return std::max(0, blocks - 1) * prop.multiProcessorCount; };
     g_dev.n_cu = prop.multiProcessorCount;
     g_dev.wgs_px4 = bound(per_cu[PX4]);
     g_dev.wgs_plain = bound(std::min(per_cu[PX4], per_cu[PLAIN]));
     g_dev.wgs_general = bound(per_cu[GENERAL]);
     g_dev.wgs_levels = bound(per_cu[LEVELS]);
+    g_dev.wgs_levels2 = bound(per_cu[LEVELS2]);
 }
 
 static bool kfd_is_open(void)
@@ -968,6 +972,9 @@
 extern "C" void lqrhip_set_dp_persistent_px(int px) { g_knobs.dpp_px = (px == 2 || px == 3 || px == 4) ? px : 0; }
 extern "C" void lqrhip_set_dp_persistent_limit(int workgroups) { g_knobs.dpp_limit = workgroups; }
 extern "C" void lqrhip_set_band_levels(int slots) { g_knobs.band_levels = slots; }
+extern "C" void lqrhip_set_levels_wg_slots(int slots) { g_knobs.levels_wg_slots = slots == 1 || slots == 2 ? slots : -1; }
+static unsigned long long g_levels_pair_launches = 0;
+extern "C" unsigned long long lqrhip_levels_pair_launches(int reset) { const unsigned long long n = g_levels_pair_launches; if (reset) g_levels_pair_launches = 0; return n; }
 static PlanBatch plan_batch(const LqrHipBatch *b)
 {
     PlanBatch pb;
@@ -1134,7 +1141,7 @@
     return 0;
 }
 
-static int launch_band_levels(LqrHipBatch *b, const DpK &k, int w, int h, int lr, int P, bool rigm)
+static int launch_band_levels(LqrHipBatch *b, const DpK &k, int w, int h, int lr, int P, int wg_slots, bool rigm)
 {
     LqrHipCarver *c0 = b->cs[0];
     const size_t n = b->cs.size();
@@ -1144,6 +1151,16 @@
     const dim3 grid(lv_grid(n, P));
     CENSUS(LQRHIP_CENSUS_BAND_LEVELS);
     const DpForm f = dp_form(k, lr, rigm);
+    if (wg_slots == 2) {
+        const dim3 grid2(lv2_grid(n, P));
+#define CASE(LR, RIG) if (f.lr == LR && f.rig == RIG && f.delta == 1 && !f.rigm) \
+        hipLaunchKernelGGL((k_band_levels2<LR, RIG>), grid2, dim3(256), 0, b->stream, b->d_desc, k, w, h, c0->stride, b->exch.get(), epoch, g_dev_err, P, (int) n); else
+        K_BAND_LEVELS2_FORMS(CASE) return no_form("k_band_levels2");
+#undef CASE
+        HIPCK(hipGetLastError());
+        g_levels_pair_launches++;
+        return 0;
+    }
 #define CASE(LR, RIG, DELTA, RIGM) if (f.lr == LR && f.rig == RIG && f.delta == DELTA && f.rigm == RIGM) \
         hipLaunchKernelGGL((k_band_levels<LR, RIG, DELTA, RIGM>), grid, dim3(128), 0, b->stream, b->d_desc, k, w, h, c0->stride, b->exch.get(), epoch, g_dev_err, P, (int) n); else
     K_BAND_LEVELS_FORMS(CASE) return no_form("k_band_levels");
@@ -1268,7 +1285,7 @@
     const DpK &k = v.k;
     if (s.band == LQRHIP_CENSUS_BAND_LEVELS) {
         ProfScope ps("band_levels", b->stream, 0);
-        if (int rc = launch_band_levels(b, k, wnew, h, leftright_next, s.levels_P, v.rigm)) return rc;
+        if (int rc = launch_band_levels(b, k, wnew, h, leftright_next, s.levels_P, s.levels_wg_slots, v.rigm)) return rc;
     } else if (s.band == LQRHIP_CENSUS_BAND_TW) {
         ProfScope ps("band_update", b->stream, 0);
         CENSUS(LQRHIP_CENSUS_BAND_TW);
diff --git a/include/lqr_hip.h b/include/lqr_hip.h
--- a/include/lqr_hip.h
+++ b/include/lqr_hip.h
@@ -161,6 +161,8 @@
 int lqrhip_prof_get_union(const char *kernel, double *ms_union);
 int lqrhip_moved_bytes(unsigned long long *bytes, int reset);
 void lqrhip_set_band_levels(int slots);
+void lqrhip_set_levels_wg_slots(int slots);
+unsigned long long lqrhip_levels_pair_launches(int reset);
 int lqrhip_band_levels_stats(unsigned long long *out8, int reset);
 enum {
     LQRHIP_CENSUS_VP_PARALLEL = 0,
```

New measurement: 543,300 Mseams*px/s, median of 6. 1.01x the previous value.
